# noahares/raxtax

Measured on AMD Instinct MI355X. Metric: classified queries/sec (whole node), higher is better.
Workload: dtype u32 bit-planes + f64

## Files before the change

raxtax_amd/csrc/rtx_api_batch.hip:

```cpp
#include "rtx_index.hpp"

#ifndef RTX_B2_HEAVY_PER_ATILE
#define RTX_B2_HEAVY_PER_ATILE 4u
#endif

namespace rtxi {

int bind(rtx_index *ix) {
    if (!ix) { set_error("null index handle"); return RTX_ERR_INVALID; }
    RTX_HIP(hipSetDevice(ix->device));
    return RTX_OK;
}

int ensure_events(rtx_index *ix, size_t count) {
    while (ix->events.size() < count) {
        hipEvent_t e;
        RTX_HIP(hipEventCreate(&e));
        ix->events.push_back(e);
    }
    return RTX_OK;
}


SubBatch sub_batch_of(rtx_index *ix, uint32_t sb, bool timed) {
    const rtx_index::SubPlan &p = ix->plan[sb];
    SubBatch b;
    b.sb = sb;
    b.q0 = p.q0;
    b.nq = p.nq;
    b.cls = &ix->cls[p.cls];
    b.set = ix->staged ? (sb & 1u) : 0u;
    b.s = ix->stream;
    b.timed = timed;
    b.timed_all = timed && ix->stage_timing != 0;
    return b;
}

int plan_sub_batches(rtx_index *ix) {
    ix->plan.clear();
    uint64_t pos = 0;
    for (uint32_t c = 0; c < ix->n_cls; c++) {
        ix->cls[c].pos0 = pos;
        pos += ix->cls[c].n;
    }
    if (pos != ix->n_q) { set_error("internal: the length classes hold %llu of %llu queries", (unsigned long long)pos, (unsigned long long)ix->n_q); return RTX_ERR_STATE; }
    for (int pass = 0; pass < 2; pass++)
        for (uint32_t c = 0; c < ix->n_cls; c++) {
            rtx_index::BatchClass &k = ix->cls[c];
            if (k.side != (pass == 0)) continue;
            k.sb0 = ix->n_sub_total();
            for (uint64_t a = 0; a < k.n; a += k.sub_batch) ix->plan.push_back({k.pos0 + a, (uint32_t)std::min<uint64_t>(k.sub_batch, k.n - a), c});
            k.n_sub = ix->n_sub_total() - k.sb0;
        }
    return RTX_OK;
}

constexpr uint32_t kDietMinRows = 1024;
uint32_t diet_rows(const rtx_index *ix, uint32_t B) { return std::min<uint32_t>(B, std::max<uint32_t>(kDietMinRows, B >> ix->diet_shift)); }
uint32_t counts_rows_layout(const rtx_index *ix, const rtx_index::BatchClass &k) { return k.diet && !ix->dbg_full_run && !ix->dbg_full ? k.cnt_rows : k.sub_batch; }
uint8_t *counts_lo(rtx_index *ix, rtx_index::Scratch &sc) { return reinterpret_cast<uint8_t *>(sc.d_counts.p); }
uint16_t *counts_hi(rtx_index *ix, const rtx_index::BatchClass &k, rtx_index::Scratch &sc) {
    return reinterpret_cast<uint16_t *>(reinterpret_cast<uint8_t *>(sc.d_counts.p) + (size_t)counts_rows_layout(ix, k) * ix->npad);
}
int ensure_full_counts(rtx_index *ix, const rtx_index::BatchClass &k, rtx_index::Scratch &sc) { return sc.d_counts.alloc(counts_elems(ix, k.planes, k.sub_batch)); }

hipEvent_t stage_event(rtx_index *ix, const SubBatch &b, int stage, int which) {
    return ix->events[((size_t)b.sb * RTX_NUM_STAGES + stage) * 2 + which];
}

static KmerParams kmer_params(rtx_index *ix, const SubBatch &b) {
    rtx_index::Scratch &sc = ix->sc[b.set];
    rtx_index::ResultSet &r = ix->res();
    const rtx_index::BatchClass &k = *b.cls;
    KmerParams kp{};
    kp.bases = ix->d_bases.p;
    kp.base_off = ix->in[ix->cur_in].d_base_off.p;
    kp.q0 = b.q0;
    kp.perm = r.d_perm.p;
    kp.row_of = ix->d_row_of.p;
    kp.list_len = ix->d_list_len.p;
    kp.row_len = ix->d_row_len.p;
    kp.zero_row = ix->n_rows;
    kp.kmers = sc.d_kmers.p;
    kp.kstride = k.kstride;
    kp.seginfo = ix->d_seginfo.p;
    kp.seg_stride = ix->seg_stride;
    kp.segcls = ix->d_segcls.p;
    kp.cls_stride = ix->cls_stride;
    kp.ntiles = ix->ntiles;
    kp.seg_dbits = ix->d_seg_dbits.p;
    kp.seg_sbits = ix->d_seg_sbits.p;
    kp.seg_sbase = ix->d_seg_sbase.p;
    kp.seg_blocks = ix->seg_blocks;
    kp.rows = sc.d_rows.p;
    kp.rstride = k.rstride;
    kp.dmask = sc.d_dmask.p;
    kp.srows = sc.d_srows.p;
    kp.nsparse = sc.d_nsparse.p;
    kp.t = sc.d_t.p;
    kp.nrows = sc.d_nrows.p;
    kp.hq = r.d_hq.p;
    kp.t_all = r.d_t_all.p;
    kp.nrows_all = r.d_nrows_all.p;
    kp.hist = sc.d_hist.p;
    kp.hstride = k.hstride;
    return kp;
}

static bool run_prunes(const rtx_index *ix, const rtx_index::BatchClass &k) { return k.prune && !ix->dbg_full_run; }
static bool on_records_path(const rtx_index *ix, const rtx_index::BatchClass &k, const rtx_index::Scratch &sc) { return run_prunes(ix, k) && k.rec && sc.d_rec.p != nullptr; }
static bool on_diet(const rtx_index *ix, const rtx_index::BatchClass &k, const rtx_index::Scratch &sc) { return on_records_path(ix, k, sc) && k.diet && sc.d_cnt_row.p != nullptr; }

static RecordRef record_ref(const rtx_index *ix, const rtx_index::Scratch &sc, const rtx_index::ResultSet &r) { return RecordRef{sc.d_rec_nslots.p, sc.d_rec_slots.p, sc.d_rec_cnt.p, sc.d_rec.p, ix->rec_slots(), ix->rec_seg_len, r.d_flags.p}; }
static ProbTables prob_tables(const rtx_index *ix) { return ProbTables{ix->d_tab_cmf.p, ix->d_tab_ratio.p, ix->d_tab_off.p, ix->d_tab_moff.p, ix->d_tab_ilo.p, ix->d_tab_sat.p, ix->tab_tmax}; }

int enqueue_kmer(rtx_index *ix, const SubBatch &b, hipStream_t s) {
    KmerParams kp = kmer_params(ix, b);
    kp.mode = run_prunes(ix, *b.cls) && ix->seg_blocks ? 1u : 0u;
    if (b.timed_all) RTX_HIP(hipEventRecord(stage_event(ix, b, RTX_STAGE_KMER_EXTRACT, 0), s));
    launch_kmer_extract(s, kp, b.nq);
    if (b.timed_all) RTX_HIP(hipEventRecord(stage_event(ix, b, RTX_STAGE_KMER_EXTRACT, 1), s));
    return RTX_OK;
}

static HitParams hit_params(rtx_index *ix, const SubBatch &b, uint32_t flags) {
    rtx_index::Scratch &sc = ix->sc[b.set];
    rtx_index::ResultSet &r = ix->res();
    const rtx_index::BatchClass &k = *b.cls;
    HitParams hp{};
    hp.bitmap = ix->d_bitmap.p;
    hp.stride_bytes = ix->stride_bytes;
    hp.n_rows1 = ix->n_rows + 1;
    hp.n_refs = ix->n_refs;
    hp.ref_base = ix->ref_lo;
    hp.rows = sc.d_rows.p;
    hp.rstride = k.rstride;
    hp.dmask = sc.d_dmask.p;
    hp.nrows = sc.d_nrows.p;
    hp.zero_row = ix->n_rows;
    hp.srows = sc.d_srows.p;
    hp.nsparse = sc.d_nsparse.p;
    hp.segslots = ix->d_segslots.p;
    hp.ntiles = ix->ntiles;
    hp.t = sc.d_t.p;
    hp.counts = sc.d_counts.p;
    hp.counts_lo = ix->packs(k.planes) ? counts_lo(ix, sc) : nullptr;
    hp.counts_hi = ix->packs(k.planes) ? counts_hi(ix, k, sc) : nullptr;
    hp.npad = ix->npad;
    hp.hist = sc.d_hist.p;
    hp.hstride = k.hstride;
    hp.tile_max = sc.d_tilemax.p;
    hp.flags = flags;
    hp.q0 = b.q0;
    hp.perm = r.d_perm.p;
    hp.exact = ExactRef{ix->in[ix->cur_in].d_exact_ids.p, ix->in[ix->cur_in].d_exact_off.p, r.dev_exact ? r.d_exact_grp.p : nullptr, ix->d_em_goff.p, ix->d_em_gids.p};
    hp.nq = b.nq;
    hp.group_rows = k.pair ? ix->d_group_rows.p : nullptr;
    hp.group_base = b.sb * ix->groups_per_sub;
    hp.pair_urec = sc.d_urec.p;
    hp.pair_nu = sc.d_nu.p;
    hp.pair_ustride = 2u * k.rstride;
    return hp;
}

static HitParams bounds_params(const rtx_index *ix, const rtx_index::Scratch &sc, const HitParams &hp) {
    HitParams up = hp;
    up.bitmap = ix->d_ubitmap.p;
    up.stride_bytes = ix->u_stride_bytes;
    up.n_refs = ix->u_nblocks;
    up.dmask = nullptr;
    up.nsparse = nullptr;
    up.ntiles = ix->u_ntiles;
    up.counts = nullptr;
    up.counts_lo = nullptr;
    up.counts_hi = nullptr;
    up.hist = nullptr;
    up.tile_max = nullptr;
    up.bounds_tile_ub = sc.d_tile_ub.p;
    up.bounds_tile_stride = ix->ntiles;
    up.bounds_ntiles = ix->ntiles;
    up.bounds_best = sc.d_best_key.p;
    up.flags = 0;
    up.group_base = hp.group_base + ix->n_groups_run;
    return up;
}

static Bounds2Params bounds2_params(const rtx_index *ix, const rtx_index::Scratch &sc, const HitParams &up, bool heavy) {
    Bounds2Params bp{};
    bp.abitmap = ix->d_abitmap.p;
    bp.bbitmap = ix->d_bbitmap.p;
    bp.n_rows1 = ix->n_rows + 1;
    bp.n_atiles = ix->n_atiles;
    bp.ntiles = ix->ntiles;
    bp.zero_row = ix->n_rows;
    bp.pair_urec = sc.d_urec.p;
    bp.pair_nu = sc.d_nu.p;
    bp.pair_ustride = up.pair_ustride;
    bp.nq = up.nq;
    bp.t = sc.d_t.p;
    bp.tile_ub = sc.d_tile_ub.p;
    bp.tile_ub_stride = ix->ntiles;
    bp.best_key = sc.d_best_key.p;
    bp.delta_ct = ix->b2_delta[0];
    bp.delta_cm = ix->b2_delta[1];
    bp.delta_lo = ix->b2_delta[2];
    bp.delta_hi = ix->b2_delta[3];
    bp.group_rows = up.group_rows;
    bp.group_base = up.group_base;
    bp.heavy = heavy ? sc.d_heavy.p : nullptr;
    bp.heavy_max = std::max<uint32_t>(1u, std::min<uint32_t>(RTX_B2_HEAVY_PER_ATILE * ix->n_atiles, ix->n_btiles / 2u));
    return bp;
}

static PruneParams prune_params(rtx_index *ix, const SubBatch &b, uint32_t flags, int part, const ExactRef &exact) {
    rtx_index::Scratch &sc = ix->sc[b.set];
    const rtx_index::BatchClass &k = *b.cls;
    PruneParams pr{};
    pr.tile_ub = sc.d_tile_ub.p;
    pr.best_key = sc.d_best_key.p;
    pr.tile_ub_stride = ix->ntiles;
    pr.ntiles = ix->ntiles;
    pr.nq = b.nq;
    pr.n_refs = ix->n_refs;
    pr.n_total = ix->n_total;
    pr.ref_base = ix->ref_lo;
    pr.phase = (uint32_t)part;
    pr.best = part ? sc.d_best.p : nullptr;
    pr.bitmap = ix->d_bitmap.p;
    pr.cbitmap = part == 0 && (ix->two_level_used || (k.planes > kBounds2MaxPlanes && ix->two_level_opt && ix->n_refs == ix->n_total)) ? reinterpret_cast<const uint2 *>(ix->d_cbitmap.p) : nullptr;
    pr.n_rows1 = ix->n_rows + 1;
    pr.stride_bytes = ix->stride_bytes;
    pr.rows = sc.d_rows.p;
    pr.rstride = k.rstride;
    pr.nrows = sc.d_nrows.p;
    pr.t = sc.d_t.p;
    pr.flags = flags;
    pr.q0 = b.q0;
    pr.perm = ix->res().d_perm.p;
    pr.exact = exact;
    pr.lnfact = ix->d_lnfact.p;
    pr.inv = ix->d_inv.p;
    pr.nlf = std::min<uint32_t>(kLnFactLen, k.tmax + k.tmax / 2 + 2);
    pr.hist = sc.d_hist.p;
    pr.hstride = k.hstride;
    pr.live = sc.d_live.p;
    pr.live_words = LiveLayout{ix->ntiles}.words();
    pr.pair_live = ItemsLayout(b.nq, ix->ntiles).pair_live(sc.d_items.p);
    pr.thr_out = sc.d_prune_thr.p;
    pr.i1_out = sc.d_prune_i1.p;
    pr.stats = ix->d_prune_stats.p;
    pr.detail = ix->debug_taps && ix->d_prune_detail.n >= (size_t)b.nq * kPruneDetailWords ? ix->d_prune_detail.p : nullptr;
    return pr;
}

static HitParams fine_params(const rtx_index *ix, const rtx_index::Scratch &sc, const HitParams &hp) {
    HitParams fp = hp;
    fp.bitmap = ix->d_fbitmap.p;
    fp.stride_bytes = ix->f_stride_bytes;
    fp.n_refs = ix->f_nblocks;
    fp.ntiles = ix->f_ntiles;
    fp.counts = nullptr;
    fp.counts_lo = nullptr;
    fp.counts_hi = nullptr;
    fp.tile_max = nullptr;
    fp.flags = 0;
    fp.group_rows = nullptr;
    fp.live = sc.d_live.p;
    fp.live_words = LiveLayout{ix->ntiles}.words();
    fp.prune_thr = sc.d_prune_thr.p;
    fp.fine_n_refs = ix->n_refs;
    fp.fine_ref_ntiles = ix->ntiles;
    fp.fine_stats = ix->d_prune_stats.p + 2 * kPruneStatCopies * 8;
    return fp;
}

int enqueue_hit(rtx_index *ix, const SubBatch &b, uint32_t flags, hipStream_t s, int part, hipStream_t s_mid) {
    rtx_index::Scratch &sc = ix->sc[b.set];
    rtx_index::ResultSet &r = ix->res();
    const rtx_index::BatchClass &k = *b.cls;
    ix->last_set = b.set;
    HitParams hp = hit_params(ix, b, flags);
    const bool prune = run_prunes(ix, k);
    if (k.pair && part != 2) {
        if (b.timed_all) RTX_HIP(hipEventRecord(stage_event(ix, b, RTX_STAGE_PAIR_UNION, 0), s));
        launch_pair_union(s, sc.d_rows.p, sc.d_nrows.p, k.rstride, b.nq, sc.d_urec.p, sc.d_nu.p, 2u * k.rstride);
        if (b.timed_all) RTX_HIP(hipEventRecord(stage_event(ix, b, RTX_STAGE_PAIR_UNION, 1), s));
    }
    if (b.timed && !prune) RTX_HIP(hipEventRecord(stage_event(ix, b, RTX_STAGE_HIT_COUNT, 0), s));
    if (part != 0 && !prune) { set_error("internal: a split run without tile pruning"); return RTX_ERR_STATE; }
    if (prune) {
        if (part != 2) {
            const HitParams up = bounds_params(ix, sc, hp);
            if (b.timed) RTX_HIP(hipEventRecord(stage_event(ix, b, RTX_STAGE_TILE_BOUNDS, 0), s));
            ix->two_level_used = part == 0 && ix->two_level_opt && ix->d_abitmap.p && ix->d_bbitmap.p && ix->n_refs == ix->n_total && k.planes <= kBounds2MaxPlanes;
            if (ix->two_level_used) {
                const bool heavy_ok = sc.d_heavy.p && sc.d_heavy_items.p && sc.d_heavy_items.n >= HeavyItemsLayout(b.nq, ix->u_ntiles).total();
                launch_bounds2(s, bounds2_params(ix, sc, up, heavy_ok), b.nq, k.planes, up, ix->u_ntiles, heavy_ok ? sc.d_heavy_items.p : nullptr);
            } else {
                RTX_HIP(hipMemsetAsync(sc.d_best_key.p, 0, (size_t)b.nq * 4, s));
                launch_hit_count_pair_bounds(s, up, b.nq, ix->u_ntiles, k.planes);
            }
            if (b.timed) RTX_HIP(hipEventRecord(stage_event(ix, b, RTX_STAGE_TILE_BOUNDS, 1), s));
        }
        if (s_mid && s_mid != s && part == 0) {
            RTX_HIP(hipEventRecord(ix->ev_mid[b.sb], s));
            RTX_HIP(hipStreamWaitEvent(s_mid, ix->ev_mid[b.sb], 0));
            s = s_mid;
        }
        if (b.timed && part != 1) RTX_HIP(hipEventRecord(stage_event(ix, b, RTX_STAGE_TILE_PRUNE, 0), s));
        PruneParams pr = prune_params(ix, b, flags, part, hp.exact);
        const bool records = part == 0 && on_records_path(ix, k, sc), diet = part == 0 && on_diet(ix, k, sc);
        const RecordRef rr = record_ref(ix, sc, r);
        if (records) { pr.rec = rr; pr.rec_max_slots = rr.stride; }
        if (k.diet && !diet) { set_error("internal: the counts buffer is on its diet without the records path"); return RTX_ERR_STATE; }
        if (diet) {
            RTX_HIP(hipMemsetAsync(sc.d_cnt_cursor.p, 0, 4, s));
            pr.cnt_row = sc.d_cnt_row.p;
            pr.cnt_cursor = sc.d_cnt_cursor.p;
            pr.cnt_cap = k.cnt_rows;
            pr.flags_out = r.d_flags.p;
            hp.cnt_row = sc.d_cnt_row.p;
        }
        launch_prune(s, pr, prob_tables(ix), b.nq);
        if (part == 1) { RTX_HIP(hipGetLastError()); return RTX_OK; }
        if (part == 0 && ix->fine_opt && ix->d_fbitmap.p && k.pair && sc.d_fine_items.p) {
            const FineItemsLayout fine(b.nq, ix->f_ntiles);
            uint32_t *const fi = sc.d_fine_items.p;
            launch_fine_bounds(s, fine_params(ix, sc, hp), b.nq, ix->ntiles, ix->f_ntiles, pr.pair_live, fine.cursors(fi), fine.items(fi), fine.count(fi), k.planes);
        }
        RTX_HIP(hipMemsetAsync(sc.d_tilemax.p, 0, (size_t)b.nq * ix->ntiles * 2, s));
        hp.live = sc.d_live.p;
        hp.live_words = pr.live_words;
        hp.prune_thr = sc.d_prune_thr.p;
        if (records) hp.rec = rr;
        if (k.pair) {
            const ItemsLayout items(b.nq, ix->ntiles);
            launch_live_items(s, sc.d_live.p, pr.live_words, pr.pair_live, b.nq, ix->ntiles, items.offsets(sc.d_items.p), items.items(sc.d_items.p), items.count(sc.d_items.p));
            hp.items = items.items(sc.d_items.p);
            hp.n_items = items.count(sc.d_items.p);
        }
        if (ix->seg_blocks) {
            KmerParams kp = kmer_params(ix, b);
            kp.mode = 2u;
            kp.live = sc.d_live.p;
            kp.live_words = pr.live_words;
            launch_kmer_extract(s, kp, b.nq);
        }
        if (b.timed) {
            RTX_HIP(hipEventRecord(stage_event(ix, b, RTX_STAGE_TILE_PRUNE, 1), s));
            RTX_HIP(hipEventRecord(stage_event(ix, b, RTX_STAGE_HIT_COUNT, 0), s));
        }
    }
    if (k.pair) launch_hit_count_pair(s, hp, b.nq, ix->ntiles, k.planes);
    else launch_hit_count(s, hp, b.nq, ix->ntiles, k.planes);
    if (b.timed) RTX_HIP(hipEventRecord(stage_event(ix, b, RTX_STAGE_HIT_COUNT, 1), s));
    ix->hit_stream = s;
    return RTX_OK;
}

int enqueue_count(rtx_index *ix, const SubBatch &b, uint32_t flags, hipStream_t s_mid) {
    int rc = enqueue_kmer(ix, b, b.s);
    return rc ? rc : enqueue_hit(ix, b, flags, b.s, 0, s_mid);
}

static WalkParams walk_params(rtx_index *ix, const SubBatch &b, const double *prefix);
static int reset_sub_alloc(rtx_index *ix, hipStream_t s);

int enqueue_prob_prefix(rtx_index *ix, const SubBatch &b, bool fuse_walk, bool prob_only) {
    rtx_index::Scratch &sc = ix->sc[b.set];
    const rtx_index::BatchClass &k = *b.cls;
    hipStream_t s = b.s;
    ProbParams pp{};
    pp.t = sc.d_t.p;
    pp.hist = sc.d_hist.p;
    pp.hstride = k.hstride;
    pp.tmax = k.tmax;
    pp.n1max = k.tmax / 2 + 1;
    pp.lnfact = ix->d_lnfact.p;
    pp.n_refs = ix->n_total;
    pp.q0 = b.q0;
    pp.table_z = sc.d_table_z.p;
    rtx_index::ResultSet &r = ix->res();
    pp.z = r.d_z.p;
    pp.gs = r.d_gs.p;
    pp.status = r.d_status.p;
    pp.ndist = r.d_ndist.p;
    pp.prune_thr = run_prunes(ix, k) ? sc.d_prune_thr.p : nullptr;
    pp.prune_i1 = pp.prune_thr ? sc.d_prune_i1.p : nullptr;
    if (b.timed_all) RTX_HIP(hipEventRecord(stage_event(ix, b, RTX_STAGE_PROB_TABLE, 0), s));
    if (k.use_tables) {
        launch_prob_order(s, sc.d_t.p, b.nq, sc.d_order.p);
        pp.order = sc.d_order.p;
        launch_prob_lookup(s, pp, prob_tables(ix), b.nq);
    } else {
        if (k.huge) {
            pp.gstride = (uint32_t)((prob_table_lds_bytes(k.tmax) + 7) / 8);
            if (ix->d_prob_scratch.n < (size_t)b.nq * pp.gstride) { set_error("internal: scratch of prob_table too small"); return RTX_ERR_STATE; }
            pp.gscratch = ix->d_prob_scratch.p;
        }
        launch_prob_table(s, pp, b.nq);
    }
    if (b.timed_all) RTX_HIP(hipEventRecord(stage_event(ix, b, RTX_STAGE_PROB_TABLE, 1), s));
    if (prob_only) return RTX_OK;

    PrefixParams fp{};
    fp.status = r.d_status.p;
    fp.t = sc.d_t.p;
    fp.tz_in_lds = (size_t)k.hstride * 8 <= 16 * 1024 ? 1u : 0u;
    fp.q0 = b.q0;
    fp.counts = sc.d_counts.p;
    fp.counts_lo = counts_lo(ix, sc);
    fp.counts_hi = counts_hi(ix, k, sc);
    fp.packed = ix->packs(k.planes) ? 1u : 0u;
    fp.npad = ix->npad;
    fp.table_z = sc.d_table_z.p;
    fp.hstride = k.hstride;
    fp.n_refs = ix->n_refs;
    fp.bnd_bits = ix->d_bnd_bits.p;
    fp.bnd_rank = ix->d_bnd_rank.p;
    fp.prefix = sc.d_prefix.p;
    fp.n_bnd = ix->n_bnd_local;
    fp.tile_max = ix->tile_skip ? sc.d_tilemax.p : nullptr;
    fp.ntiles = ix->ntiles;
    fp.prune_thr = pp.prune_thr;
    fp.prune_stats = fp.prune_thr ? ix->d_prune_stats.p + kPruneStatCopies * 8 : nullptr;
    fp.fuse_walk = fuse_walk ? 1u : 0u;
    const bool records = fuse_walk && on_records_path(ix, k, sc);
    fp.rec_nslots = records ? sc.d_rec_nslots.p : nullptr;
    fp.cnt_row = fuse_walk && on_diet(ix, k, sc) ? sc.d_cnt_row.p : nullptr;
    if (fuse_walk) {
        fp.walk = walk_params(ix, b, sc.d_prefix.p);
        int rc_r = fp.walk.sub_alloc ? reset_sub_alloc(ix, s) : RTX_OK;
        if (rc_r) return rc_r;
    }
    if (b.timed_all) RTX_HIP(hipEventRecord(stage_event(ix, b, RTX_STAGE_TAXON_PREFIX, 0), s));
    launch_taxon_prefix(s, fp, b.nq);
    if (records) {
        TailParams tp{};
        tp.rec = record_ref(ix, sc, r);
        tp.t = sc.d_t.p;
        tp.table_z = sc.d_table_z.p;
        tp.hstride = k.hstride;
        tp.bnd_bits = ix->d_bnd_bits.p;
        tp.bnd_rank = ix->d_bnd_rank.p;
        tp.prefix = sc.d_prefix.p;
        if (fp.cnt_row) { tp.cnt_cursor = sc.d_cnt_cursor.p; tp.cnt_cap = k.cnt_rows; tp.flags_out = r.d_flags.p; }
        tp.n_bnd = ix->n_bnd_local;
        tp.nq = b.nq;
        tp.walk = fp.walk;
        tp.prefix_stats = fp.prune_stats;
        tp.stats = ix->d_prune_stats.p ? ix->d_prune_stats.p + 3 * kPruneStatCopies * 8 : nullptr;
        launch_records_tail(s, tp, b.nq);
    }
    if (b.timed_all) RTX_HIP(hipEventRecord(stage_event(ix, b, RTX_STAGE_TAXON_PREFIX, 1), s));
    return RTX_OK;
}

int alloc_result_set(rtx_index *ix, rtx_index::ResultSet &r, uint64_t n_queries, uint64_t min_arena) {
    int rc;
    if ((rc = r.d_status.alloc(n_queries)) || (rc = r.d_t_all.alloc(n_queries)) || (rc = r.d_nrows_all.alloc(n_queries)) ||
        (rc = r.d_n_rows.alloc(n_queries)) || (rc = r.d_gs.alloc(n_queries)) || (rc = r.d_z.alloc(n_queries)) ||
        (rc = r.d_hq.alloc(n_queries)) || (rc = r.d_row_start.alloc(n_queries)) || (rc = r.d_ndist.alloc(n_queries)) ||
        (rc = r.d_cursor.alloc(2)) || (rc = r.d_flags.alloc(1)))
        return rc;
    const uint64_t want_arena = std::max<uint64_t>(n_queries * 10 + 4096, min_arena);
    if (r.arena_cap < want_arena) {
        if ((rc = r.d_arena.alloc(want_arena))) return rc;
        r.arena_cap = want_arena;
    }
    return alloc_final(ix, r, n_queries);
}

int settle_join(rtx_index *ix) {
    if (ix->join_pending && ix->join_ev) RTX_HIP(hipStreamWaitEvent(ix->stream, ix->join_ev, 0));
    ix->join_pending = false;
    return RTX_OK;
}

int alloc_final(rtx_index *ix, rtx_index::ResultSet &r, uint64_t n_queries) {
    int rc;
    if ((rc = r.d_fin_t.alloc(n_queries)) || (rc = r.d_fin_status.alloc(n_queries)) || (rc = r.d_fin_gs.alloc(n_queries)) ||
        (rc = r.d_fin_row_begin.alloc(n_queries)) || (rc = r.d_fin_row_count.alloc(n_queries)) || (rc = r.d_fin_cursor.alloc(2)))
        return rc;
    if ((rc = r.d_peak2.alloc(n_queries)) || (rc = r.d_peak.alloc(n_queries)) || (rc = r.d_strand.alloc(n_queries))) return rc;
    if (ix->nearest_opt && ((rc = r.d_nearest2.alloc(n_queries)) || (rc = r.d_ties2.alloc(n_queries)) || (rc = r.d_nearest.alloc(n_queries)) || (rc = r.d_ties.alloc(n_queries))))
        return rc;
    if (ix->identity_opt && ((rc = r.d_dist.alloc(n_queries)) || (rc = r.d_qlen.alloc(n_queries)))) return rc;
    if (ix->strand_opt && ((rc = r.d_sel_t.alloc(n_queries)) || (rc = r.d_sel_status.alloc(n_queries)) || (rc = r.d_sel_gs.alloc(n_queries)) ||
                           (rc = r.d_sel_row_begin.alloc(n_queries)) || (rc = r.d_sel_row_count.alloc(n_queries))))
        return rc;
    const uint64_t rows = r.arena_cap, D = ix->fin_D;
    if ((rc = r.d_fin_lineage.alloc(rows)) || (rc = r.d_fin_node.alloc(rows)) || (rc = r.d_fin_depth.alloc(rows)) || (rc = r.d_fin_depth8.alloc(rows)) ||
        (rc = r.d_fin_local.alloc(rows)) || (rc = r.d_fin_conf.alloc(rows * D)) || (rc = r.d_fin_hund.alloc(rows * D)))
        return rc;
    r.fin_cap = rows;
    return RTX_OK;
}

int enqueue_finalise(rtx_index *ix, const SubBatch &b, hipStream_t s) {
    rtx_index::ResultSet &r = ix->res();
    FinaliseParams fp{};
    fp.status = r.d_status.p;
    fp.t_all = r.d_t_all.p;
    fp.gs = r.d_gs.p;
    fp.n_rows = r.d_n_rows.p;
    fp.row_start = r.d_row_start.p;
    fp.arena = r.d_arena.p;
    fp.arena_cap = r.arena_cap;
    fp.perm = r.d_perm.p;
    fp.q0 = b.q0;
    fp.nq = b.nq;
    fp.node_depth = ix->d_node_depth.p;
    fp.node_sig0 = ix->d_node_sig0.p;
    fp.node_begin = ix->d_node_begin.p;
    fp.node_eb = ix->d_node_eb.p;
    fp.D = ix->fin_D;
    fp.o_t = r.d_fin_t.p;
    fp.o_status = r.d_fin_status.p;
    fp.o_gs = r.d_fin_gs.p;
    fp.o_row_begin = r.d_fin_row_begin.p;
    fp.o_row_count = r.d_fin_row_count.p;
    fp.r_lineage = r.d_fin_lineage.p;
    fp.r_node = r.d_fin_node.p;
    fp.r_depth = r.d_fin_depth.p;
    fp.r_depth8 = r.d_fin_depth8.p;
    fp.r_hund = r.d_fin_hund.p;
    fp.r_local = r.d_fin_local.p;
    fp.r_conf = r.d_fin_conf.p;
    fp.row_cap = r.fin_cap;
    fp.fin_cursor = r.d_fin_cursor.p;
    fp.flags_out = r.d_flags.p;
    launch_finalise(s, fp);
    if (r.stream_dl && b.sb < r.h_fin_sub.size())
        RTX_HIP(hipMemcpyAsync(&r.h_fin_sub[b.sb], r.d_fin_cursor.p, 8, hipMemcpyDeviceToHost, s));
    return RTX_OK;
}

static WalkParams walk_params(rtx_index *ix, const SubBatch &b, const double *prefix) {
    rtx_index::ResultSet &r = ix->res();
    WalkParams wp{};
    wp.status = r.d_status.p;
    wp.q0 = b.q0;
    wp.prefix = prefix;
    wp.n_bnd = ix->n_bnd;
    wp.rec = ix->d_noderec.p;
    wp.arena = r.d_arena.p;
    const bool side = b.cls->side;
    wp.arena_cap = side ? r.arena_cap : r.side_base;
    wp.arena_cursor = r.d_cursor.p + (side ? 1 : 0);
    wp.sub_alloc = !side && b.nq >= kWalkSubMinQueries && r.arena_cap < (1ull << 32) ? ix->d_sub_alloc.p : nullptr;
    wp.n_rows = r.d_n_rows.p;
    wp.row_start = r.d_row_start.p;
    wp.flags_out = r.d_flags.p;
    return wp;
}
static int reset_sub_alloc(rtx_index *ix, hipStream_t s) {
    if (ix->d_sub_alloc.p) RTX_HIP(hipMemsetAsync(ix->d_sub_alloc.p, 0, (size_t)kWalkSubAllocs * kWalkSubStride * 8, s));
    return RTX_OK;
}

int enqueue_walk(rtx_index *ix, const SubBatch &b, const double *prefix, hipStream_t s) {
    const WalkParams wp = walk_params(ix, b, prefix);
    int rc_r = wp.sub_alloc ? reset_sub_alloc(ix, s) : RTX_OK;
    if (rc_r) return rc_r;
    if (b.timed_all) RTX_HIP(hipEventRecord(stage_event(ix, b, RTX_STAGE_LINEAGE_WALK, 0), s));
    launch_lineage_walk(s, wp, b.nq);
    if (b.timed_all) RTX_HIP(hipEventRecord(stage_event(ix, b, RTX_STAGE_LINEAGE_WALK, 1), s));
    return RTX_OK;
}

int order_batch(rtx_index *ix, bool cluster) {
    const uint32_t n = (uint32_t)ix->n_q;
    rtx_index::ResultSet &r = ix->res();
    int rc;
    if ((rc = r.d_perm.alloc(n)) || (rc = r.d_iperm.alloc(n))) return rc;
    const bool multi = ix->n_cls > 1;
    const bool sketch = cluster && n > 2;
    if (sketch || multi) {
        if ((rc = ix->d_skey_in.alloc(n)) || (rc = ix->d_skey_out.alloc(n)) || (rc = ix->d_sidx.alloc(n))) return rc;
        size_t tmp = 0;
        if (cluster_sort(ix->stream, nullptr, &tmp, ix->d_skey_in.p, ix->d_skey_out.p, ix->d_sidx.p, r.d_perm.p, n, multi)) {
            set_error("radix sort: size query failed");
            return RTX_ERR_HIP;
        }
        if (ix->d_sort_tmp.n < tmp && (rc = ix->d_sort_tmp.alloc(tmp + 256))) return rc;
        if (sketch) {
            launch_sketch(ix->stream, ix->d_bases.p, ix->in[ix->cur_in].d_base_off.p, n, ix->d_skey_in.p, ix->d_sidx.p);
            if (ix->d_loc_table.p && ix->locator_opt)
                launch_locator(ix->stream, ix->d_bases.p, ix->in[ix->cur_in].d_base_off.p, n, ix->d_loc_table.p, ix->n_total, ix->d_skey_in.p);
        }
        if (multi) launch_class_keys(ix->stream, ix->d_skey_in.p, ix->in[ix->cur_in].d_base_off.p, n, ix->key_lim, !sketch, ix->d_sidx.p);
        tmp = ix->d_sort_tmp.n;
        if (cluster_sort(ix->stream, ix->d_sort_tmp.p, &tmp, ix->d_skey_in.p, ix->d_skey_out.p, ix->d_sidx.p, r.d_perm.p, n, multi)) {
            set_error("radix sort of the query sketches failed");
            return RTX_ERR_HIP;
        }
        launch_invert_perm(ix->stream, r.d_perm.p, n, r.d_iperm.p);
    } else {
        launch_identity_perm(ix->stream, n, r.d_perm.p, r.d_iperm.p);
    }
    RTX_HIP(hipGetLastError());
    return RTX_OK;
}

void record_batch(rtx_index *ix) {
    rtx_index::ResultSet &r = ix->res();
    r.n_q = ix->n_q;
    r.n_user = ix->strand_used ? ix->n_user : ix->n_q;
    r.has_peak = false;
    r.has_nearest = false;
    r.has_identity = false;
    r.profiled = false;
    r.n_sub = ix->n_sub_total();
    r.n_side = 0;
    for (uint32_t c = 0; c < ix->n_cls; c++)
        if (ix->cls[c].side) r.n_side += ix->cls[c].n_sub;
    r.in_set = ix->cur_in;
    r.dev_exact = ix->dev_exact_used;
    r.stream_dl = false;
}

int begin_run(rtx_index *ix, uint32_t *n_sub_out, bool *timed_out, bool cluster) {
    int rc_p = plan_sub_batches(ix);
    if (rc_p) return rc_p;
    const uint32_t n_sub = ix->n_sub_total();
    record_batch(ix);
    rtx_index::ResultSet &r = ix->res();
    const bool timed = n_sub <= 4096;
    if (timed) {
        int rc = ensure_events(ix, (size_t)n_sub * RTX_NUM_STAGES * 2);
        if (rc) return rc;
    }
    const bool ev_all = timed && ix->stage_timing;
    if (ev_all) RTX_HIP(hipEventRecord(ix->events[(size_t)RTX_STAGE_ORDER * 2], ix->stream));
    int rc_o = order_batch(ix, cluster);
    if (rc_o) return rc_o;
    if (ev_all) RTX_HIP(hipEventRecord(ix->events[(size_t)RTX_STAGE_ORDER * 2 + 1], ix->stream));
    {
        uint64_t n_side_q = 0;
        for (uint32_t c = 0; c < ix->n_cls; c++)
            if (ix->cls[c].side) n_side_q += ix->cls[c].n;
        const uint64_t side_rows = n_side_q ? n_side_q * kWalkMaxRows + 64 : 0;
        if (side_rows + ix->n_q * 2 + 1024 > r.arena_cap) {
            int rc_a = r.d_arena.alloc(r.arena_cap + side_rows);
            if (rc_a) return rc_a;
            r.arena_cap += side_rows;
        }
        if (r.fin_cap < r.arena_cap || r.d_fin_t.n < ix->n_q) {
            int rc_f = alloc_final(ix, r, ix->n_q);
            if (rc_f) return rc_f;
        }
        r.side_base = r.arena_cap - side_rows;
        int rc_h = r.h_side_base.resize(2);
        if (rc_h) return rc_h;
        r.h_side_base[0] = 0;
        r.h_side_base[1] = r.side_base;
        RTX_HIP(hipMemcpyAsync(r.d_cursor.p, r.h_side_base.data(), 2 * sizeof(unsigned long long), hipMemcpyHostToDevice, ix->stream));
    }
    RTX_HIP(hipMemsetAsync(r.d_flags.p, 0, sizeof(uint32_t), ix->stream));
    RTX_HIP(hipMemsetAsync(r.d_fin_cursor.p, 0, 2 * sizeof(unsigned long long), ix->stream));
    const bool whole = ix->n_refs == ix->n_total && !ix->staged;
    const bool shard = ix->staged && ix->shard_prune_opt && ix->n_refs != ix->n_total;
    auto scratch_ok = [&](const rtx_index::Scratch &sc, uint32_t B) {
        const ScratchNeed n = ScratchNeed().set_queries(ix, B);
        return sc.d_tile_ub.p != nullptr && sc.d_tile_ub.n >= n.tile_ub && sc.d_best_key.n >= n.best_key && sc.d_prune_thr.n >= n.prune_thr &&
               sc.d_live.n >= n.live && sc.d_best.n >= n.best && sc.d_items.n >= n.items;
    };
    bool any_pair = false, any_prune = false;
    uint32_t b_max = 1;
    for (uint32_t c = 0; c < ix->n_cls; c++) {
        rtx_index::BatchClass &k = ix->cls[c];
        k.pair = ix->pair_opt && cluster && k.planes <= 11 && ix->n_q > 1 && k.rstride <= 4096;
        const rtx_index::Scratch &s0 = ix->sc[k.side ? kSideSet : 0u];
        ScratchNeed need = ScratchNeed().set_queries(ix, k.sub_batch);
        if (whole && ix->rec_opt != 0u && ix->pruning())
            for (uint32_t j = 0; j < 4u; j++) {
                rtx_index::Scratch &sc = ix->sc[j];
                if ((j == kSideSet) != k.side || sc.d_kmers.p == nullptr || sc.d_rec.p == nullptr || sc.d_rec.n >= need.rec) continue;
                RTX_HIP(hipStreamSynchronize(ix->stream));
                if (sc.d_rec.alloc(need.rec)) sc.d_rec.release();
            }
        k.prune = ix->pruning() && k.pair && k.use_tables && ix->tile_skip && ix->d_ubitmap.p && (whole || shard) &&
                  scratch_ok(s0, k.sub_batch) && (!ix->staged || scratch_ok(ix->sc[1], k.sub_batch));
        k.rec = k.prune && whole && ix->rec_opt != 0u && ix->n_bnd_local == ix->n_bnd && s0.d_rec.p != nullptr && s0.d_rec.n >= need.rec;
        auto diet_ok = [&](const rtx_index::Scratch &sc) { return sc.d_rec.p != nullptr && sc.d_cnt_row.p != nullptr && sc.d_cnt_cursor.p != nullptr && sc.d_cnt_row.n >= need.cnt_row; };
        k.diet = k.rec && diet_rows(ix, k.sub_batch) < k.sub_batch && diet_ok(s0);
        if (k.diet && !k.side)
            for (uint32_t j = 1; j <= 2u; j++)
                if (ix->sc[j].d_kmers.p != nullptr && !diet_ok(ix->sc[j])) k.diet = false;
        k.cnt_rows = k.diet ? diet_rows(ix, k.sub_batch) : k.sub_batch;
        {
            need.add_class(ix, k, k.sub_batch, k.cnt_rows);
            for (uint32_t j = 0; j < 4u; j++) {
                rtx_index::Scratch &sc = ix->sc[j];
                if ((j == kSideSet) != k.side || sc.d_kmers.p == nullptr || (sc.d_counts.n >= need.counts && sc.d_prefix.n >= need.prefix)) continue;
                RTX_HIP(hipStreamSynchronize(ix->stream));
                int rc_c = sc.d_counts.alloc(need.counts);
                if (!rc_c) rc_c = sc.d_prefix.alloc(need.prefix);
                if (rc_c) return rc_c;
            }
        }
        any_pair = any_pair || k.pair;
        any_prune = any_prune || k.prune;
        b_max = std::max(b_max, k.sub_batch);
    }
    ix->sub_batch_max = b_max;
    ix->any_prune = any_prune;
    ix->groups_per_sub = (b_max + 1u) / 2u;
    ix->dbg_full = false;
    if (any_prune) {
        int rc_s = ix->d_prune_stats.alloc(kPruneStatCopies * 32);
        if (!rc_s && ix->debug_taps) rc_s = ix->d_prune_detail.alloc((size_t)b_max * kPruneDetailWords);
        if (rc_s) return rc_s;
        RTX_HIP(hipMemsetAsync(ix->d_prune_stats.p, 0, kPruneStatCopies * 256, ix->stream));
    }
    if (any_pair) {
        ix->n_groups_run = n_sub * ix->groups_per_sub;
        int rc_g = ix->d_group_rows.alloc((size_t)2 * n_sub * ix->groups_per_sub);
        if (rc_g) return rc_g;
        RTX_HIP(hipMemsetAsync(ix->d_group_rows.p, 0, (size_t)2 * n_sub * ix->groups_per_sub * 4, ix->stream));
    }
    ix->n_sub_last = timed ? n_sub : 0;
    ix->overlap_used = 0;
    if (ix->overlap_opt != 0u && whole && n_sub >= 2 && !ix->shared_device && any_prune && ix->sc[1].d_kmers.p != nullptr && scratch_ok(ix->sc[1], b_max) == scratch_ok(ix->sc[0], b_max)) {
        ix->overlap_used = 2;
        if (ix->overlap_opt >= 2u && n_sub >= 3 && ix->sc[2].d_kmers.p != nullptr && scratch_ok(ix->sc[2], b_max) == scratch_ok(ix->sc[0], b_max)) ix->overlap_used = 3;
    }
    if (r.dev_exact) {
        ExactParams xp{ix->d_bases.p, ix->in[ix->cur_in].d_base_off.p, (uint32_t)ix->n_q, ix->d_em_table.p, ix->em_bits, ix->d_em_rep_off.p,
                       ix->d_em_rep_bytes.p, r.d_exact_grp.p, ix->em_hash_mask};
        const bool ev = timed && ix->stage_timing;
        if (ev) RTX_HIP(hipEventRecord(ix->events[(size_t)RTX_STAGE_EXACT_MATCH * 2], ix->stream));
        launch_exact_match(ix->stream, xp);
        if (ev) RTX_HIP(hipEventRecord(ix->events[(size_t)RTX_STAGE_EXACT_MATCH * 2 + 1], ix->stream));
        if (!r.ev_exact) RTX_HIP(hipEventCreateWithFlags(&r.ev_exact, hipEventDisableTiming));
        RTX_HIP(hipEventRecord(r.ev_exact, ix->stream));
    }
    *n_sub_out = n_sub;
    *timed_out = timed;
    return RTX_OK;
}

int enqueue_batch(rtx_index *ix, uint32_t flags) {
    if (ix->n_refs != ix->n_total) {
        set_error("this handle holds a reference shard: drive it with rtx_shard_count/_prob/_walk");
        return RTX_ERR_STATE;
    }
    uint32_t n_sub = 0;
    bool timed = false;
    int rc;
    if (ix->join_pending && !ix->hold_join && (rc = settle_join(ix))) return rc;
    rc = begin_run(ix, &n_sub, &timed, ix->cluster != 0);
    if (rc) return rc;
    rtx_index::ResultSet &r = ix->res();
    ix->n_near_last = 0;
    r.has_nearest = ix->nearest_opt != 0u && r.d_nearest2.p != nullptr && r.d_nearest2.n >= r.n_q && r.d_nearest.n >= r.n_user;
    if (ix->nearest_opt != 0u && !r.has_nearest) { set_error("internal: RTX_OPT_NEAREST without its arrays"); return RTX_ERR_STATE; }
    ix->ident_timed = false;
    r.has_identity = ix->identity_opt != 0u && r.has_nearest && r.d_dist.p != nullptr && r.d_dist.n >= r.n_user && r.d_qlen.n >= r.n_user && ix->d_em_ref_grp.p != nullptr;
    if (ix->identity_opt != 0u && !r.has_identity) { set_error("internal: RTX_OPT_IDENTITY without its arrays"); return RTX_ERR_STATE; }
    if (n_sub <= 4096) {
        if (!ix->copy_stream) RTX_HIP(hipStreamCreateWithFlags(&ix->copy_stream, hipStreamNonBlocking));
        while (r.ev_sub.size() < n_sub) {
            hipEvent_t e;
            RTX_HIP(hipEventCreateWithFlags(&e, hipEventDisableTiming));
            r.ev_sub.push_back(e);
        }
        if ((rc = r.h_cursor_sub.resize(n_sub)) || (rc = r.h_fin_sub.resize(n_sub))) return rc;
        r.stream_dl = true;
    }
    const bool fuse = ix->n_bnd_local == ix->n_bnd;
    const uint32_t nsets = ix->overlap_used;
    const bool overlap = nsets != 0u;
    if (overlap) {
        if (!ix->stream2) RTX_HIP(hipStreamCreateWithFlags(&ix->stream2, hipStreamNonBlocking));
        if (nsets == 3u && !ix->stream3) RTX_HIP(hipStreamCreateWithFlags(&ix->stream3, hipStreamNonBlocking));
        while (ix->ev_front.size() < n_sub) {
            hipEvent_t e, f, g;
            RTX_HIP(hipEventCreateWithFlags(&e, hipEventDisableTiming));
            RTX_HIP(hipEventCreateWithFlags(&f, hipEventDisableTiming));
            RTX_HIP(hipEventCreateWithFlags(&g, hipEventDisableTiming));
            ix->ev_front.push_back(e);
            ix->ev_back.push_back(f);
            ix->ev_mid.push_back(g);
        }
    }
    const uint32_t n_side = r.n_side;
    const bool ra = ix->run_ahead_opt != 0u && nsets == 2u && n_side == 0u && r.stream_dl && n_sub >= 2u;
    if (ix->join_pending) {
        if (ra) ix->join_pending = false;
        else if ((rc = settle_join(ix))) return rc;
    }
    if (ra)
        for (uint32_t k = 0; k < 2u; k++)
            if (!ix->ev_set_free[k]) RTX_HIP(hipEventCreateWithFlags(&ix->ev_set_free[k], hipEventDisableTiming));
    for (uint32_t sb = 0; sb < n_sub; sb++) {
        SubBatch b = sub_batch_of(ix, sb, timed);
        const bool side = b.cls->side;
        if (side) {
            b.set = kSideSet;
            if (overlap) {
                if (sb == 0) {
                    RTX_HIP(hipEventRecord(ix->ev_mid[0], ix->stream));
                    RTX_HIP(hipStreamWaitEvent(ix->stream2, ix->ev_mid[0], 0));
                }
                b.s = ix->stream2;
            }
        } else if (overlap) {
            const uint32_t m = sb - n_side;
            b.set = m % nsets;
            if (m >= nsets) RTX_HIP(hipStreamWaitEvent(ix->stream, ix->ev_back[sb - nsets], 0));
            else if (ra && ix->set_busy[b.set]) RTX_HIP(hipStreamWaitEvent(ix->stream, ix->ev_set_free[b.set], 0));
        }
        if ((rc = enqueue_count(ix, b, flags, nsets == 3u && !side && n_side == 0 ? ix->stream3 : nullptr))) return rc;
        if (overlap && !side) {
            RTX_HIP(hipEventRecord(ix->ev_front[sb], ix->hit_stream));
            b.s = ix->stream2;
            RTX_HIP(hipStreamWaitEvent(b.s, ix->ev_front[sb], 0));
        }
        {
            const rtx_index::Scratch &sc = ix->sc[b.set];
            launch_peak(b.s, PeakParams{sc.d_hist.p, b.cls->hstride, sc.d_t.p, b.q0, r.d_perm.p, b.nq, r.d_peak2.p});
        }
        if (r.has_nearest) {
            rtx_index::Scratch &sc = ix->sc[b.set];
            const rtx_index::BatchClass &k = *b.cls;
            NearestParams np{};
            np.hist = sc.d_hist.p;
            np.hstride = k.hstride;
            np.t = sc.d_t.p;
            np.q0 = b.q0;
            np.perm = r.d_perm.p;
            np.nq = b.nq;
            np.tile_max = sc.d_tilemax.p;
            np.ntiles = ix->ntiles;
            np.n_refs = ix->n_refs;
            np.counts = sc.d_counts.p;
            np.counts_lo = ix->packs(k.planes) ? counts_lo(ix, sc) : nullptr;
            np.counts_hi = ix->packs(k.planes) ? counts_hi(ix, k, sc) : nullptr;
            np.npad = ix->npad;
            np.cnt_rows = counts_rows_layout(ix, k);
            np.cnt_row = on_diet(ix, k, sc) ? sc.d_cnt_row.p : nullptr;
            if (on_records_path(ix, k, sc)) {
                const RecordRef rr = record_ref(ix, sc, r);
                np.rec_nslots = rr.nslots;
                np.rec_slots = rr.slots;
                np.rec_cnt = rr.cnt;
                np.rec = rr.rec;
                np.rec_stride = rr.stride;
                np.rec_seg_len = rr.seg_len;
            }
// ... 168 lines not shown
    k.hstride = (uint32_t)align_up(tmax + 1, 8);
    k.planes = tmax <= 255 ? 8 : (tmax <= 1023 ? 10 : (tmax <= kMidClassMaxT && mid ? 11 : (tmax <= 4095 ? 12 : 16)));
    k.huge = prob_table_lds_bytes((uint32_t)tmax) > kProbTableLdsLimit;
}

static int size_workspace(rtx_index *ix, uint64_t n_queries);

int prepare_workspace(rtx_index *ix, uint64_t n_queries, const uint64_t cls_n_in[5], const uint64_t cls_max_in[5]) {
    uint64_t cn[5], cm[5];
    for (int c = 0; c < 5; c++) { cn[c] = cls_n_in[c]; cm[c] = cls_max_in[c]; }
    if (ix->n_refs != ix->n_total) {
        uint64_t mx = 0;
        for (int c = 0; c < 5; c++) mx = std::max(mx, cm[c]);
        return prepare_workspace_single(ix, n_queries, mx >= 8 ? mx - 7 : 1, mx);
    }
    if (cn[0] && cn[1] && cn[0] < kMinShortClass) { cn[1] += cn[0]; cm[1] = std::max(cm[1], cm[0]); cn[0] = 0; cm[0] = 0; }
    if (cn[2] && ((cn[2] < kMinMidClass && ix->prob_mode != 2) || !ix->pair_opt || !ix->pruning() || ix->prob_mode == 1)) { cn[3] += cn[2]; cm[3] = std::max(cm[3], cm[2]); cn[2] = 0; cm[2] = 0; }
    if (cn[3] && cn[4] && cn[3] + cn[4] <= kSideMaxQueries) { cn[4] += cn[3]; cm[4] = std::max(cm[4], cm[3]); cn[3] = 0; cm[3] = 0; }
    const uint64_t key[14] = {n_queries, cn[0], cn[1], cn[2] << 32 | cn[3], cn[4], cm[0], cm[1], cm[2] << 32 | cm[3], cm[4], ix->sub_batch_req,
                              (uint64_t)ix->packed_opt | (uint64_t)ix->pair_opt << 1 | (uint64_t)ix->pruning() << 2 | (uint64_t)ix->shard_prune_opt << 3 | (uint64_t)ix->fine_opt << 4 |
                                  (uint64_t)(ix->prob_mode & 3) << 5 | (uint64_t)ix->rec_opt << 8 | (uint64_t)ix->overlap_opt << 16 | (uint64_t)ix->min_subs << 20,
                              (uint64_t)ix->n_bnd_local, ix->shared_device ? 1u : 0u, ix->strand_opt | ix->nearest_opt << 1 | ix->identity_opt << 2};
    if (ix->ws_valid && std::memcmp(key, ix->ws_key, sizeof key) == 0 && !ix->staged) {
        ix->n_q = n_queries;
        return RTX_OK;
    }
    ix->ws_valid = false;
    ix->n_cls = 0;
    const uint64_t cls_len[4] = {255 + 7, 1023 + 7, kMidClassMaxT + 7, class3_max_len()};
    for (int c = 0; c < 4; c++) ix->key_lim[c] = ~0ull;
    int last = -1;
    for (int c = 0; c < 5; c++) {
        if (!cn[c]) continue;
        if (last >= 0) ix->key_lim[ix->n_cls - 1] = cls_len[last];
        shape_class(ix->cls[ix->n_cls], cn[c], cm[c], c == 2);
        ix->n_cls++;
        last = c;
    }
    if (ix->n_cls == 0) { set_error("internal: a batch without queries"); return RTX_ERR_INVALID; }
    ix->n_q = n_queries;
    int rc = size_workspace(ix, n_queries);
    if (rc) return rc;
    std::memcpy(ix->ws_key, key, sizeof key);
    ix->ws_valid = true;
    return RTX_OK;
}

int prepare_workspace_single(rtx_index *ix, uint64_t n_queries, uint64_t tmax, uint64_t max_len) {
    ix->ws_valid = false;
    ix->strand_used = false;
    tmax = std::min<uint64_t>(tmax, 65535);
    ix->n_cls = 1;
    for (int c = 0; c < 4; c++) ix->key_lim[c] = ~0ull;
    shape_class(ix->cls[0], n_queries, tmax + 7);
    ix->cls[0].max_len = max_len;
    ix->n_q = n_queries;
    return size_workspace(ix, n_queries);
}

static int size_workspace(rtx_index *ix, uint64_t n_queries) {
    int rc;
    uint32_t tab_t = 0;
    for (uint32_t c = 0; c < ix->n_cls; c++) {
        if (ix->cls[c].tmax > kProbTablesMaxT && ix->prob_mode == 2) { set_error("prob tables need t <= %u (got %u)", kProbTablesMaxT, ix->cls[c].tmax); return RTX_ERR_TOO_LONG; }
        if (ix->cls[c].tmax <= kProbTablesMaxT && ix->cls[c].planes <= 11) tab_t = std::max(tab_t, ix->cls[c].tmax);
    }
    bool tables = false;
    if (tab_t && (rc = ensure_prob_tables(ix, tab_t, &tables))) return rc;
    for (uint32_t c = 0; c < ix->n_cls; c++) ix->cls[c].use_tables = tables && ix->cls[c].tmax >= 2 && ix->cls[c].tmax <= kProbTablesMaxT && ix->cls[c].planes <= 11;
    rtx_index::ResultSet &r = ix->res();
    if ((rc = alloc_result_set(ix, r, n_queries))) return rc;
    if ((rc = ix->d_sub_alloc.alloc((size_t)kWalkSubAllocs * kWalkSubStride))) return rc;
    const uint64_t want_arena = n_queries * 10 + 4096;
    uint32_t n_sets = ix->n_refs == ix->n_total && !ix->shared_device ? 1u + std::min<uint32_t>(ix->overlap_opt, 2u) : 1u;
    size_t free_b = 0, total_b = 0;
    RTX_HIP(hipMemGetInfo(&free_b, &total_b));
    uint64_t held = 0;
    for (const auto &sc : ix->sc) held += sc.d_counts.n * 2 + sc.d_prefix.n * 8 + sc.d_rec.n * 4 + sc.d_srows.n * 4;
    const uint64_t budget = (uint64_t)((free_b + held) * 0.6);
    uint64_t worst = 0;
    for (uint32_t c = 0; c < ix->n_cls; c++) {
        rtx_index::BatchClass &k = ix->cls[c];
        k.will_prune = ix->pruning() && ix->d_ubitmap.p && ix->pair_opt && ix->ntiles >= RTX_PRUNE_MIN_TILES && k.tmax <= kProbTablesMaxT && (ix->n_refs == ix->n_total || ix->shard_prune_opt);
        const uint64_t per_q = class_per_q(ix, k);
        uint32_t B = ix->sub_batch_req;
        if (B == 0) {
            B = (uint32_t)std::min<uint64_t>(k.will_prune ? kDefaultSubBatchPruned : ix->ntiles >= 16 ? kDefaultSubBatchLarge : kDefaultSubBatch,
                                             std::max<uint64_t>(64, budget / per_q));
            if (k.huge) B = std::min<uint32_t>(B, 1024u);
            if (k.will_prune && k.n < (uint64_t)ix->min_subs * B) B = (uint32_t)std::max<uint64_t>(16384, (k.n + ix->min_subs - 1) / ix->min_subs);
        }
        if (B > kMaxSubBatch) B = kMaxSubBatch;
        B = (uint32_t)std::max<uint64_t>(1, std::min<uint64_t>(B, k.n));
        k.sub_batch = B;
        worst = std::max<uint64_t>(worst, (uint64_t)B * per_q);
    }
    {
        uint32_t bulk = 0;
        for (uint32_t c = 1; c < ix->n_cls; c++)
            if (ix->cls[c].n > ix->cls[bulk].n) bulk = c;
        worst = 0;
        for (uint32_t c = 0; c < ix->n_cls; c++) {
            ix->cls[c].side = ix->n_refs == ix->n_total && c != bulk && ix->cls[c].n <= kSideMaxQueries && ix->cls[c].n * 64u <= ix->cls[bulk].n;
            if (!ix->cls[c].side) worst = std::max<uint64_t>(worst, (uint64_t)ix->cls[c].sub_batch * class_per_q(ix, ix->cls[c]));
        }
    }
    {
        uint64_t n_side_q = 0;
        for (uint32_t c = 0; c < ix->n_cls; c++)
            if (ix->cls[c].side) n_side_q += ix->cls[c].n;
        const uint64_t want2 = want_arena + (n_side_q ? n_side_q * kWalkMaxRows + 64 : 0);
        if (r.arena_cap < want2) {
            if ((rc = r.d_arena.alloc(want2))) return rc;
            r.arena_cap = want2;
        }
    }
    while (n_sets > 1u && (uint64_t)n_sets * worst > budget) n_sets--;
    ix->staged = false;
    if ((rc = plan_sub_batches(ix))) return rc;
    if ((rc = alloc_scratch_set(ix, 0))) return rc;
    {
        bool any_side = false;
        for (uint32_t c = 0; c < ix->n_cls; c++) any_side = any_side || ix->cls[c].side;
        if (any_side) { if ((rc = alloc_scratch_set(ix, kSideSet))) return rc; }
        else ix->sc[kSideSet].release_all();
    }
    for (uint32_t k = 1; k <= 2u; k++) {
        if (k < n_sets && ix->n_sub_total() > 1) {
            if (alloc_scratch_set(ix, k)) ix->sc[k].d_kmers.release();
        } else if (ix->n_refs == ix->n_total) {
            ix->sc[k].release_all();
        }
    }
    return RTX_OK;
}

int alloc_scratch_set(rtx_index *ix, uint32_t k) {
    int rc;
    rtx_index::Scratch &sc = ix->sc[k];
    const ScratchNeed n = scratch_set_need(ix, k);
    if ((rc = sc.d_kmers.alloc(n.kmers)) || (rc = sc.d_rows.alloc(n.rows)) || (rc = sc.d_dmask.alloc(n.dmask)) || (rc = sc.d_nsparse.alloc(n.nsparse)) || (rc = sc.d_srows.alloc(n.srows)) ||
        (rc = sc.d_t.alloc(n.t)) || (rc = sc.d_nrows.alloc(n.nrows)) || (rc = sc.d_counts.alloc(n.counts)) || (rc = sc.d_hist.alloc(n.hist)) || (rc = sc.d_table_z.alloc(n.hist)) ||
        (rc = sc.d_prefix.alloc(n.prefix)) || (rc = sc.d_order.alloc(n.order)) || (rc = sc.d_tilemax.alloc(n.tilemax)) || (rc = sc.d_urec.alloc(n.urec)) || (rc = sc.d_nu.alloc(n.nu)))
        return rc;
    if (n.prob_scratch && (rc = ix->d_prob_scratch.alloc(std::max(n.prob_scratch, ix->d_prob_scratch.n)))) return rc;
    if (ix->pruning() && ix->d_ubitmap.p && (ix->n_refs == ix->n_total || ix->shard_prune_opt)) {
        if ((rc = sc.d_tile_ub.alloc(n.tile_ub)) || (rc = sc.d_best_key.alloc(n.best_key)) || (rc = sc.d_prune_thr.alloc(n.prune_thr)) || (rc = sc.d_prune_i1.alloc(n.prune_i1)) ||
            (rc = sc.d_best.alloc(n.best)) || (rc = sc.d_live.alloc(n.live)) || (rc = sc.d_items.alloc(n.items)))
            return rc;
        if (ix->d_abitmap.p && (sc.d_heavy.alloc(n.heavy) || sc.d_heavy_items.alloc(n.heavy_items))) { sc.d_heavy.release(); sc.d_heavy_items.release(); }
        if (ix->d_fbitmap.p && sc.d_fine_items.alloc(n.fine_items)) sc.d_fine_items.release();
        if (ix->rec_opt && ix->n_refs == ix->n_total) {
            if (sc.d_rec_nslots.alloc(n.rec_nslots) || sc.d_rec_slots.alloc(n.rec_slots) || sc.d_rec_cnt.alloc(n.rec_cnt) ||
                sc.d_rec.alloc(n.rec) || sc.d_cnt_row.alloc(n.cnt_row) || sc.d_cnt_cursor.alloc(n.cnt_cursor))
                sc.d_rec.release();
        }
    }
    return RTX_OK;
}

}

extern "C" {

int rtx_batch_prefetch(rtx_index *ix, uint64_t n_queries, const uint8_t *bases, const uint64_t *base_off,
                       const uint32_t *exact_ids, const uint64_t *exact_off) {
    int rc = bind(ix);
    if (rc) return rc;
    rtx_index::Inputs &in = ix->in[ix->cur_in ^ 1u];
    const bool with_labels = in.labels_pending && in.n_labels == n_queries;
    in.labels_pending = in.has_labels = false;
    const bool with_weights = in.weights_pending && in.n_weights == n_queries;
    in.weights_pending = in.has_weights = false;
    if (n_queries == 0 || !base_off || (!bases && base_off[n_queries])) {
        set_error("rtx_batch_upload: invalid argument");
        return RTX_ERR_INVALID;
    }
    const bool both = ix->strand_opt != 0u;
    if (both) {
        if (exact_off || exact_ids) { set_error("RTX_OPT_STRAND: exact-match ids cannot be passed in (those of the reverse complements must come from the same lookup: pass NULL)"); return RTX_ERR_INVALID; }
        if (!rtx_index_has_exact_lookup(ix) || ix->n_refs != ix->n_total) { set_error("RTX_OPT_STRAND needs the exact-match lookup of the device (a handle built from the reference sequences, RTX_OPT_DEVICE_EXACT on)"); return RTX_ERR_STATE; }
        if (n_queries > 0x7FFFFFFFull) { set_error("RTX_OPT_STRAND: too many queries in one batch"); return RTX_ERR_INVALID; }
    }
    const uint64_t n_dev = both ? 2 * n_queries : n_queries;
    if (!ix->h2d_stream) RTX_HIP(hipStreamCreateWithFlags(&ix->h2d_stream, hipStreamNonBlocking));
    if (!in.ready) RTX_HIP(hipEventCreateWithFlags(&in.ready, hipEventDisableTiming));
    if (in.recorded) RTX_HIP(hipEventSynchronize(in.ready));
    in.staged = false;
    if (ix->ev_activated) RTX_HIP(hipStreamWaitEvent(ix->h2d_stream, ix->ev_activated, 0));
    uint64_t max_len = 0;
    uint64_t cls_n[5] = {0, 0, 0, 0, 0}, cls_max[5] = {0, 0, 0, 0, 0};
    {
        const uint64_t lim3 = class3_max_len();
        for (uint64_t q = 0; q < n_queries; q++) {
            if (base_off[q + 1] < base_off[q]) { set_error("base_off not monotone at query %llu", (unsigned long long)q); return RTX_ERR_INVALID; }
            const uint64_t len = base_off[q + 1] - base_off[q];
            max_len = std::max(max_len, len);
            const int c = len <= 262 ? 0 : (len <= 1030 ? 1 : (len <= kMidClassMaxT + 7 ? 2 : (len <= lim3 ? 3 : 4)));
            cls_n[c]++;
            cls_max[c] = std::max(cls_max[c], len);
        }
    }
    const uint64_t total = base_off[n_queries] - base_off[0];
    uint64_t n_exact = 0;
    if (exact_off) {
        if (exact_off[0] != 0) { set_error("exact_off[0] must be 0"); return RTX_ERR_INVALID; }
        n_exact = exact_off[n_queries];
        for (uint64_t q = 0; q < n_queries; q++)
            if (exact_off[q + 1] < exact_off[q]) { set_error("exact_off not monotone"); return RTX_ERR_INVALID; }
        if (n_exact && !exact_ids) { set_error("exact_ids is null"); return RTX_ERR_INVALID; }
        for (uint64_t i = 0; i < n_exact; i++)
            if (exact_ids[i] >= ix->n_total) { set_error("exact id %u out of range", exact_ids[i]); return RTX_ERR_INVALID; }
    }
    const uint64_t n_packed = (total + 1) / 2;
    if ((rc = in.h_packed.resize(total + 64)) || (rc = in.h_base_off.resize(n_queries + 1)) || (rc = in.d_packed.alloc(total + 64)) ||
        (rc = in.d_base_off.alloc(n_dev + 1)) || (rc = in.d_exact_off.alloc(n_dev + 1)) || (rc = in.d_exact_ids.alloc(n_exact + 1)))
        return rc;
    for (uint64_t q = 0; q <= n_queries; q++) in.h_base_off[q] = base_off[q] - base_off[0];
    in.packed = total == 0 || rtx::pack_nibbles_mt(bases + base_off[0], total, in.h_packed.data(), rtx::host_threads(8u));
    if (!in.packed) std::memcpy(in.h_packed.data(), bases + base_off[0], total);
    RTX_HIP(hipMemcpyAsync(in.d_packed.p, in.h_packed.data(), in.packed ? n_packed : total, hipMemcpyHostToDevice, ix->h2d_stream));
    RTX_HIP(hipMemcpyAsync(in.d_base_off.p, in.h_base_off.data(), (n_queries + 1) * 8, hipMemcpyHostToDevice, ix->h2d_stream));
    if (exact_off) {
        if ((rc = in.h_exact_off.resize(n_queries + 1)) || (rc = in.h_exact_ids.resize(n_exact + 1))) return rc;
        std::memcpy(in.h_exact_off.data(), exact_off, (n_queries + 1) * 8);
        if (n_exact) std::memcpy(in.h_exact_ids.data(), exact_ids, n_exact * 4);
        RTX_HIP(hipMemcpyAsync(in.d_exact_off.p, in.h_exact_off.data(), (n_queries + 1) * 8, hipMemcpyHostToDevice, ix->h2d_stream));
        if (n_exact) RTX_HIP(hipMemcpyAsync(in.d_exact_ids.p, in.h_exact_ids.data(), n_exact * 4, hipMemcpyHostToDevice, ix->h2d_stream));
    } else {
        RTX_HIP(hipMemsetAsync(in.d_exact_off.p, 0, (n_dev + 1) * 8, ix->h2d_stream));
    }
    RTX_HIP(hipEventRecord(in.ready, ix->h2d_stream));
    in.recorded = true;
    in.n_q = n_dev;
    in.n_user = n_queries;
    in.total = total;
    in.max_len = max_len;
    for (int c = 0; c < 5; c++) { in.cls_n[c] = both ? 2 * cls_n[c] : cls_n[c]; in.cls_max[c] = cls_max[c]; }
    in.n_exact = n_exact;
    in.has_exact = exact_off != nullptr;
    in.has_labels = with_labels;
    in.has_weights = with_weights;
    in.staged = true;
    return RTX_OK;
}

int rtx_batch_activate(rtx_index *ix) {
    int rc = bind(ix);
    if (rc) return rc;
    rtx_index::Inputs &in = ix->in[ix->cur_in ^ 1u];
    if (!in.staged) { set_error("rtx_batch_activate without a staged batch (rtx_batch_prefetch)"); return RTX_ERR_STATE; }
    ix->uploaded = ix->ran = ix->synced = false;
    if ((rc = prepare_workspace(ix, in.n_q, in.cls_n, in.cls_max))) return rc;
    const bool both = in.n_q != in.n_user;
    const uint64_t total_dev = both ? 2 * in.total : in.total;
    ix->sum_query_bytes = total_dev;
    if ((rc = ix->d_bases.alloc(total_dev + 64))) return rc;
    RTX_HIP(hipStreamWaitEvent(ix->stream, in.ready, 0));
    if (in.packed) {
        rtx::launch_unpack_nibbles(ix->stream, in.d_packed.p, ix->d_bases.p, in.total, in.total + 64);
    } else {
        RTX_HIP(hipMemcpyAsync(ix->d_bases.p, in.d_packed.p, in.total, hipMemcpyDeviceToDevice, ix->stream));
        RTX_HIP(hipMemsetAsync(ix->d_bases.p + in.total, 0, 64, ix->stream));
    }
    if (both) {
        rtx::launch_revcomp(ix->stream, ix->d_bases.p, in.d_base_off.p, (uint32_t)in.n_user, in.total);
        RTX_HIP(hipMemsetAsync(ix->d_bases.p + total_dev, 0, 64, ix->stream));
    }
    ix->strand_used = both;
    ix->n_user = in.n_user;
    ix->dev_exact_used = !in.has_exact && ix->dev_exact_opt && ix->d_em_table.p && ix->n_refs == ix->n_total;
    if (ix->dev_exact_used && (rc = ix->res().d_exact_grp.alloc(in.n_q))) return rc;
    if (!ix->ev_activated) RTX_HIP(hipEventCreateWithFlags(&ix->ev_activated, hipEventDisableTiming));
    RTX_HIP(hipEventRecord(ix->ev_activated, ix->stream));
    in.staged = false;
    ix->cur_in ^= 1u;
    ix->uploaded = true;
    return RTX_OK;
}

int rtx_pack_bases(const uint8_t *bases, uint64_t n_bases, uint8_t *packed) {
    if ((!bases || !packed) && n_bases) { set_error("rtx_pack_bases: null argument"); return RTX_ERR_INVALID; }
    return rtx::pack_nibbles_mt(bases, n_bases, packed, rtx::host_threads(8u)) ? 1 : 0;
}

int rtx_batch_upload(rtx_index *ix, uint64_t n_queries, const uint8_t *bases, const uint64_t *base_off,
                     const uint32_t *exact_ids, const uint64_t *exact_off) {
    if (ix) ix->uploaded = ix->ran = ix->synced = false;
    int rc = rtx_batch_prefetch(ix, n_queries, bases, base_off, exact_ids, exact_off);
    return rc ? rc : rtx_batch_activate(ix);
}

int rtx_batch_run(rtx_index *ix, uint32_t flags) {
    int rc = bind(ix);
    if (rc) return rc;
    if (!ix->uploaded) { set_error("rtx_batch_run before rtx_batch_upload"); return RTX_ERR_STATE; }
    ix->last_flags = flags;
    ix->synced = false;
    rc = enqueue_batch(ix, flags);
    ix->ran = rc == RTX_OK;
    return rc;
}

int rtx_batch_sync(rtx_index *ix) {
    int rc = bind(ix);
    if (rc) return rc;
    if (!ix->ran) { set_error("rtx_batch_sync before rtx_batch_run"); return RTX_ERR_STATE; }
// ... 8 lines not shown
```

raxtax_amd/csrc/rtx_hit_pair.hip:

```cpp
#include <hip/hip_runtime.h>

#include <algorithm>

#include "rtx_hit_common.hpp"

namespace rtx {

constexpr uint32_t kPairCap = kHitListCap;
constexpr uint32_t kPairListDw = kPairCap + 192u;
constexpr uint32_t kPairMaskWords = 64u;
constexpr uint32_t kPairSidDw = 2u * kSparseIt * 64u;
constexpr uint32_t kPairLdsBytes = 3u * kPairListDw * 4u + 2u * kPairMaskWords * 8u + 32u * 4u + kPairSidDw * 4u;
#ifndef RTX_PAIR_NB
#define RTX_PAIR_NB 3
#endif
#ifndef RTX_PAIR_WAVES
#define RTX_PAIR_WAVES 2
#endif
constexpr int kPairNB = RTX_PAIR_NB;

constexpr uint32_t kUnionMaxRows = 2048u;
__device__ __forceinline__ uint32_t lower_bound_u16(const uint16_t *l, uint32_t n, uint32_t key) {
    uint32_t lo = 0;
#pragma unroll
// ... 130 lines not shown
    constexpr int kRecChunks = 8;
    auto load_recs = [&](uint2 (&rec)[kRecChunks], uint32_t from) {
#pragma unroll
        for (int c = 0; c < kRecChunks; c++) {
            const uint32_t i = from + (uint32_t)c * 64u + lane;
            rec[c] = urec[i < p.pair_ustride ? i : p.pair_ustride - 1u];
        }
    };
    uint2 rec[kRecChunks];
    load_recs(rec, 0);
    const uint32_t ns_a = kBounds || !has_a ? 0u : p.nsparse[(size_t)qa * p.ntiles + tile], ns_b = !kBounds && has_b ? p.nsparse[(size_t)qb * p.ntiles + tile] : 0u;
    const uint32_t *srows_a = p.srows + ((size_t)qa * p.ntiles + tile) * (kSegMaxSparseRows + 1);
    const uint32_t *srows_b = p.srows + ((size_t)(has_b ? qb : qa) * p.ntiles + tile) * (kSegMaxSparseRows + 1);
    {
        const unsigned long long *dm_a = p.dmask + ((size_t)qa * p.ntiles + tile) * mwords;
        const unsigned long long *dm_b = p.dmask + ((size_t)(has_b ? qb : qa) * p.ntiles + tile) * mwords;
        uint32_t sa[kSparseIt], sb[kSparseIt];
#pragma unroll
        for (int it = 0; it < kSparseIt; it++) {
            sa[it] = kBounds ? 0u : srows_a[(uint32_t)it * 64u + lane];
            sb[it] = kBounds ? 0u : srows_b[(uint32_t)it * 64u + lane];
        }
        for (uint32_t i = lane; i < mwords; i += 64) {
            m_a[i] = has_a ? (kBounds ? ~0ull : dm_a[i]) : 0ull;
            m_b[i] = has_b ? (kBounds ? ~0ull : dm_b[i]) : 0ull;
        }
#pragma unroll
        for (int it = 0; it < kSparseIt; it++) {
            l_sid[(uint32_t)it * 64u + lane] = sa[it];
            l_sid[(kSparseIt + (uint32_t)it) * 64u + lane] = sb[it];
        }
    }
    wave_lds_sync();
    const uint32_t n_u = p.pair_nu[pair];
    const __amdgpu_buffer_rsrc_t rsrc = tile_rsrc(p.bitmap, p.n_rows1, tile);
    const uint32_t voff = lane * 16u;
    const uint32_t zero_off = p.zero_row << 10;
    const unsigned long long lt_mask = (1ull << lane) - 1ull;
    uint32_t rows_loaded = 0;
    uint32_t u0 = 0;
    bool first_round = true;
    while (u0 < n_u) {
        uint32_t n_both = 0, n_a = 0, n_b = 0;
        bool room = true;
        while (room && u0 < n_u) {
            if (u0) load_recs(rec, u0);
#pragma unroll
            for (int c = 0; c < kRecChunks; c++) {
                if (u0 >= n_u) break;
                if (n_both + 64u > kPairCap || n_a + 64u > kPairCap || n_b + 64u > kPairCap) { room = false; break; }
                const bool in = u0 + lane < n_u;
                const uint32_t pos_a = rec[c].y & 0xFFFFu, pos_b = rec[c].y >> 16;
                const bool da = in && (rec[c].x & (1u << 30)) && ((m_a[pos_a >> 6] >> (pos_a & 63u)) & 1ull);
                const bool db = in && (rec[c].x & (1u << 31)) && ((m_b[pos_b >> 6] >> (pos_b & 63u)) & 1ull);
                const uint32_t row = (rec[c].x & 0x3FFFFFFFu) << 10;
                const bool sh = da && db && first_round, oa = da && !sh, ob = db && !sh;
                const unsigned long long bb = __ballot(sh), ba = __ballot(oa), bo = __ballot(ob);
                if (sh) l_both[n_both + (uint32_t)__popcll(bb & lt_mask)] = row;
                if (oa) l_a[n_a + (uint32_t)__popcll(ba & lt_mask)] = row;
                if (ob) l_b[n_b + (uint32_t)__popcll(bo & lt_mask)] = row;
                n_both += (uint32_t)__popcll(bb);
                n_a += (uint32_t)__popcll(ba);
                n_b += (uint32_t)__popcll(bo);
                u0 += 64;
            }
        }
        rows_loaded += n_both + n_a + n_b;
        constexpr int NB = NP > 10 ? 3 : kPairNB;
        constexpr uint32_t GR = 8u * (uint32_t)NB;
        const uint32_t g_both = (n_both + GR - 1u) / GR, g_a = (n_a + GR - 1u) / GR, g_b = (n_b + GR - 1u) / GR;
        for (uint32_t i = n_both + lane; i < g_both * GR; i += 64) l_both[i] = zero_off;
        for (uint32_t i = n_a + lane; i < g_a * GR; i += 64) l_a[i] = zero_off;
        for (uint32_t i = n_b + lane; i < g_b * GR; i += 64) l_b[i] = zero_off;
        wave_lds_sync();
        const uint32_t *first = g_both ? l_both : (g_a ? l_a : (g_b ? l_b : nullptr));
        if (first) {
            uint4 buf[NB][8];
            const uint32_t idv = first[lane < GR ? lane : 0u];
#pragma unroll
            for (int b = 0; b < NB; b++) load8v_at(buf[b], rsrc, voff, idv, b * 8);
            const uint32_t *after_a = g_b ? l_b : l_zero, *after_both = g_a ? l_a : after_a;
            if (g_both) {
                fold_seg<NP, 1, NB>(pa, pb, buf, l_both, g_both, after_both, lane, rsrc, voff);
#pragma unroll
                for (int w = 0; w < 4; w++)
#pragma unroll
                    for (int b = 0; b < NP; b++) pb[w][b] = pa[w][b];
            }
            if (g_a) fold_seg<NP, 1, NB>(pa, pb, buf, l_a, g_a, after_a, lane, rsrc, voff);
            if (g_b) fold_seg<NP, 2, NB>(pa, pb, buf, l_b, g_b, l_zero, lane, rsrc, voff);
        }
        wave_lds_sync();
        first_round = false;
    }
    if (lane == 0 && p.group_rows) atomicAdd(&p.group_rows[p.group_base + pair], rows_loaded);

    if (kBounds == 1) {
        if (has_a) bounds_epilogue<NP>(p, pa, qa, tile, lane);
        if (has_b) bounds_epilogue<NP>(p, pb, qb, tile, lane);
        return;
    }
    if (kBounds == 2) {
        if (has_a) fine_epilogue<NP>(p, pa, qa, tile, lane, fine_a);
        if (has_b) fine_epilogue<NP>(p, pb, qb, tile, lane, fine_b);
        if (lane == 0u && p.fine_stats) atomicAdd(&p.fine_stats[(size_t)(pair & (kPruneStatCopies - 1u)) * 8u + 1u], 1ull);
        return;
    }
    uint32_t *hist_lds = lds_dw;
    uint32_t *cnt8 = lds_dw + (NP > 10 ? 2048u : 1024u);
    uint4 pre_a[kSparseIt][kSparseV], pre_b[kSparseIt][kSparseV];
    auto thr_of = [&](uint32_t q) -> uint32_t { return p.prune_thr ? (uint32_t)__builtin_amdgcn_readfirstlane((int)p.prune_thr[q]) : 0u; };
    if (ns_a) sparse_prefetch(p, lane, ns_a, l_sid, pre_a);
    if (ns_b) sparse_prefetch(p, lane, ns_b, l_sid + kSparseIt * 64u, pre_b);
    if (has_a) {
        const uint32_t ka = rec_slot_of(p, qa, tile, lane);
        if (ka != 0xFFFFFFFFu) rec_epilogue<NP>(p, pa, qa, tile, lane, p.t[qa], active, hist_lds, cnt8, ns_a, pre_a, thr_of(qa), ka, p.rec.stride);
        else hit_epilogue_x<NP, kPacked, true, true, true>(p, pa, qa, tile, lane, p.t[qa], active, hist_lds, cnt8, ns_a, srows_a, pre_a, thr_of(qa));
    }
    if (has_b) {
        wave_lds_sync();
        const uint32_t kb = rec_slot_of(p, qb, tile, lane);
        if (kb != 0xFFFFFFFFu) rec_epilogue<NP>(p, pb, qb, tile, lane, p.t[qb], active, hist_lds, cnt8, ns_b, pre_b, thr_of(qb), kb, p.rec.stride);
        else hit_epilogue_x<NP, kPacked, true, true, true>(p, pb, qb, tile, lane, p.t[qb], active, hist_lds, cnt8, ns_b, srows_b, pre_b, thr_of(qb));
    }
}

template <int NP, bool kPacked, int kBounds, bool kItems>
__global__ __launch_bounds__(64, RTX_PAIR_WAVES) void hit_count_pair_kernel(HitParams p) {
    extern __shared__ uint32_t lds_dw[];
    const uint32_t lane = threadIdx.x;
    if (kItems) {
        const uint32_t n_items = (uint32_t)__builtin_amdgcn_readfirstlane((int)p.n_items[0]), g8 = gridDim.x >> 3, x = blockIdx.x & 7u;
        const uint32_t e8 = (n_items + 7u) >> 3, first = x * e8;
        const uint32_t end = first + e8 < n_items ? first + e8 : n_items;
        uint32_t j = first + (blockIdx.x >> 3);
        while (j < end) {
            const uint32_t item = (uint32_t)__builtin_amdgcn_readfirstlane((int)p.items[j]);
            uint32_t lane_v = lane;
            asm volatile("" : "+v"(lane_v));
            pair_tile_block<NP, kPacked, kBounds>(p, lds_dw, item / p.ntiles, item % p.ntiles, lane_v);
            wave_lds_sync();
            if (e8 <= g8) break;
            uint32_t nxt = 0;
            if (lane_v == 0u) nxt = atomicAdd(&p.n_items[1u + x], 1u);
            j = first + g8 + (uint32_t)__builtin_amdgcn_readfirstlane((int)nxt);
        }
        return;
    }
    const uint32_t np8 = gridDim.x >> 3;
    const uint32_t pair = blockIdx.x < np8 * 8u ? (blockIdx.x & 7u) * np8 + (blockIdx.x >> 3) : blockIdx.x;
    pair_tile_block<NP, kPacked, kBounds>(p, lds_dw, pair, blockIdx.y, lane);
}

__global__ __launch_bounds__(1024) void live_offsets_kernel(const uint32_t *__restrict__ pair_live, uint32_t np, uint32_t *__restrict__ off,
                                                            uint32_t *__restrict__ n_items) {
    __shared__ uint32_t wsum[2][16];
    const uint32_t tid = threadIdx.x, lane = tid & 63u, wave = tid >> 6;
    constexpr uint32_t kPer = 8;
    uint32_t carry = 0, buf = 0;
    for (uint32_t base = 0; base < np; base += 1024u * kPer, buf ^= 1u) {
        const uint32_t i0 = base + tid * kPer;
        uint32_t c[kPer], cnt = 0;
#pragma unroll
        for (uint32_t j = 0; j < kPer; j++) c[j] = i0 + j < np ? pair_live[i0 + j] : 0u;
#pragma unroll
        for (uint32_t j = 0; j < kPer; j++) cnt += c[j];
        const uint32_t incl = wave_incl_scan_u32(cnt);
        if (lane == 63u) wsum[buf][wave] = incl;
        __syncthreads();
        uint32_t o = carry + incl - cnt, tot = 0;
#pragma unroll
        for (uint32_t w = 0; w < 16u; w++) {
            const uint32_t sw = wsum[buf][w];
            o += w < wave ? sw : 0u;
            tot += sw;
        }
#pragma unroll
        for (uint32_t j = 0; j < kPer; j++) {
            if (i0 + j < np) off[i0 + j] = o;
            o += c[j];
        }
        carry += tot;
    }
    if (tid == 0u) n_items[0] = carry;
    if (tid < 8u) n_items[1u + tid] = 0;
}

__global__ __launch_bounds__(1024) void live_items_kernel(const uint32_t *__restrict__ live, uint32_t live_words, uint32_t nq, uint32_t ntiles,
                                                          const uint32_t *__restrict__ off, uint32_t *__restrict__ items) {
    extern __shared__ uint32_t tl[];
    const uint32_t tid = threadIdx.x, lane = tid & 63u;
    const uint32_t np = (nq + 1u) / 2u, g0 = blockIdx.x * 1024u, pair = g0 + tid;
    for (uint32_t T = tid; T < ntiles; T += 1024) tl[T] = 0;
    __syncthreads();
    const uint32_t nw = (ntiles + 31u) >> 5;
    const bool valid = pair < np;
    const uint32_t *wa = live + (size_t)((valid ? pair : 0u) * 2u) * live_words;
    const bool hb = valid && pair * 2u + 1u < nq;
    if (valid)
        for (uint32_t w = 0; w < nw; w++) {
            uint32_t bits = wa[w] | (hb ? wa[live_words + w] : 0u);
            while (bits) {
                atomicAdd(&tl[w * 32u + (uint32_t)__builtin_ctz(bits)], 1u);
                bits &= bits - 1u;
            }
        }
    __syncthreads();
    if (tid < 64u) {
        uint32_t running = 0;
        for (uint32_t T0 = 0; T0 < ntiles; T0 += 64) {
            const uint32_t v = T0 + lane < ntiles ? tl[T0 + lane] : 0u;
            const uint32_t incl = wave_incl_scan_u32(v);
            if (T0 + lane < ntiles) tl[T0 + lane] = running + incl - v;
            running += (uint32_t)__builtin_amdgcn_readlane((int)incl, 63);
        }
    }
    __syncthreads();
    if (!valid) return;
    const uint32_t base = off[g0];
    for (uint32_t w = 0; w < nw; w++) {
        uint32_t bits = wa[w] | (hb ? wa[live_words + w] : 0u);
        while (bits) {
            const uint32_t tile = w * 32u + (uint32_t)__builtin_ctz(bits);
            bits &= bits - 1u;
            items[base + atomicAdd(&tl[tile], 1u)] = pair * ntiles + tile;
        }
    }
}

void launch_pair_union(hipStream_t s, const uint32_t *rows, const uint32_t *nrows, uint32_t rstride, uint32_t nq, uint2 *urec,
                       uint32_t *nu, uint32_t ustride) {
    hipLaunchKernelGGL(pair_union_kernel, dim3((nq + 1u) / 2u), dim3(64), 0, s, rows, nrows, rstride, nq, urec, nu, ustride);
}

#ifndef RTX_ITEM_GRID_HALVES
#define RTX_ITEM_GRID_HALVES 4
#endif
template <int NP>
static void launch_hit_count_pair_np(hipStream_t s, const HitParams &p, uint32_t nq, uint32_t ntiles) {
    static_assert(3u * kPairListDw >= 1024u + 2048u + 64u, "histogram (t <= 1023) and byte counters (+ pad words) alias the lists");
    static_assert(kPairLdsBytes >= (2048u + 2048u + 64u) * 4u, "eleven planes: histogram (t <= 2047) and byte counters alias the whole prologue");
    static_assert(kSegMaxSparseRows + 1 >= kSparseIt * 64, "the slot id lists are read without a bound");
    const uint32_t np = (nq + 1u) / 2u;
    const dim3 grid = p.items ? dim3((uint32_t)((std::min<uint64_t>((uint64_t)np * ntiles, std::max<uint64_t>((uint64_t)RTX_ITEM_GRID_HALVES * np / 2u, 2048ull)) + 7u) & ~7ull)) : dim3(np, ntiles);
    if (NP <= 10 && p.counts_lo) {
        if (p.items) hipLaunchKernelGGL((hit_count_pair_kernel<(NP <= 10 ? NP : 10), true, false, true>), grid, dim3(64), kPairLdsBytes, s, p);
        else hipLaunchKernelGGL((hit_count_pair_kernel<(NP <= 10 ? NP : 10), true, false, false>), grid, dim3(64), kPairLdsBytes, s, p);
    } else {
        if (p.items) hipLaunchKernelGGL((hit_count_pair_kernel<NP, false, false, true>), grid, dim3(64), kPairLdsBytes, s, p);
        else hipLaunchKernelGGL((hit_count_pair_kernel<NP, false, false, false>), grid, dim3(64), kPairLdsBytes, s, p);
    }
}
void launch_hit_count_pair(hipStream_t s, const HitParams &p, uint32_t nq, uint32_t ntiles, int planes) {
    if (planes <= 8) launch_hit_count_pair_np<8>(s, p, nq, ntiles);
    else if (planes <= 10) launch_hit_count_pair_np<10>(s, p, nq, ntiles);
    else launch_hit_count_pair_np<11>(s, p, nq, ntiles);
}

void launch_live_items(hipStream_t s, const uint32_t *live, uint32_t live_words, const uint32_t *pair_live, uint32_t nq, uint32_t ntiles, uint32_t *off,
                       uint32_t *items, uint32_t *n_items) {
    const uint32_t np = (nq + 1u) / 2u;
    hipLaunchKernelGGL(live_offsets_kernel, dim3(1), dim3(1024), 0, s, pair_live, np, off, n_items);
    hipLaunchKernelGGL(live_items_kernel, dim3((np + 1023u) / 1024u), dim3(1024), (size_t)ntiles * 4, s, live, live_words, nq, ntiles, off, items);
}

void launch_hit_count_pair_bounds(hipStream_t s, const HitParams &p, uint32_t nq, uint32_t u_ntiles, int planes) {
    if (planes <= 8) hipLaunchKernelGGL((hit_count_pair_kernel<8, true, 1, false>), dim3((nq + 1u) / 2u, u_ntiles), dim3(64), kPairLdsBytes, s, p);
    else if (planes <= 10) hipLaunchKernelGGL((hit_count_pair_kernel<10, true, 1, false>), dim3((nq + 1u) / 2u, u_ntiles), dim3(64), kPairLdsBytes, s, p);
    else hipLaunchKernelGGL((hit_count_pair_kernel<11, false, 1, false>), dim3((nq + 1u) / 2u, u_ntiles), dim3(64), kPairLdsBytes, s, p);
}

void launch_hit_count_pair_bounds_items(hipStream_t s, const HitParams &p, uint32_t nq, uint32_t u_ntiles, int planes) {
    const uint32_t np = (nq + 1u) / 2u;
    const dim3 grid((uint32_t)((std::min<uint64_t>((uint64_t)np * u_ntiles, 4096ull) + 7u) & ~7ull));
    if (planes <= 8) hipLaunchKernelGGL((hit_count_pair_kernel<8, true, 1, true>), grid, dim3(64), kPairLdsBytes, s, p);
    else if (planes <= 10) hipLaunchKernelGGL((hit_count_pair_kernel<10, true, 1, true>), grid, dim3(64), kPairLdsBytes, s, p);
    else hipLaunchKernelGGL((hit_count_pair_kernel<11, false, 1, true>), grid, dim3(64), kPairLdsBytes, s, p);
}

__device__ __forceinline__ uint32_t fine_pair_mask(const uint32_t *live, uint32_t live_words, uint32_t pair, uint32_t nq, uint32_t U) {
    const uint32_t T0 = U * 8u;
    const uint32_t *wa = live + (size_t)(pair * 2u) * live_words + (T0 >> 5);
    uint32_t m = (wa[0] >> (T0 & 31u)) & 0xFFu;
    if (pair * 2u + 1u < nq) m |= (wa[live_words] >> (T0 & 31u)) & 0xFFu;
    return m;
}
__global__ __launch_bounds__(256) void fine_count_kernel(const uint32_t *__restrict__ live, uint32_t live_words, const uint32_t *__restrict__ pair_live,
                                                         uint32_t nq, uint32_t f_ntiles, uint32_t *__restrict__ cnt) {
    const uint32_t pair = blockIdx.x * 256u + threadIdx.x, np = (nq + 1u) / 2u, lane = threadIdx.x & 63u;
    const bool on = pair < np && pair_live[pair < np ? pair : 0u] >= kFineMinLive;
    for (uint32_t U = 0; U < f_ntiles; U++) {
        const unsigned long long b = __ballot(on && fine_pair_mask(live, live_words, pair, nq, U) != 0u);
        if (b && lane == (uint32_t)__builtin_ctzll(b)) atomicAdd(&cnt[U], (uint32_t)__popcll(b));
    }
}
__global__ void fine_scan_kernel(uint32_t *__restrict__ cnt, uint32_t f_ntiles, uint32_t *__restrict__ n_items) {
    uint32_t run = 0;
    for (uint32_t U = 0; U < f_ntiles; U++) {
        const uint32_t c = cnt[U];
        cnt[U] = run;
        run += c;
    }
    n_items[0] = run;
    for (uint32_t x = 1; x <= 8u; x++) n_items[x] = 0;
}
__global__ __launch_bounds__(256) void fine_scatter_kernel(const uint32_t *__restrict__ live, uint32_t live_words, const uint32_t *__restrict__ pair_live,
                                                           uint32_t nq, uint32_t f_ntiles, uint32_t *__restrict__ cursor, uint32_t *__restrict__ items) {
    const uint32_t pair = blockIdx.x * 256u + threadIdx.x, np = (nq + 1u) / 2u, lane = threadIdx.x & 63u;
    const bool on = pair < np && pair_live[pair < np ? pair : 0u] >= kFineMinLive;
    for (uint32_t U = 0; U < f_ntiles; U++) {
        const bool has = on && fine_pair_mask(live, live_words, pair, nq, U) != 0u;
        const unsigned long long b = __ballot(has);
        if (b == 0ull) continue;
        const int leader = __builtin_ctzll(b);
        uint32_t base = 0;
        if ((int)lane == leader) base = atomicAdd(&cursor[U], (uint32_t)__popcll(b));
        base = (uint32_t)__shfl((int)base, leader, 64);
        if (has) items[base + (uint32_t)__popcll(b & ((1ull << lane) - 1ull))] = pair * f_ntiles + U;
    }
}
__global__ __launch_bounds__(256) void pair_live_recount_kernel(const uint32_t *__restrict__ live, uint32_t live_words, uint32_t nq, uint32_t ntiles,
                                                                uint32_t *__restrict__ pair_live, unsigned long long *__restrict__ stats) {
    const uint32_t pair = blockIdx.x * 256u + threadIdx.x, np = (nq + 1u) / 2u;
    uint32_t n = 0;
    if (pair < np) {
        const uint32_t *wa = live + (size_t)(pair * 2u) * live_words;
        const bool hb = pair * 2u + 1u < nq;
        for (uint32_t w = 0; w < (ntiles + 31u) >> 5; w++) n += (uint32_t)__popc(wa[w] | (hb ? wa[live_words + w] : 0u));
        pair_live[pair] = n;
    }
    if (stats) {
        n = wave_incl_scan_u32(n);
        if ((threadIdx.x & 63u) == 63u && n) atomicAdd(&stats[(size_t)(blockIdx.x & (kPruneStatCopies - 1u)) * 8u + 2u], (unsigned long long)n);
    }
}

void launch_fine_bounds(hipStream_t s, const HitParams &p, uint32_t nq, uint32_t ntiles, uint32_t f_ntiles, uint32_t *pair_live, uint32_t *cnt,
                        uint32_t *items, uint32_t *n_items, int planes) {
    const uint32_t np = (nq + 1u) / 2u, nb = (np + 255u) / 256u;
    (void)hipMemsetAsync(cnt, 0, (size_t)f_ntiles * 4, s);
    hipLaunchKernelGGL(fine_count_kernel, dim3(nb), dim3(256), 0, s, p.live, p.live_words, pair_live, nq, f_ntiles, cnt);
    hipLaunchKernelGGL(fine_scan_kernel, dim3(1), dim3(1), 0, s, cnt, f_ntiles, n_items);
    hipLaunchKernelGGL(fine_scatter_kernel, dim3(nb), dim3(256), 0, s, p.live, p.live_words, pair_live, nq, f_ntiles, cnt, items);
    HitParams fp = p;
    fp.items = items;
    fp.n_items = n_items;
    const dim3 grid((uint32_t)((std::min<uint64_t>((uint64_t)np * f_ntiles, std::max<uint64_t>((uint64_t)RTX_ITEM_GRID_HALVES * np / 2u, 2048ull)) + 7u) & ~7ull));
    if (planes <= 8) hipLaunchKernelGGL((hit_count_pair_kernel<8, true, 2, true>), grid, dim3(64), kPairLdsBytes, s, fp);
    else if (planes <= 10) hipLaunchKernelGGL((hit_count_pair_kernel<10, true, 2, true>), grid, dim3(64), kPairLdsBytes, s, fp);
    else hipLaunchKernelGGL((hit_count_pair_kernel<11, false, 2, true>), grid, dim3(64), kPairLdsBytes, s, fp);
    hipLaunchKernelGGL(pair_live_recount_kernel, dim3(nb), dim3(256), 0, s, p.live, p.live_words, nq, ntiles, pair_live, p.fine_stats);
}

}
```

raxtax_amd/csrc/rtx_index.hpp:

```cpp
#pragma once

#include <hip/hip_runtime.h>

#include <algorithm>
#include <cmath>
#include <cstdlib>
#include <cstring>
#include <thread>

#include "rtx_internal.hpp"
#include "rtx_kernels.hpp"
#include "rtx_math.hpp"

using namespace rtx;

namespace rtxi {


constexpr uint32_t kEmptyRow = 0xFFFFFFFFu;
constexpr uint32_t kLnFactLen = 98320;

#define RTX_HIP(call)                                                                          \
    do {                                                                                       \
        hipError_t e_ = (call);                                                                \
// ... 106 lines not shown
    DevBuf<double> d_lnfact, d_inv;
    int prob_mode = 0;
    uint32_t tab_tmax = 0;
    DevBuf<double> d_tab_cmf, d_tab_ratio;
    DevBuf<uint64_t> d_tab_off;
    DevBuf<uint32_t> d_tab_moff;
    DevBuf<uint16_t> d_tab_ilo, d_tab_sat;
    FlatNodes nodes;
    std::vector<uint32_t> bnd;
    uint32_t n_bnd = 0;
    DevBuf<uint4> d_noderec;
    DevBuf<uint8_t> d_node_depth, d_node_sig0;
    DevBuf<uint32_t> d_node_begin;
    DevBuf<double> d_node_eb;
    uint32_t fin_D = 1;
    DevBuf<uint32_t> d_bnd_rank;
    DevBuf<uint8_t> d_bnd_bits;
    uint32_t dev_exact_opt = 1;
    uint32_t nearest_opt = 0;
    uint32_t identity_opt = 0;
    DevBuf<uint32_t> d_em_ref_grp;
    uint32_t strand_opt = 0;
    bool strand_used = false;
    uint64_t n_user = 0;
    uint32_t em_groups = 0, em_bits = 0;
    uint64_t em_hash_mask = ~0ull;
    DevBuf<uint2> d_em_table;
    DevBuf<uint64_t> d_em_rep_off;
    DevBuf<uint8_t> d_em_rep_bytes;
    DevBuf<uint32_t> d_em_goff, d_em_gids;
    std::vector<uint32_t> h_em_goff, h_em_gids;
    bool dev_exact_used = false;
    struct HostExact {
        std::vector<uint32_t> grp;
        std::vector<uint64_t> off;
        std::vector<uint32_t> ids;
        bool csr_valid = false, valid = false;
    } host_exact[2];
    uint64_t n_q = 0;
    bool uploaded = false, ran = false, synced = false;
    uint32_t last_flags = 0;
    uint32_t cluster = 1;
    uint32_t packed_opt = 1;
    uint32_t tile_skip = 1;
    uint32_t pair_opt = 1;
    uint32_t prune_opt = 1;
    uint32_t self_sample_opt = 1;
    bool prune_pays = true;
    double self_live = -1.0;
    bool pruning() const { return prune_opt != 0u && (prune_pays || self_sample_opt == 0u); }
    bool dbg_full = false;
    bool dbg_full_run = false;
    DevBuf<uint32_t> d_ubitmap;
    uint32_t u_stride_bytes = 0, u_ntiles = 0;
    uint64_t u_nblocks = 0;
    DevBuf<uint32_t> d_fbitmap;
    uint32_t f_stride_bytes = 0, f_ntiles = 0;
    uint64_t f_nblocks = 0;
    uint32_t fine_opt = 1;
    DevBuf<uint32_t> d_abitmap;
    DevBuf<uint8_t> d_bbitmap;
    uint32_t n_atiles = 0, n_btiles = 0;
    DevBuf<uint8_t> d_cbitmap;
    uint32_t two_level_opt = 1;
    uint32_t b2_delta[4] = {283u, 205u, 92u, 128u};
    bool two_level_used = false;
    uint32_t rec_seg_len = 1024;
    uint32_t diet_shift = 3;
    uint32_t rec_opt = 4;
    uint32_t rec_slots() const { return std::min<uint32_t>(rec_opt, kRecMaxSlots); }
    uint32_t overlap_opt = 1;
    uint32_t overlap_used = 0;
    hipStream_t stream2 = nullptr, stream3 = nullptr, hit_stream = nullptr;
    std::vector<hipEvent_t> ev_front, ev_back, ev_mid;
    DevBuf<unsigned long long> d_prune_stats;
    uint32_t shard_prune_opt = 0;
    uint32_t debug_taps = 0;
    DevBuf<uint32_t> d_prune_detail;
    uint32_t locator_opt = 1;
    DevBuf<uint32_t> d_loc_table;
    DevBuf<uint32_t> d_group_rows;
    uint32_t n_groups_run = 0;
    uint32_t groups_per_sub = 0;
    bool packs(int pl) const { return packed_opt && pl <= 10; }
    DevBuf<uint64_t> d_skey_in, d_skey_out;
    DevBuf<uint32_t> d_sidx;
    DevBuf<uint8_t> d_sort_tmp;
    DevBuf<uint8_t> d_bases;
    struct Inputs {
        DevBuf<uint8_t> d_packed;
        DevBuf<uint64_t> d_base_off, d_exact_off;
        DevBuf<uint32_t> d_exact_ids;
        PinBuf<uint8_t> h_packed;
        PinBuf<uint64_t> h_base_off, h_exact_off;
        PinBuf<uint32_t> h_exact_ids;
        uint64_t n_q = 0, total = 0, max_len = 0, n_exact = 0;
        uint64_t n_user = 0;
        uint64_t cls_n[5] = {0, 0, 0, 0, 0}, cls_max[5] = {0, 0, 0, 0, 0};
        bool packed = true, has_exact = false, staged = false, recorded = false;
        DevBuf<char> d_labels;
        DevBuf<uint64_t> d_label_off;
        PinBuf<char> h_labels;
        PinBuf<uint64_t> h_label_off;
        uint64_t n_labels = 0;
        bool labels_pending = false, has_labels = false;
        DevBuf<uint32_t> d_weights;
        PinBuf<uint32_t> h_weights;
        uint64_t n_weights = 0;
        bool weights_pending = false, has_weights = false;
        hipEvent_t ready = nullptr;
    } in[2];
    uint32_t cur_in = 0;
    hipStream_t h2d_stream = nullptr;
    hipEvent_t ev_activated = nullptr;
    uint64_t sum_query_bytes = 0;
    uint32_t sub_batch_req = 0;
    uint32_t min_subs = 4;
    uint64_t ws_key[14] = {0};
    bool ws_valid = false;
    struct BatchClass {
        uint64_t pos0 = 0, n = 0, max_len = 0;
        uint32_t tmax = 0, kstride = 0, rstride = 0, hstride = 0, sub_batch = 0, sb0 = 0, n_sub = 0;
        int planes = 10;
        bool use_tables = false, pair = false, prune = false, rec = false, huge = false, will_prune = false;
        bool side = false;
        bool diet = false;
        uint32_t cnt_rows = 0;
    } cls[5];
    uint32_t n_cls = 0;
    uint64_t key_lim[4] = {~0ull, ~0ull, ~0ull, ~0ull};
    struct SubPlan { uint64_t q0; uint32_t nq, cls; };
    std::vector<SubPlan> plan;
    uint32_t n_sub_total() const { return (uint32_t)plan.size(); }
    uint32_t sub_batch_max = 0;
    bool any_prune = false;
    DevBuf<double> d_prob_scratch;
    struct Scratch {
        DevBuf<uint16_t> d_kmers, d_counts, d_tilemax;
        DevBuf<uint32_t> d_rows, d_t, d_nrows, d_hist, d_order, d_srows, d_nsparse;
        DevBuf<unsigned long long> d_dmask;
        DevBuf<double> d_table_z, d_prefix;
        DevBuf<uint2> d_urec;
        DevBuf<uint32_t> d_nu;
        DevBuf<uint32_t> d_live, d_best_key;
        DevBuf<uint32_t> d_items;
        DevBuf<uint16_t> d_tile_ub, d_prune_thr, d_prune_i1;
        DevBuf<uint32_t> d_best;
        DevBuf<uint8_t> d_heavy;
        DevBuf<uint32_t> d_heavy_items;
        DevBuf<uint32_t> d_fine_items;
        DevBuf<uint16_t> d_rec_nslots, d_rec_slots;
        DevBuf<uint32_t> d_rec_cnt, d_rec;
        DevBuf<uint32_t> d_cnt_row, d_cnt_cursor;
        template <class S, class F>
        static void each(S &s, F &&f) {
            f(s.d_kmers); f(s.d_counts); f(s.d_tilemax); f(s.d_rows); f(s.d_t); f(s.d_nrows); f(s.d_hist); f(s.d_order); f(s.d_srows); f(s.d_nsparse);
            f(s.d_dmask); f(s.d_table_z); f(s.d_prefix); f(s.d_urec); f(s.d_nu); f(s.d_live); f(s.d_best_key); f(s.d_items); f(s.d_tile_ub); f(s.d_prune_thr);
            f(s.d_prune_i1); f(s.d_best); f(s.d_heavy); f(s.d_heavy_items); f(s.d_fine_items); f(s.d_rec_nslots); f(s.d_rec_slots); f(s.d_rec_cnt); f(s.d_rec);
            f(s.d_cnt_row); f(s.d_cnt_cursor);
        }
        void release_all() { each(*this, [](auto &b) { b.release(); }); }
        uint64_t bytes() const {
            uint64_t b = 0;
            each(*this, [&](const auto &buf) { b += buf.bytes(); });
            return b - d_cnt_row.bytes() - d_cnt_cursor.bytes();
        }
    } sc[4];
    bool staged = false;
    uint32_t last_set = 0;
    const BatchClass &last_cls() const { return cls[staged ? 0u : plan.back().cls]; }
    DevBuf<double> d_probs_dbg;
    DevBuf<uint16_t> d_counts_dbg;
    DevBuf<unsigned long long> d_sub_alloc;
    struct ResultSet {
        DevBuf<uint8_t> d_status;
        DevBuf<uint32_t> d_t_all, d_nrows_all, d_n_rows, d_flags, d_ndist;
        DevBuf<double> d_gs, d_z;
        DevBuf<unsigned long long> d_hq, d_row_start, d_cursor;
        DevBuf<DevRow> d_arena;
        uint64_t arena_cap = 0;
        uint64_t side_base = 0;
        PinBuf<unsigned long long> h_side_base;
        DevBuf<uint32_t> d_fin_t, d_fin_row_count, d_fin_lineage, d_fin_node, d_fin_depth;
        DevBuf<uint8_t> d_fin_status, d_fin_depth8, d_fin_hund;
        DevBuf<double> d_fin_gs, d_fin_local, d_fin_conf;
        DevBuf<unsigned long long> d_fin_row_begin, d_fin_cursor;
        uint64_t fin_cap = 0;
        DevBuf<uint32_t> d_perm, d_iperm;
        DevBuf<uint32_t> d_exact_grp;
        DevBuf<uint32_t> d_peak2, d_peak, d_sel_t, d_sel_row_count;
        DevBuf<uint8_t> d_strand, d_sel_status;
        DevBuf<double> d_sel_gs;
        DevBuf<unsigned long long> d_sel_row_begin;
        hipEvent_t ev_select = nullptr;
        DevBuf<uint32_t> d_nearest2, d_ties2, d_nearest, d_ties;
        bool has_nearest = false;
        DevBuf<uint32_t> d_dist, d_qlen;
        bool has_identity = false;
        uint64_t n_user = 0;
        bool has_peak = false;
        hipEvent_t ev_exact = nullptr;
        PinBuf<uint32_t> h_flags;
        hipEvent_t ev_flags = nullptr;
        std::vector<hipEvent_t> ev_sub;
        PinBuf<unsigned long long> h_cursor_sub, h_fin_sub;
        uint64_t n_q = 0;
        uint32_t n_sub = 0, n_side = 0;
        uint32_t in_set = 0;
        bool dev_exact = false;
        bool stream_dl = false;
        bool profiled = false;
        struct Bytes { uint64_t order, groups, rest; };
        Bytes bytes() const {
            return {(d_perm.n + d_iperm.n) * 4, d_exact_grp.n * 4,
                    d_status.n + (d_t_all.n + d_nrows_all.n + d_n_rows.n + d_ndist.n) * 4 + (d_gs.n + d_z.n + d_hq.n + d_row_start.n) * 8 + d_arena.n * sizeof(DevRow) +
                        (d_fin_t.n + d_fin_row_count.n + d_fin_lineage.n + d_fin_node.n + d_fin_depth.n) * 4 + d_fin_status.n + d_fin_depth8.n + d_fin_hund.n +
                        (d_fin_gs.n + d_fin_local.n + d_fin_conf.n + d_fin_row_begin.n) * 8};
        }
        void destroy_events() {
            for (auto e : ev_sub) (void)hipEventDestroy(e);
            if (ev_exact) (void)hipEventDestroy(ev_exact);
            if (ev_flags) (void)hipEventDestroy(ev_flags);
            if (ev_select) (void)hipEventDestroy(ev_select);
        }
    } rs[2];
    uint32_t rs_w = 0;
    ResultSet &res() { return rs[rs_w]; }
    std::vector<hipEvent_t> events;
    uint32_t n_sub_last = 0;
    std::vector<hipEvent_t> ev_near;
    uint32_t n_near_last = 0;
    hipEvent_t ev_ident[2] = {nullptr, nullptr};
    bool ident_timed = false;
    struct HostRes {
        PinBuf<uint32_t> v_row_lineage, v_row_node, v_row_depth;
        PinBuf<uint8_t> v_row_depth8, v_row_hund;
        PinBuf<uint32_t> h_t;
        PinBuf<uint8_t> h_status;
        PinBuf<double> v_row_conf, v_row_local;
        PinBuf<double> h_gs;
        PinBuf<unsigned long long> v_row_begin;
        PinBuf<uint32_t> v_row_count;
        PinBuf<uint8_t> h_strand;
        PinBuf<uint32_t> h_peak;
        PinBuf<uint32_t> h_nearest, h_ties;
        bool has_nearest = false;
        PinBuf<uint32_t> h_dist, h_qlen;
        bool has_identity = false;
        uint64_t n_user = 0;
        bool both = false;
    } host_res[2];
    uint32_t res_set = 0;
    PinBuf<uint32_t> h_nrows_all;
    bool text_on = false;
    uint32_t text_flags = 0;
    uint64_t text_tree_uid = 0;
    uint32_t device_text_opt = 0;
    uint32_t derep_opt = 0;
    rtx_qual_params quality{};
    bool quality_on = false;
    std::vector<rtx::TrimPrimer> primers;
    DevBuf<char> d_lin_bytes, d_text;
    DevBuf<uint64_t> d_lin_off;
    DevBuf<uint8_t> d_lin_depth, d_text_tmp;
    DevBuf<unsigned long long> d_text_len, d_text_off;
    struct HostText {
        PinBuf<char> out, tsv;
        PinBuf<uint64_t> out_off, tsv_off;
        uint64_t nq = 0;
        bool valid = false, tsv_on = false;
    } host_text[2];
    hipStream_t copy_stream = nullptr;
    PinBuf<unsigned long long> h_hq;
    uint32_t stage_timing = 0;

    uint32_t run_ahead_opt = 0;
    bool join_pending = false;
    hipEvent_t join_ev = nullptr;
    bool hold_join = false;
    hipEvent_t ev_set_free[3] = {nullptr, nullptr, nullptr};
    bool set_busy[3] = {false, false, false};
    uint64_t n_run_ahead = 0, n_run_ahead_retry = 0;

    struct Profile {
        bool on = false;
        uint32_t cutoff = 0, flags = 0;
        DevBuf<unsigned long long> d_acc;
        DevBuf<uint32_t> d_parent, d_ref_leaf;
        std::vector<uint64_t> h_acc;
        float ms = 0.f;
        uint32_t launches = 0;
        hipEvent_t ev[2] = {nullptr, nullptr};
    } prof;

    bool shared_device = false;
    ~rtx_index() {
        for (auto e : events) (void)hipEventDestroy(e);
        for (auto e : prof.ev)
            if (e) (void)hipEventDestroy(e);
        for (auto e : ev_near) (void)hipEventDestroy(e);
        for (auto e : ev_ident)
            if (e) (void)hipEventDestroy(e);
        for (auto &r : rs) r.destroy_events();
        for (auto e : ev_set_free)
            if (e) (void)hipEventDestroy(e);
        for (auto e : ev_front) (void)hipEventDestroy(e);
        for (auto e : ev_back) (void)hipEventDestroy(e);
        for (auto e : ev_mid) (void)hipEventDestroy(e);
        if (stream2) (void)hipStreamDestroy(stream2);
        if (stream3) (void)hipStreamDestroy(stream3);
        for (auto &i : in)
            if (i.ready) (void)hipEventDestroy(i.ready);
        if (ev_activated) (void)hipEventDestroy(ev_activated);
        if (h2d_stream) (void)hipStreamDestroy(h2d_stream);
        if (copy_stream) (void)hipStreamDestroy(copy_stream);
        if (stream) (void)hipStreamDestroy(stream);
    }
};

namespace rtxi {

int bind(rtx_index *ix);
int ensure_events(rtx_index *ix, size_t count);

struct SubBatch {
    uint32_t sb, nq, set;
    uint64_t q0;
    const rtx_index::BatchClass *cls;
    hipStream_t s;
    bool timed;
    bool timed_all;
};
SubBatch sub_batch_of(rtx_index *ix, uint32_t sb, bool timed);
uint8_t *counts_lo(rtx_index *ix, rtx_index::Scratch &sc);
uint16_t *counts_hi(rtx_index *ix, const rtx_index::BatchClass &k, rtx_index::Scratch &sc);
uint32_t counts_rows_layout(const rtx_index *ix, const rtx_index::BatchClass &k);
uint32_t diet_rows(const rtx_index *ix, uint32_t B);
int ensure_full_counts(rtx_index *ix, const rtx_index::BatchClass &k, rtx_index::Scratch &sc);
hipEvent_t stage_event(rtx_index *ix, const SubBatch &b, int stage, int which);
int enqueue_kmer(rtx_index *ix, const SubBatch &b, hipStream_t s);
int enqueue_hit(rtx_index *ix, const SubBatch &b, uint32_t flags, hipStream_t s, int part = 0, hipStream_t s_mid = nullptr);
int enqueue_count(rtx_index *ix, const SubBatch &b, uint32_t flags, hipStream_t s_mid = nullptr);
int enqueue_prob_prefix(rtx_index *ix, const SubBatch &b, bool fuse_walk, bool prob_only = false);
int enqueue_walk(rtx_index *ix, const SubBatch &b, const double *prefix, hipStream_t s);
int order_batch(rtx_index *ix, bool cluster);
void record_batch(rtx_index *ix);
int begin_run(rtx_index *ix, uint32_t *n_sub_out, bool *timed_out, bool cluster);
int enqueue_batch(rtx_index *ix, uint32_t flags);
int ensure_prob_tables(rtx_index *ix, uint32_t tmax, bool *usable);
uint32_t length_class(uint64_t len);
uint64_t class3_max_len();
int prepare_workspace(rtx_index *ix, uint64_t n_queries, const uint64_t cls_n[5], const uint64_t cls_max[5]);
int prepare_workspace_single(rtx_index *ix, uint64_t n_queries, uint64_t tmax, uint64_t max_len);
int plan_sub_batches(rtx_index *ix);
int alloc_scratch_set(rtx_index *ix, uint32_t k);
constexpr uint32_t kSideSet = 3;
int node_tables(rtx_index *ix);
int alloc_result_set(rtx_index *ix, rtx_index::ResultSet &r, uint64_t n_queries, uint64_t min_arena = 0);
int settle_join(rtx_index *ix);
int alloc_final(rtx_index *ix, rtx_index::ResultSet &r, uint64_t n_queries);
int enqueue_finalise(rtx_index *ix, const SubBatch &b, hipStream_t s);
int enqueue_profile(rtx_index *ix, rtx_index::ResultSet &r);
void set_derep_hash_mask(uint64_t mask);
int enqueue_text(rtx_index *ix, const rtx_index::ResultSet &r);


struct ItemList {
    size_t np, ntiles;
    ItemList(size_t nq, size_t tiles) : np((nq + 1u) / 2u), ntiles(tiles) {}
    size_t cap() const { return np * ntiles; }
    size_t end() const { return cap() + 9u; }
    uint32_t *items(uint32_t *p) const { return p; }
    uint32_t *count(uint32_t *p) const { return p + cap(); }
};
struct ItemsLayout : ItemList {
    using ItemList::ItemList;
    size_t total() const { return end() + 2u * np; }
    uint32_t *pair_live(uint32_t *p) const { return p + end(); }
    uint32_t *offsets(uint32_t *p) const { return p + end() + np; }
};
struct FineItemsLayout : ItemList {
    using ItemList::ItemList;
    size_t total() const { return end() + ntiles; }
    uint32_t *cursors(uint32_t *p) const { return p + end(); }
};
struct HeavyItemsLayout : ItemList {
    using ItemList::ItemList;
    size_t total() const { return end(); }
};
struct LiveLayout {
    uint32_t ntiles;
    uint32_t words() const { return (ntiles + 31u) / 32u + 1u; }
    size_t total(size_t B) const { return (B + 1u) * words(); }
};

inline size_t counts_elems(const rtx_index *ix, int planes, size_t rows) { return ix->packs(planes) ? rows * ix->npad * 5 / 8 : rows * ix->npad; }

struct ScratchNeed {
    size_t kmers = 0, rows = 0, dmask = 0, counts = 0, hist = 0 , prefix = 0, urec = 0;
    size_t prob_scratch = 0;
    size_t nsparse = 0, srows = 0, t = 0, nrows = 0, order = 0, tilemax = 0, nu = 0;
    size_t tile_ub = 0, best_key = 0, prune_thr = 0, prune_i1 = 0, best = 0, live = 0, items = 0;
    size_t heavy = 0, heavy_items = 0, fine_items = 0;
    size_t rec_nslots = 0, rec_slots = 0, rec_cnt = 0, rec = 0, cnt_row = 0, cnt_cursor = 0;
    ScratchNeed &set_queries(const rtx_index *ix, size_t B) {
        const size_t nt = ix->ntiles;
        t = nrows = order = best_key = prune_thr = prune_i1 = rec_nslots = cnt_row = B;
        nsparse = tilemax = tile_ub = B * nt;
        srows = B * nt * (kSegMaxSparseRows + 1);
        nu = (B + 1u) / 2u;
        best = B * kPruneBestWords;
        live = LiveLayout{ix->ntiles}.total(B);
        items = ItemsLayout(B, nt).total();
        heavy = B + 1u;
        heavy_items = HeavyItemsLayout(B, ix->u_ntiles).total();
        fine_items = FineItemsLayout(B, ix->f_ntiles).total();
        rec_slots = rec_cnt = B * kRecMaxSlots;
        rec = B * ix->rec_slots() * ix->rec_seg_len;
        cnt_cursor = 4;
        return *this;
    }
    void add_class(const rtx_index *ix, const rtx_index::BatchClass &kc, size_t B, size_t cnt_rows) {
        auto up = [](size_t &a, size_t v) { a = std::max(a, v); };
        up(kmers, B * kc.kstride);
        up(rows, B * kc.rstride);
        up(dmask, B * ix->ntiles * (kc.rstride / 64));
        up(counts, counts_elems(ix, kc.planes, cnt_rows));
        up(prefix, cnt_rows * ix->n_bnd_local);
        up(hist, B * kc.hstride);
        up(urec, ((B + 1u) / 2u) * 2u * kc.rstride);
        if (kc.huge) up(prob_scratch, B * ((prob_table_lds_bytes(kc.tmax) + 7) / 8));
    }
};

inline ScratchNeed scratch_set_need(const rtx_index *ix, uint32_t k) {
    ScratchNeed n;
    size_t b_max = 1;
    for (uint32_t c = 0; c < ix->n_cls; c++) {
        const rtx_index::BatchClass &kc = ix->cls[c];
        if (kc.side != (k == kSideSet)) continue;
        const size_t B = kc.sub_batch;
        b_max = std::max(b_max, B);
        const bool diet = kc.will_prune && ix->rec_opt != 0u && ix->n_refs == ix->n_total && ix->n_bnd_local == ix->n_bnd;
        n.add_class(ix, kc, B, diet ? diet_rows(ix, (uint32_t)B) : B);
    }
    return n.set_queries(ix, b_max);
}

inline uint64_t class_per_q(const rtx_index *ix, const rtx_index::BatchClass &k) {
    return (uint64_t)k.kstride * 2 + (uint64_t)k.rstride * 12 + 4 + (uint64_t)ix->ntiles * (k.rstride / 8 + ((kSegMaxSparseRows + 1) * 4 + 10)) + (ix->packs(k.planes) ? ix->npad * 5 / 4 : ix->npad * 2) +
           (uint64_t)k.hstride * 12 + (uint64_t)ix->n_bnd_local * 8 + 64 + (k.huge ? prob_table_lds_bytes(k.tmax) : 0) +
           (k.will_prune ? (uint64_t)ix->ntiles * 2 + 12 + (ix->ntiles + 31u) / 32u * 2u + 2u + kPruneBestWords * 4 +
                               ((uint64_t)ix->ntiles + 2u) * 2u   +
                               (ix->d_fbitmap.p ? (uint64_t)ix->f_ntiles * 2u + 1u : 0u)  +
                               (ix->rec_opt && ix->n_refs == ix->n_total ? (uint64_t)std::min<uint32_t>(ix->rec_opt, kRecMaxSlots) * 32768u + kRecMaxSlots * 6u + 2u : 0u)
                           : 0);
}

}
```

raxtax_amd/csrc/rtx_kernels.hip:

```cpp
#include <hip/hip_runtime.h>

#include "rtx_kernels.hpp"
#include "rtx_math.hpp"
#include "rtx_wave.hpp"
#include "rtx_hit_common.hpp"
#include "rtx_walk.hpp"

namespace rtx {

static constexpr uint32_t kEmptyRow = 0xFFFFFFFFu;

__global__ __launch_bounds__(256) void bitmap_build_kernel(const uint64_t *__restrict__ off,
                                                           const uint32_t *__restrict__ post,
                                                           const uint32_t *__restrict__ row_of,
                                                           uint32_t *__restrict__ bitmap, uint32_t stride_words, uint32_t n_rows1,
                                                           uint32_t ref_lo, uint32_t ref_hi, uint32_t shift) {
    const uint32_t k = blockIdx.x;
    const uint32_t row = row_of[k];
    if (row == kEmptyRow) return;
    const uint64_t b = off[k], e = off[k + 1];
    for (uint64_t i = b + threadIdx.x; i < e; i += blockDim.x) {
        const uint32_t g = post[i];
        if (g < ref_lo || g >= ref_hi) continue;
        uint32_t word, bit;
        ref_slot((g - ref_lo) >> shift, stride_words * 4u, word, bit);
        atomicOr(&bitmap[bitmap_word(row, word, n_rows1)], 1u << bit);
    }
}

__device__ __forceinline__ bool window_kmer(const uint8_t *__restrict__ seq, uint64_t w, uint32_t &k) {
    k = 0;
    bool ok = true;
#pragma unroll
    for (int j = 0; j < 8; j++) {
        const uint32_t c = seq[w + j];
        ok = ok && (c == 1u || c == 2u || c == 4u || c == 8u);
        k |= ((uint32_t)__ffs((int)c) - 1u) << (14 - 2 * j);
    }
    k &= 0xFFFFu;
    return ok;
}

__global__ __launch_bounds__(64) void ref_kmer_mark_kernel(const uint8_t *__restrict__ bases,
                                                           const uint64_t *__restrict__ off, uint64_t n_refs,
                                                           uint32_t *__restrict__ present ) {
    __shared__ uint32_t bm[2048];
    const uint32_t lane = threadIdx.x;
    for (uint32_t i = lane; i < 2048; i += 64) bm[i] = 0;
    __syncthreads();
    for (uint64_t r = blockIdx.x; r < n_refs; r += gridDim.x) {
        const uint64_t b0 = off[r], len = off[r + 1] - b0;
        for (uint64_t w = lane; w + 8 <= len; w += 64) {
            uint32_t k;
            if (window_kmer(bases + b0, w, k)) atomicOr(&bm[k >> 5], 1u << (k & 31u));
        }
    }
    __syncthreads();
    for (uint32_t i = lane; i < 2048; i += 64)
        if (bm[i]) atomicOr(&present[i], bm[i]);
}

__global__ __launch_bounds__(64) void ref_bitmap_set_kernel(const uint8_t *__restrict__ bases,
                                                            const uint64_t *__restrict__ off, uint64_t n_refs,
                                                            const uint32_t *__restrict__ row_of,
                                                            uint32_t *__restrict__ bitmap, uint32_t stride_words, uint32_t n_rows1,
                                                            uint32_t shift) {
    const uint64_t r = blockIdx.x;
    if (r >= n_refs) return;
    const uint32_t lane = threadIdx.x;
    const uint64_t b0 = off[r], len = off[r + 1] - b0;
    uint32_t word, bitpos;
    ref_slot((uint32_t)(r >> shift), stride_words * 4u, word, bitpos);
    const uint32_t bit = 1u << bitpos;
    for (uint64_t w = lane; w + 8 <= len; w += 64) {
        uint32_t k;
        if (window_kmer(bases + b0, w, k)) atomicOr(&bitmap[bitmap_word(row_of[k], word, n_rows1)], bit);
    }
}

__global__ __launch_bounds__(256) void row_popcount_kernel(const uint32_t *__restrict__ row_of,
                                                           const uint32_t *__restrict__ bitmap, uint32_t stride_words, uint32_t n_rows1,
                                                           uint32_t *__restrict__ list_len) {
    __shared__ uint32_t part[4];
    const uint32_t k = blockIdx.x;
    const uint32_t row = row_of[k];
    if (row == kEmptyRow) {
        if (threadIdx.x == 0) list_len[k] = 0;
        return;
    }
    uint32_t c = 0;
    for (uint32_t i = threadIdx.x; i < stride_words; i += 256) c += __popc(bitmap[bitmap_word(row, i, n_rows1)]);
#pragma unroll
    for (int d = 32; d >= 1; d >>= 1) c += __shfl_xor(c, d, 64);
    if ((threadIdx.x & 63u) == 0) part[threadIdx.x >> 6] = c;
    __syncthreads();
    if (threadIdx.x == 0) list_len[k] = part[0] + part[1] + part[2] + part[3];
}

__device__ __forceinline__ unsigned long long transpose64(unsigned long long x, uint32_t lane) {
#pragma unroll
    for (int s = 32; s >= 1; s >>= 1) {
        const unsigned long long m = s == 32 ? 0x00000000FFFFFFFFull : s == 16 ? 0x0000FFFF0000FFFFull : s == 8 ? 0x00FF00FF00FF00FFull
                                   : s == 4 ? 0x0F0F0F0F0F0F0F0Full : s == 2 ? 0x3333333333333333ull : 0x5555555555555555ull;
        const unsigned long long y = __shfl_xor(x, s, 64);
        x = (lane & (uint32_t)s) ? (((y >> s) & m) | (x & ~m)) : ((x & m) | ((y & m) << s));
    }
    return x;
}

template <bool kTilesOnly>
__global__ __launch_bounds__(64) void kmer_extract_kernel(KmerParams p) {
    const uint32_t mode = kTilesOnly ? 2u : p.mode;
    __shared__ __attribute__((aligned(16))) uint32_t bm[kTilesOnly ? 64 : 2048];
    const uint32_t q = blockIdx.x;
    const uint32_t lane = threadIdx.x;
    const uint64_t gq = p.q0 + q;
    const uint64_t qin = p.perm[gq];
    const uint64_t b0 = p.base_off[qin];
    const uint64_t len = p.base_off[qin + 1] - b0;
    const uint8_t *seq = p.bases + b0;

    uint32_t t = 0, nrows = 0;
    unsigned long long hq = 0;
    uint32_t *rout = p.rows + (size_t)q * p.rstride;
    const unsigned long long lt_mask = (1ull << lane) - 1ull;
    if (mode == 2u) {
        nrows = p.nrows[q];
    } else {
    for (uint32_t i = lane; i < 2048; i += 64) bm[i] = 0;
    {
        uint32_t *h = p.hist + (size_t)q * p.hstride;
        for (uint32_t i = lane; i < p.hstride; i += 64) h[i] = 0;
    }
    __syncthreads();

    if (len >= 8) {
        const uint64_t nwin = len - 7;
        const uint64_t wpl = (nwin + 63) / 64;
        const uint64_t w0 = (uint64_t)lane * wpl;
        const uint64_t w1 = w0 + wpl < nwin ? w0 + wpl : nwin;
        for (uint64_t i = w0; i < w1; i += 16) {
            unsigned long long v[3];
            __builtin_memcpy(v, seq + i, 24);
            const uint32_t nw = w1 - i < 16 ? (uint32_t)(w1 - i) : 16u;
            uint32_t k = 0, run = 0;
#pragma unroll
            for (int b = 0; b < 23; b++) {
                const uint32_t c = (uint32_t)(v[b >> 3] >> ((b & 7) * 8)) & 0xFFu;
                const bool ok = c == 1u || c == 2u || c == 4u || c == 8u;
                k = ((k << 2) | (((uint32_t)__ffs((int)c) - 1u) & 3u)) & 0xFFFFu;
                run = ok ? run + 1u : 0u;
                if (b >= 7 && (uint32_t)(b - 7) < nw && run >= 8u) atomicOr(&bm[k >> 5], 1u << (k & 31u));
            }
        }
    }
    __syncthreads();

    uint16_t *kout = p.kmers + (size_t)q * p.kstride;
    const unsigned long long *bm64 = reinterpret_cast<const unsigned long long *>(bm);
    uint32_t base = 0;
    for (uint32_t r = 0; r < 16; r++) {
        unsigned long long word = bm64[r * 64 + lane];
        const uint32_t cnt = (uint32_t)__popcll(word);
        const uint32_t incl = wave_incl_scan_u32(cnt);
        uint32_t pos = base + incl - cnt;
        const uint32_t kbase = (r * 64 + lane) * 64;
        while (word) {
            const uint32_t bit = (uint32_t)__builtin_ctzll(word);
            word &= word - 1;
            if (pos < p.kstride) kout[pos] = (uint16_t)(kbase + bit);
            pos++;
        }
        base += (uint32_t)__builtin_amdgcn_readlane((int)incl, 63);
    }
    t = base;
    __syncthreads();
    const bool all_kmers = t > 65535u;

    const uint32_t tt = all_kmers ? 0u : (t < p.kstride ? t : p.kstride);
    for (uint32_t i0 = 0; i0 < tt; i0 += 256) {
        uint32_t kk[4], row[4], ll[4];
#pragma unroll
        for (int u = 0; u < 4; u++) {
            const uint32_t i = i0 + u * 64 + lane;
            kk[u] = i < tt ? (uint32_t)kout[i] : 0xFFFFFFFFu;
        }
#pragma unroll
        for (int u = 0; u < 4; u++) {
            row[u] = kEmptyRow;
            ll[u] = 0;
            if (kk[u] != 0xFFFFFFFFu) {
                const uint2 rl = p.row_len[kk[u]];
                row[u] = rl.x;
                ll[u] = rl.y;
            }
        }
#pragma unroll
        for (int u = 0; u < 4; u++) {
            hq += ll[u];
            const unsigned long long m = __ballot(row[u] != kEmptyRow);
            if (row[u] != kEmptyRow) rout[nrows + __popcll(m & lt_mask)] = row[u];
            nrows += (uint32_t)__popcll(m);
        }
    }
    for (uint32_t i = nrows + lane; i < ((nrows + 63u) & ~63u); i += 64) rout[i] = p.zero_row;
    __syncthreads();
    }
    if (mode == 1u) {
#pragma unroll
        for (int d = 32; d >= 1; d >>= 1) hq += __shfl_xor(hq, d, 64);
        if (lane == 0) { p.t[q] = t > 65535u ? 0u : t; p.nrows[q] = nrows; p.hq[gq] = hq; p.t_all[gq] = t; }
        return;
    }
    const uint32_t nchunks = (nrows + 63u) >> 6;
    const uint32_t *live = mode == 2u ? p.live + (size_t)q * p.live_words : nullptr;
    const uint32_t nt = p.ntiles;
    const uint32_t mstride = p.rstride >> 6;
    unsigned long long *dm = p.dmask + (size_t)q * nt * mstride;
    uint32_t *sout = p.srows + (size_t)q * nt * (kSegMaxSparseRows + 1);
    uint32_t nseg = 0;
    __shared__ unsigned long long l_sb[64];
    __shared__ uint32_t l_base[64];
    bool few_done = false;
    if (live && p.seg_blocks) {
        const uint32_t lw = (nt + 31u) >> 5;
        uint32_t nlive = 0;
        for (uint32_t w = 0; w < lw; w++) nlive += (uint32_t)__popc(live[w]);
        if (nlive <= kKmerFewLive) {
            for (uint32_t w = 0; w < lw; w++) {
                uint32_t bits = (uint32_t)__builtin_amdgcn_readfirstlane((int)live[w]);
                while (bits) {
                    const uint32_t tile = w * 32u + (uint32_t)__builtin_ctz(bits);
                    bits &= bits - 1u;
                    if (tile >= nt) break;
                    uint32_t cd = 0, cs = 0;
                    for (uint32_t c0 = 0; c0 < nchunks; c0 += 4) {
                        uint32_t row[4], cls[4];
#pragma unroll
                        for (int u = 0; u < 4; u++) {
                            const uint32_t i = (c0 + (uint32_t)u) * 64 + lane;
                            row[u] = i < nrows ? rout[i] : kEmptyRow;
                        }
#pragma unroll
                        for (int u = 0; u < 4; u++) {
                            const uint32_t r = row[u] == kEmptyRow ? 0u : row[u];
                            cls[u] = (p.segcls[(size_t)tile * p.cls_stride + (r >> 4)] >> ((r & 15u) * 2u)) & 3u;
                            if (row[u] == kEmptyRow) cls[u] = 0u;
                        }
                        uint32_t srank[4], slot[4];
                        bool take[4];
#pragma unroll
                        for (int u = 0; u < 4; u++) {
                            const uint32_t c = c0 + (uint32_t)u;
                            take[u] = false;
                            srank[u] = 0u;
                            if (c >= nchunks) continue;
                            const bool sparse = cls[u] == 2u;
                            const unsigned long long ms = __ballot(sparse);
                            srank[u] = cs + (uint32_t)__popcll(ms & lt_mask);
                            take[u] = sparse && srank[u] < kSegMaxSparseRows;
                            const unsigned long long bt = __ballot(take[u]);
                            const unsigned long long md = __ballot(cls[u] == 1u || (sparse && !take[u]));
                            if (lane == 0) dm[(size_t)tile * mstride + c] = md;
                            cd += (uint32_t)__popcll(md);
                            cs += (uint32_t)__popcll(bt);
                        }
#pragma unroll
                        for (int u = 0; u < 4; u++) {
                            slot[u] = 0u;
                            if (take[u]) slot[u] = p.seginfo[(size_t)row[u] * p.seg_stride + tile] - 2u;
                        }
#pragma unroll
                        for (int u = 0; u < 4; u++)
                            if (take[u]) sout[(size_t)tile * (kSegMaxSparseRows + 1) + srank[u]] = slot[u];
                    }
                    if (lane == 0) {
                        p.nsparse[(size_t)q * nt + tile] = cs;
                        nseg += cd;
                    }
                }
            }
            few_done = true;
        }
    }
    for (uint32_t tb = 0; p.seg_blocks && !few_done && tb < nt; tb += 64) {
// ... 327 lines not shown
            for (uint32_t i0 = 0; i0 < i_lo; i0 += 64) {
                const uint32_t i = i0 + lane;
                const bool hit = i < i_lo && ln_pmf_tab(lf, t, n, m_lo, i, ln_total) >= kLnNegligibleP;
                const unsigned long long bal = __ballot(hit);
                if (bal) { i_s = i0 + (uint32_t)__ffsll((long long)bal) - 1u; break; }
            }
            const uint32_t h = act ? hist[m] : 0u;
            PmfState st{1.0, 1.0, 0};
            if (act) st = pmf_start_at(lf, t, n, m, i_s, ln_total);
            uint32_t bw = n + 1;
            double base = 1.0;
            double fbuf = 1.0;
            uint32_t f_lo = 0xFFFFFFFFu;
            auto flush = [&](uint32_t i_last) {
                if (!kGlobal || f_lo == 0xFFFFFFFFu) return;
                const uint32_t idx = (i_last & ~63u) + lane;
                if (idx >= f_lo && idx <= i_last) slots[wave * n1 + idx] *= fbuf;
                f_lo = 0xFFFFFFFFu;
            };
            for (uint32_t i = i_s; i <= n; i++) {
                bool sat = !act;
                if (i > i_s && act) {
                    const double c_old = st.c;
                    const int k_old = st.k;
                    if (kGlobal) pmf_step(st, InvDiv(), t, n, m, i);
                    else pmf_step(st, inv, t, n, m, i);
                    sat = st.c == c_old && k_old == 0 && st.k == 0;
                }
                if (i > i_s && __all(sat)) {
                    if (i > 0) flush(i - 1u);
                    base = wave_prod_f64_dpp(act ? pmf_cmf_pow(st, h) : 1.0);
                    bw = i;
                    break;
                }
                if (i >= i_lo) {
                    const double f = wave_prod_f64_dpp(act ? pmf_cmf_pow(st, h) : 1.0);
                    if (kGlobal) {
                        if (lane == (i & 63u)) fbuf = f;
                        if (f_lo == 0xFFFFFFFFu) f_lo = i;
                        if ((i & 63u) == 63u || i == n) flush(i);
                    } else if (lane == 0) {
                        slots[wave * n1 + i] *= f;
                    }
                }
            }
            if (lane == 0) { gbw[g] = bw; gbase[g] = base; gstart[g] = i_s; }
        }
        __syncthreads();
        for (uint32_t i = tid; i <= n; i += kProbThreads) {
            double P = 0.0;
            if (i >= i_lo) {
                P = slots[i];
#pragma unroll
                for (uint32_t w = 1; w < kProbWaves; w++) P *= slots[w * n1 + i];
                for (uint32_t g = 0; g < ngroups; g++) {
                    const uint32_t b = gbw[g];
                    if (b != kGroupSkipped && i >= b) P *= gbase[g];
                }
            }
            Pi[i] = P;
        }
        __syncthreads();
        for (uint32_t g = wave; g < ngroups; g += kProbWaves) {
            const uint32_t j = g * 64 + lane;
            if (!kGlobal && j >= D) continue;
            const bool valid = j < D;
            const uint32_t m_raw = valid ? ms[D - 1 - j] : 1u;
            if (valid && m_raw == 0) tz[0] = Pi[0];
            if (!kGlobal && m_raw == 0) continue;
            const uint32_t m = m_raw ? m_raw : 1u;
            const uint32_t b = gbw[g];
            if (b == kGroupSkipped) {
                if (valid && m_raw) tz[m] = 0.0;
                continue;
            }
            const uint32_t i_s = gstart[g];
            const uint32_t last = b == 0 ? 0u : (b - 1 < n ? b - 1 : n);
            PmfState st = pmf_start_at(lf, t, n, m, i_s, ln_total);
            double acc = 0.0;
            if (kGlobal) {
                double Pc = 0.0;
                const uint32_t i_first = i_s > i_lo ? i_s : i_lo;
                for (uint32_t i = i_s; i <= last; i++) {
                    if (i > i_s) pmf_step(st, InvDiv(), t, n, m, i);
                    if (i < i_lo) continue;
                    if ((i & 63u) == 0u || i == i_first) { const uint32_t idx = (i & ~63u) + lane; Pc = Pi[idx <= n ? idx : n]; }
                    const double P = __shfl(Pc, (int)(i & 63u), 64);
                    if (P > 0.0 && st.k == 0 && st.c > 0.0) acc += st.v * P / st.c;
                }
            } else {
                for (uint32_t i = i_s; i <= last; i++) {
                    if (i > i_s) pmf_step(st, inv, t, n, m, i);
                    if (i < i_lo) continue;
                    const double P = Pi[i];
                    if (P > 0.0 && st.k == 0 && st.c > 0.0) acc += st.v * P / st.c;
                }
            }
            if (!(valid && m_raw)) continue;
            tz[m] = acc;
        }
    }
    __syncthreads();
    double part = 0.0;
    for (uint32_t j = tid; j < D; j += kProbThreads) {
        const uint32_t m = ms[j];
        part += (double)hist[m] * tz[m];
    }
    part = wave_sum_f64(part);
    if (lane == 0) red[wave] = part;
    __syncthreads();
    double Z = red[0];
#pragma unroll
    for (uint32_t w = 1; w < kProbWaves; w++) Z += red[w];
    __syncthreads();
    const double inv_n = 1.0 / (double)p.n_refs;
    double gsum = 0.0;
    for (uint32_t j = tid; j < D; j += kProbThreads) {
        const uint32_t m = ms[j];
        const double v = tz[m] / Z;
        tz[m] = v;
        const double d = v - inv_n;
        gsum += (double)hist[m] * d * d;
    }
    gsum = wave_sum_f64(gsum);
    if (lane == 0) red[8 + wave] = gsum;
    __syncthreads();
    if (tid == 0) {
        p.z[gq] = Z;
        double gtot = red[8];
#pragma unroll
        for (uint32_t w = 1; w < kProbWaves; w++) gtot += red[8 + w];
        p.gs[gq] = sqrt(gtot);
        p.status[gq] = RTX_Q_OK;
    }
}

__global__ __launch_bounds__(64) void lineage_walk_kernel(WalkParams p) {
    __shared__ WalkLds L;
    lineage_walk_wave(p, blockIdx.x, threadIdx.x, L, GapPrefix{p.prefix + (size_t)blockIdx.x * p.n_bnd, nullptr});
}

__device__ __forceinline__ uint4 load_counts8(const uint16_t *p) {
    typedef uint32_t u32x4 __attribute__((ext_vector_type(4)));
    const u32x4 v = __builtin_nontemporal_load(reinterpret_cast<const u32x4 *>(p));
    return make_uint4(v.x, v.y, v.z, v.w);
}

static constexpr double kLiveEps = 1e-30;

template <int NW, bool TZ_LDS, bool PACKED>
__global__ __launch_bounds__(NW * 64) void taxon_prefix_kernel(PrefixParams p) {
    extern __shared__ double tz_lds[];
    __shared__ double wsum[2][NW];
    const uint32_t q = blockIdx.x, tid = threadIdx.x, lane = tid & 63u, wave = tid >> 6;
    const uint64_t gq = p.q0 + q;
    if (p.rec_nslots && p.rec_nslots[q] != 0u) return;
    if (p.status[gq] != RTX_Q_OK || (p.cnt_row && p.cnt_row[q] == 0xFFFFFFFFu)) {
        if (p.fuse_walk && tid == 0) { p.walk.n_rows[gq] = 0; p.walk.row_start[gq] = 0; }
        return;
    }
    const uint32_t crow = p.cnt_row ? p.cnt_row[q] : q;
    double *__restrict__ P = p.prefix + (size_t)crow * p.n_bnd;
    const double *__restrict__ tzg = p.table_z + (size_t)q * p.hstride;
    __shared__ uint32_t s_mlo, s_mlive;
    __shared__ PrefixGaps s_gaps;
    if (tid == 0) s_gaps.n = 0;
    {
        const uint32_t t1 = p.t[q] + 1;
        if (tid == 0) { s_mlo = 0xFFFFFFFFu; s_mlive = 0xFFFFFFFFu; }
        __syncthreads();
        uint32_t mine = 0xFFFFFFFFu, mine_live = 0xFFFFFFFFu;
        for (uint32_t m = tid; m < t1; m += NW * 64) {
            const double v = tzg[m];
            if (TZ_LDS) tz_lds[m] = v;
            if (v != 0.0 && m < mine) mine = m;
            if (v >= kLiveEps && m < mine_live) mine_live = m;
        }
        if (mine != 0xFFFFFFFFu) atomicMin(&s_mlo, mine);
        if (mine_live != 0xFFFFFFFFu) atomicMin(&s_mlive, mine_live);
        __syncthreads();
    }
    const uint32_t m_lo = (PACKED && TZ_LDS) ? s_mlo : 0u;
    const uint32_t ge_add = ((256u - (m_lo & 0xFFu)) & 0x7Fu) * 0x01010101u;
    const uint32_t ge_top = ((256u - (m_lo & 0xFFu)) & 0x80u) ? 0xFFFFFFFFu : 0u;
    const uint16_t *__restrict__ cnt = PACKED ? nullptr : p.counts + (size_t)crow * p.npad;
    const uint8_t *__restrict__ cnt_lo = PACKED ? p.counts_lo + (size_t)crow * p.npad : nullptr;
    const uint16_t *__restrict__ cnt_hi = PACKED ? p.counts_hi + (size_t)crow * (p.npad >> 3) : nullptr;
    if (tid == 0) P[0] = 0.0;
    double carry = 0.0;
    const uint32_t n = (uint32_t)p.n_refs;
    constexpr uint32_t kSweep = NW * 512;
    const uint32_t last_chunk = (n - 1u) >> 3;
    uint4 cv_l;
    uint32_t hi_l = 0, bits_l, rank_l;
    auto request = [&](uint32_t r) {
        const uint32_t ch = r >> 3 < last_chunk ? r >> 3 : last_chunk;
        if (PACKED) {
            typedef uint32_t u32x2 __attribute__((ext_vector_type(2)));
            const u32x2 v = __builtin_nontemporal_load(reinterpret_cast<const u32x2 *>(cnt_lo + (size_t)ch * 8u));
            cv_l = make_uint4(v.x, v.y, 0u, 0u);
            hi_l = __builtin_nontemporal_load(cnt_hi + ch);
        } else {
            cv_l = load_counts8(cnt + (size_t)ch * 8u);
        }
        bits_l = p.bnd_bits[ch];
        rank_l = p.bnd_rank[ch];
    };
    uint4 cv_next;
    uint32_t hi_next = 0, bits_next, rank_next;
    auto accept = [&](uint32_t r) {
        const bool in = r < n;
        cv_next = in ? cv_l : make_uint4(0, 0, 0, 0);
        hi_next = in ? hi_l : 0u;
        bits_next = in ? bits_l : 0u;
        rank_next = rank_l;
    };
    const uint16_t *__restrict__ tmx = p.tile_max ? p.tile_max + (size_t)q * p.ntiles : nullptr;
    const uint32_t u_thr = p.prune_thr ? p.prune_thr[q] : 0u;
    const uint32_t m_live = u_thr && s_mlive <= u_thr ? u_thr + 1u : s_mlive;
    if (p.prune_stats && u_thr && wave == 0 && tmx) {
        uint32_t need = 0;
        for (uint32_t T0 = 0; T0 < p.ntiles; T0 += 64) need += (uint32_t)__popcll(__ballot(T0 + lane < p.ntiles && (uint32_t)tmx[T0 + lane] > u_thr));
        if (lane < 2u) atomicAdd(&p.prune_stats[(size_t)(q & (kPruneStatCopies - 1u)) * 8u + lane], lane == 0u ? (unsigned long long)need : 1ull);
    }
    const uint32_t ntiles = (n + 8191u) >> 13;
    unsigned long long live_mask = ~0ull;
    uint32_t live_group = 0xFFFFFFFFu;
    auto tile_live = [&](uint32_t T) -> bool {
        if (!tmx) return true;
        if ((T >> 6) != live_group) {
            live_group = T >> 6;
            const uint32_t Tl = live_group * 64u + lane;
            live_mask = __ballot(Tl < ntiles && (uint32_t)tmx[Tl] >= m_live);
        }
        return (live_mask >> (T & 63u)) & 1ull;
    };
    uint32_t filled = 1;
    uint32_t n_gaps = 0;
    auto fill = [&](uint32_t a, uint32_t b) {
        if (a >= b) return;
        if (p.fuse_walk && n_gaps < kMaxPrefixGaps) {
            if (tid == 0) { s_gaps.lo[n_gaps] = a; s_gaps.hi[n_gaps] = b; s_gaps.val[n_gaps] = carry; s_gaps.n = n_gaps + 1u; }
            n_gaps++;
            return;
        }
        for (uint32_t i = a + tid; i < b; i += NW * 64) P[i] = carry;
    };
    uint32_t buf = 0;
    uint32_t T = 0;
    while (T < ntiles) {
        while (T < ntiles && !tile_live(T)) T++;
        if (T >= ntiles) break;
        const uint32_t Ts = T;
        while (T < ntiles && tile_live(T)) T++;
        const uint32_t Te = T;
        const uint32_t rb = p.bnd_rank[Ts * 1024u];
        fill(filled, rb);
        filled = Te * 1024u <= last_chunk ? p.bnd_rank[Te * 1024u] : p.n_bnd;
        const uint32_t span_end = Te * 8192u < n ? Te * 8192u : n;
        request(Ts * 8192u + tid * 8u);
        accept(Ts * 8192u + tid * 8u);
    for (uint32_t base = Ts * 8192u; base < span_end; base += kSweep, buf ^= 1u) {
        const uint32_t r0 = base + tid * 8u;
        const uint4 cv = cv_next;
        const uint32_t hi_cur = hi_next;
        const uint32_t bits_cur = bits_next, rank_cur = rank_next;
        request(r0 + kSweep);
        const uint32_t cw[4] = {cv.x, cv.y, cv.z, cv.w};
        bool live = true;
        if (PACKED && TZ_LDS && m_lo != 0u) {
            bool mine = hi_cur != 0u;
            if (m_lo < 256u) {
                const uint32_t tx = (cv.x & 0x7F7F7F7Fu) + ge_add, ty = (cv.y & 0x7F7F7F7Fu) + ge_add;
                const uint32_t gx = (cv.x & ge_top) | (cv.x & tx) | (ge_top & tx), gy = (cv.y & ge_top) | (cv.y & ty) | (ge_top & ty);
                mine = mine || (((gx | gy) & 0x80808080u) != 0u);
            }
            live = __ballot(mine) != 0ull;
        }
        double s[8];
        double run = 0.0, incl = 0.0;
        if (live) {
            double v[8];
            if (PACKED && __ballot(hi_cur != 0u) == 0ull) {
#pragma unroll
                for (int j = 0; j < 8; j++) {
                    const uint32_t c = (cw[j >> 2] >> ((j & 3) * 8)) & 0xFFu;
                    v[j] = TZ_LDS ? tz_lds[c] : tzg[c];
                }
            } else {
#pragma unroll
                for (int j = 0; j < 8; j++) {
                    uint32_t c;
                    if (PACKED) c = ((cw[j >> 2] >> ((j & 3) * 8)) & 0xFFu) | (((hi_cur >> (2 * j)) & 3u) << 8);
                    else c = (cw[j >> 1] >> ((j & 1) * 16)) & 0xFFFFu;
                    v[j] = TZ_LDS ? tz_lds[c] : tzg[c];
                }
            }
            if (base + kSweep > n) {
#pragma unroll
                for (int j = 0; j < 8; j++) v[j] = (r0 + j < n) ? v[j] : 0.0;
            }
            s[0] = v[0];
#pragma unroll
            for (int j = 1; j < 8; j++) s[j] = s[j - 1] + v[j];
            run = s[7];
            incl = wave_incl_scan_f64_dpp(run);
        } else {
#pragma unroll
            for (int j = 0; j < 8; j++) s[j] = 0.0;
        }
        if (lane == 63) wsum[buf][wave] = incl;
        __syncthreads();
        double off = carry + (incl - run);
        double tot = 0.0;
#pragma unroll
        for (int w = 0; w < NW; w++) {
            const double ws = wsum[buf][w];
            if ((uint32_t)w < wave) off += ws;
            tot += ws;
        }
        carry += tot;
        if (PACKED) asm volatile("" : "+v"(cv_l.x), "+v"(cv_l.y), "+v"(hi_l), "+v"(bits_l), "+v"(rank_l)::"memory");
        else asm volatile("" : "+v"(cv_l.x), "+v"(cv_l.y), "+v"(cv_l.z), "+v"(cv_l.w), "+v"(bits_l), "+v"(rank_l)::"memory");
        const uint32_t bits = bits_cur;
#pragma unroll
        for (int j = 0; j < 8; j++)
            if (bits & (1u << j)) P[rank_cur + (uint32_t)__popc(bits & ((1u << j) - 1u))] = off + s[j];
        accept(r0 + kSweep);
    }
    }
    fill(filled, p.n_bnd);
    if (p.fuse_walk) {
        __syncthreads();
        if (wave == 0) lineage_walk_wave(p.walk, q, lane, *reinterpret_cast<WalkLds *>(tz_lds), GapPrefix{P, &s_gaps});
    }
}

__global__ __launch_bounds__(256) void rehist_kernel(const uint16_t *__restrict__ counts, uint64_t npad, uint64_t n_refs,
                                                     const uint32_t *__restrict__ t, uint32_t *__restrict__ hist, uint32_t hstride,
                                                     uint16_t *__restrict__ tile_max, uint32_t ntiles) {
    extern __shared__ uint32_t h_lds[];
    uint32_t *tm_lds = h_lds + hstride;
    const uint32_t q = blockIdx.x, tid = threadIdx.x;
    const uint32_t tq = t[q];
    for (uint32_t m = tid; m <= tq; m += 256) h_lds[m] = 0;
    for (uint32_t i = tid; i < ntiles; i += 256) tm_lds[i] = 0;
    __syncthreads();
    const uint16_t *c = counts + (size_t)q * npad;
    for (uint64_t r0 = 0; r0 < n_refs; r0 += 8192) {
        const uint64_t r1 = r0 + 8192 < n_refs ? r0 + 8192 : n_refs;
        uint32_t mx = 0;
        for (uint64_t r = r0 + tid; r < r1; r += 256) {
            uint32_t v = c[r];
            v = v <= tq ? v : tq;
            atomicAdd(&h_lds[v], 1u);
            mx = v > mx ? v : mx;
        }
        if (mx) atomicMax(&tm_lds[r0 >> 13], mx);
    }
    __syncthreads();
    uint32_t *h = hist + (size_t)q * hstride;
    for (uint32_t m = tid; m <= tq; m += 256) h[m] = h_lds[m];
    if (tile_max)
        for (uint32_t i = tid; i < ntiles; i += 256) tile_max[(size_t)q * ntiles + i] = (uint16_t)tm_lds[i];
}

__global__ void counts_unpack_kernel(const uint8_t *lo, const uint16_t *hi, uint64_t n, uint16_t *out) {
    const uint64_t r = (uint64_t)blockIdx.x * blockDim.x + threadIdx.x;
    if (r < n) out[r] = (uint16_t)(lo[r] | (((hi[r >> 3] >> (2u * (r & 7u))) & 3u) << 8));
}

__global__ void probs_expand_kernel(const uint16_t *counts, const double *tz, uint64_t n, double *out) {
    const uint64_t r = (uint64_t)blockIdx.x * blockDim.x + threadIdx.x;
    if (r < n) out[r] = tz[counts[r]];
}

void launch_bitmap_build(hipStream_t s, const uint64_t *off, const uint32_t *post, const uint32_t *row_of,
                         uint32_t *bitmap, uint32_t stride_words, uint32_t n_rows1, uint32_t ref_lo, uint32_t ref_hi, uint32_t shift) {
    hipLaunchKernelGGL(bitmap_build_kernel, dim3(RTX_NUM_KMERS), dim3(256), 0, s, off, post, row_of, bitmap,
                       stride_words, n_rows1, ref_lo, ref_hi, shift);
}
void launch_ref_kmer_mark(hipStream_t s, const uint8_t *bases, const uint64_t *off, uint64_t n_refs, uint32_t *present) {
    hipLaunchKernelGGL(ref_kmer_mark_kernel, dim3(4096), dim3(64), 0, s, bases, off, n_refs, present);
}
void launch_ref_bitmap_set(hipStream_t s, const uint8_t *bases, const uint64_t *off, uint64_t n_refs,
                           const uint32_t *row_of, uint32_t *bitmap, uint32_t stride_words, uint32_t n_rows1, uint32_t shift) {
    hipLaunchKernelGGL(ref_bitmap_set_kernel, dim3((unsigned)n_refs), dim3(64), 0, s, bases, off, n_refs, row_of, bitmap,
                       stride_words, n_rows1, shift);
}
void launch_row_popcount(hipStream_t s, const uint32_t *row_of, const uint32_t *bitmap, uint32_t stride_words, uint32_t n_rows1,
                         uint32_t *list_len) {
    hipLaunchKernelGGL(row_popcount_kernel, dim3(RTX_NUM_KMERS), dim3(256), 0, s, row_of, bitmap, stride_words, n_rows1, list_len);
}
__global__ __launch_bounds__(256) void row_len_pack_kernel(const uint32_t *__restrict__ row_of, const uint32_t *__restrict__ list_len, uint2 *__restrict__ out) {
    const uint32_t k = blockIdx.x * 256u + threadIdx.x;
    out[k] = make_uint2(row_of[k], list_len[k]);
}
void launch_row_len_pack(hipStream_t s, const uint32_t *row_of, const uint32_t *list_len, uint2 *out) {
    hipLaunchKernelGGL(row_len_pack_kernel, dim3(RTX_NUM_KMERS / 256), dim3(256), 0, s, row_of, list_len, out);
}
void launch_kmer_extract(hipStream_t s, const KmerParams &p, uint32_t nq) {
    if (p.mode == 2u) hipLaunchKernelGGL(kmer_extract_kernel<true>, dim3(nq), dim3(64), 0, s, p);
    else hipLaunchKernelGGL(kmer_extract_kernel<false>, dim3(nq), dim3(64), 0, s, p);
}
constexpr uint32_t kHitLdsHistMax = 12288;
void launch_hit_count(hipStream_t s, const HitParams &p_in, uint32_t nq, uint32_t ntiles, int planes) {
    HitParams p = p_in;
    const bool ghist = p.hstride > kHitLdsHistMax;
    const uint32_t first = std::max<uint32_t>(ghist ? 0u : (p.hstride + 3u) & ~3u, kHitListCap + (RTX_HIT_NB > 2 ? 192u : 64u));
    p.lds_cnt8_off = first;
    const size_t lds = (size_t)first * sizeof(uint32_t) + 4096;
    if (ghist) hipLaunchKernelGGL((hit_count_kernel<16, false, true>), dim3(nq, ntiles), dim3(64), lds, s, p);
    else if (planes <= 10 && p.counts_lo) hipLaunchKernelGGL((hit_count_kernel<10, true>), dim3(nq, ntiles), dim3(64), lds, s, p);
    else if (planes <= 10) hipLaunchKernelGGL((hit_count_kernel<10, false>), dim3(nq, ntiles), dim3(64), lds, s, p);
    else if (planes <= 12) hipLaunchKernelGGL((hit_count_kernel<12, false>), dim3(nq, ntiles), dim3(64), lds, s, p);
    else hipLaunchKernelGGL((hit_count_kernel<16, false>), dim3(nq, ntiles), dim3(64), lds, s, p);
}
size_t prob_table_lds_bytes(uint32_t tmax) {
    const size_t n1max = tmax / 2 + 1;
    const size_t ngmax = (tmax + 64) / 64 + 1;
    return sizeof(double) * (2 * n1max + n1max + (tmax + n1max + 1) + 16 + ngmax) + sizeof(uint32_t) * (2 * ngmax + 2) +
           sizeof(uint16_t) * ((size_t)tmax + 2);
}
void launch_prob_table(hipStream_t s, const ProbParams &p, uint32_t nq) {
    if (p.gscratch) hipLaunchKernelGGL(prob_table_kernel<true>, dim3(nq), dim3(kProbThreads), 0, s, p);
    else hipLaunchKernelGGL(prob_table_kernel<false>, dim3(nq), dim3(kProbThreads), prob_table_lds_bytes(p.tmax), s, p);
}
template <int NW>
static void launch_taxon_prefix_nw(hipStream_t s, const PrefixParams &p, uint32_t nq, size_t lds) {
    if (p.tz_in_lds && p.packed) hipLaunchKernelGGL((taxon_prefix_kernel<NW, true, true>), dim3(nq), dim3(NW * 64), lds, s, p);
    else if (p.tz_in_lds) hipLaunchKernelGGL((taxon_prefix_kernel<NW, true, false>), dim3(nq), dim3(NW * 64), lds, s, p);
    else if (p.packed) hipLaunchKernelGGL((taxon_prefix_kernel<NW, false, true>), dim3(nq), dim3(NW * 64), lds, s, p);
    else hipLaunchKernelGGL((taxon_prefix_kernel<NW, false, false>), dim3(nq), dim3(NW * 64), lds, s, p);
}
void launch_taxon_prefix(hipStream_t s, const PrefixParams &p, uint32_t nq) {
    size_t lds = p.tz_in_lds ? (size_t)p.hstride * sizeof(double) : 0;
    if (p.fuse_walk) lds = std::max(lds, sizeof(WalkLds));
#ifndef RTX_PREFIX_NW
#define RTX_PREFIX_NW 2
#endif
#ifndef RTX_PREFIX_NW_PRUNED
#define RTX_PREFIX_NW_PRUNED 2
#endif
    if (p.prune_thr) launch_taxon_prefix_nw<RTX_PREFIX_NW_PRUNED>(s, p, nq, lds);
    else launch_taxon_prefix_nw<RTX_PREFIX_NW>(s, p, nq, lds);
}
void launch_lineage_walk(hipStream_t s, const WalkParams &p, uint32_t nq) {
    hipLaunchKernelGGL(lineage_walk_kernel, dim3(nq), dim3(64), 0, s, p);
}
void launch_rehist(hipStream_t s, const uint16_t *counts, uint64_t npad, uint64_t n_refs, const uint32_t *t, uint32_t *hist,
                   uint32_t hstride, uint16_t *tile_max, uint32_t ntiles, uint32_t nq) {
    hipLaunchKernelGGL(rehist_kernel, dim3(nq), dim3(256), ((size_t)hstride + ntiles) * 4, s, counts, npad, n_refs, t, hist, hstride,
                       tile_max, ntiles);
}
void launch_counts_unpack(hipStream_t s, const uint8_t *lo, const uint16_t *hi, uint64_t n, uint16_t *out) {
    hipLaunchKernelGGL(counts_unpack_kernel, dim3((unsigned)((n + 255) / 256)), dim3(256), 0, s, lo, hi, n, out);
}
void launch_probs_expand(hipStream_t s, const uint16_t *counts, const double *tz, uint64_t n, double *out) {
    hipLaunchKernelGGL(probs_expand_kernel, dim3((unsigned)((n + 255) / 256)), dim3(256), 0, s, counts, tz, n, out);
}

}
```

raxtax_amd/csrc/rtx_kernels.hpp:

```cpp
#pragma once

#include <hip/hip_runtime.h>

#include <cstdint>

#include "raxtax_hip.h"
#include "rtx_math.hpp"

namespace rtx {

#ifndef RTX_NODE_TYPES_DEFINED
#define RTX_NODE_TYPES_DEFINED
enum NodeType : uint8_t { kInner = 0, kTaxon = 1, kSequence = 2 };
#endif

constexpr uint32_t kWalkMaxRows = 208;
constexpr uint32_t kSegPad = 8192;
__host__ __device__ inline uint32_t seg_pad(uint32_t i) { return kSegPad + ((i & 63u) << 2); }
constexpr uint32_t kKmerFewLive = 8;
constexpr uint32_t kHitListCap = 1024;

struct DevRow {
    uint32_t node;
    uint8_t k[RTX_MAX_DEPTH];
// ... 23 lines not shown
    exact_range(x, qin, e0, e1, ids);
    return e1 - e0 == 1u ? ids[e0] : kTextNoOverride;
}
struct ExactParams {
    const uint8_t *bases;
    const uint64_t *base_off;
    uint32_t n_q;
    const uint2 *table;
    uint32_t bits;
    const uint64_t *rep_off;
    const uint8_t *rep_bytes;
    uint32_t *grp_out;
    uint64_t hash_mask;
};
void launch_exact_match(hipStream_t s, const ExactParams &p);
__device__ __forceinline__ uint64_t em_load_word(const uint8_t *seq, uint64_t len, uint64_t j) {
    uint64_t w;
    __builtin_memcpy(&w, seq + 8u * j, 8);
    const uint64_t rest = len - 8u * j;
    if (rest < 8u) w &= (1ull << (8u * rest)) - 1ull;
    return w;
}
void launch_unpack_nibbles(hipStream_t s, const uint8_t *packed, uint8_t *bases, uint64_t n_bases, uint64_t n_out);
bool pack_nibbles_mt(const uint8_t *in, uint64_t n, uint8_t *out, unsigned nt);

__host__ __device__ inline uint8_t complement_code(uint8_t b) {
    return b > 15u ? b : (uint8_t)(((b & 1u) << 3) | ((b & 2u) << 1) | ((b & 4u) >> 1) | ((b & 8u) >> 3));
}
void launch_revcomp(hipStream_t s, uint8_t *bases, uint64_t *base_off, uint32_t n, uint64_t total);
struct PeakParams {
    const uint32_t *hist;
    uint32_t hstride;
    const uint32_t *t;
    uint64_t q0;
    const uint32_t *perm;
    uint32_t nq;
    uint32_t *peak;
};
void launch_peak(hipStream_t s, const PeakParams &p);
struct StrandParams {
    uint32_t n;
    uint32_t both;
    const uint32_t *peak2;
    const uint8_t *status;
    const uint32_t *t;
    const double *gs;
    const unsigned long long *row_begin;
    const uint32_t *row_count;
    uint8_t *strand;
    uint32_t *peak;
    uint8_t *o_status;
    uint32_t *o_t;
    double *o_gs;
    unsigned long long *o_row_begin;
    uint32_t *o_row_count;
    const uint32_t *nearest2, *ties2;
    uint32_t *nearest, *ties;
};
void launch_strand_select(hipStream_t s, const StrandParams &p);

struct NearestParams {
    const uint32_t *hist;
    uint32_t hstride;
    const uint32_t *t;
    uint64_t q0;
    const uint32_t *perm;
    uint32_t nq;
    const uint16_t *tile_max;
    uint32_t ntiles;
    uint64_t n_refs;
    const uint16_t *counts;
    const uint8_t *counts_lo;
    const uint16_t *counts_hi;
    uint64_t npad;
    uint32_t cnt_rows;
    const uint32_t *cnt_row;
    const uint16_t *rec_nslots;
    const uint16_t *rec_slots;
    const uint32_t *rec_cnt, *rec;
    uint32_t rec_stride, rec_seg_len;
    uint32_t *nearest;
    uint32_t *ties;
};
void launch_nearest(hipStream_t s, const NearestParams &p);

struct ProfileParams {
    ProfileSrc src;
    uint64_t n_pos;
    uint32_t n_user;
    const uint32_t *perm;
    const uint8_t *strand;
    ExactRef exact;
    bool override_ok;
    uint32_t cutoff;
    uint32_t n_nodes;
    unsigned long long *clade, *direct, *conf_sum;
    unsigned long long *totals;
    const uint32_t *weight;
};
void launch_profile(hipStream_t s, const ProfileParams &p);

struct IdentityParams {
    uint32_t n;
    uint32_t max_len;
    const uint32_t *nearest;
    const uint8_t *strand;
    const uint8_t *qbytes;
    const uint64_t *qoff;
    bool packed;
    const uint32_t *ref_grp;
    const uint64_t *rep_off;
    const uint8_t *rep_bytes;
    uint32_t n_refs;
    uint32_t *dist;
    uint32_t *qlen;
};
void launch_identity(hipStream_t s, const IdentityParams &p);
void launch_ref_group(hipStream_t s, const uint32_t *goff, const uint32_t *gids, uint32_t n_groups, uint32_t n_refs, uint32_t *ref_grp);

struct KmerParams {
    const uint8_t *bases;
    const uint64_t *base_off;
    uint64_t q0;
    const uint32_t *perm;
    const uint32_t *row_of;
    const uint32_t *list_len;
    const uint2 *row_len;
    uint32_t zero_row;
    uint16_t *kmers;
    uint32_t kstride;
    const uint32_t *seginfo;
    uint32_t seg_stride;
    uint32_t ntiles;
    const unsigned long long *seg_dbits, *seg_sbits;
    const uint32_t *seg_sbase;
    uint32_t seg_blocks;
    const uint32_t *segcls;
    uint32_t cls_stride;
    uint32_t *rows;
    uint32_t rstride;
    unsigned long long *dmask;
    uint32_t *srows;
    uint32_t *nsparse;
    uint32_t *t;
    uint32_t *nrows;
    unsigned long long *hq;
    uint32_t *t_all;
    uint32_t *nrows_all;
    uint32_t *hist;
    uint32_t hstride;
    uint32_t mode;
    const uint32_t *live;
    uint32_t live_words;
};

constexpr uint32_t kRecMaxSlots = 16;
struct RecordRef {
    uint16_t *nslots;
    uint16_t *slots;
    uint32_t *cnt;
    uint32_t *rec;
    uint32_t stride;
    uint32_t seg_len;
    uint32_t *flags_out;
};

struct HitParams {
    const uint32_t *bitmap;
    uint32_t n_rows1;
    uint32_t stride_bytes;
    uint64_t n_refs;
    uint32_t ref_base;
    const uint32_t *rows;
    uint32_t rstride;
    const unsigned long long *dmask;
    const uint32_t *nrows;
    uint32_t zero_row;
    uint32_t lds_cnt8_off;
    const uint32_t *srows;
    const uint32_t *nsparse;
    const uint16_t *segslots;
    uint32_t ntiles;
    const uint32_t *t;
    uint16_t *counts;
    uint8_t *counts_lo;
    uint16_t *counts_hi;
    uint64_t npad;
    uint32_t *hist;
    uint32_t hstride;
    uint16_t *tile_max;
    uint32_t flags;
    uint64_t q0;
    const uint32_t *perm;
    ExactRef exact;
    uint32_t nq;
    uint32_t *group_rows;
    uint32_t group_base;
    const uint2 *pair_urec;
    const uint32_t *pair_nu;
    uint32_t pair_ustride;
    const uint32_t *live;
    uint32_t live_words;
    const uint16_t *prune_thr;
    const uint32_t *items;
    uint32_t *n_items;
    uint16_t *bounds_tile_ub;
    uint32_t bounds_tile_stride, bounds_ntiles;
    uint32_t *bounds_best;
    const uint8_t *bounds_heavy;
    uint64_t fine_n_refs;
    uint32_t fine_ref_ntiles;
    unsigned long long *fine_stats;
    RecordRef rec;
    const uint32_t *cnt_row;
};
struct Bounds2Params {
    const uint32_t *abitmap;
    const uint8_t *bbitmap;
    uint32_t n_rows1, n_atiles, ntiles, zero_row;
    const uint2 *pair_urec;
    const uint32_t *pair_nu;
    uint32_t pair_ustride, nq;
    const uint32_t *t;
    uint16_t *tile_ub;
    uint32_t tile_ub_stride;
    uint32_t *best_key;
    uint32_t delta_ct, delta_cm, delta_lo, delta_hi;
    uint8_t *heavy;
    uint32_t heavy_max;
    uint32_t *group_rows;
    uint32_t group_base;
};
struct HitParams;
void launch_bounds2(hipStream_t s, const Bounds2Params &p, uint32_t nq, int planes, const HitParams &hp, uint32_t u_ntiles, uint32_t *items);
constexpr uint32_t kTwoLevelMinTiles = 16;
void launch_bounds2_build(hipStream_t s, const uint32_t *ubitmap, uint32_t n_rows1, uint32_t u_ntiles, uint8_t *bbitmap, uint32_t *abitmap);
constexpr uint32_t kFineShift = 3;
constexpr uint32_t kFineMinLive = 4;
constexpr uint32_t kFineMinTiles = 16;

constexpr uint32_t kPruneStatCopies = 64;
#ifndef RTX_PRUNE_SHIFT
#define RTX_PRUNE_SHIFT 6
#endif
constexpr uint32_t kPruneShift = RTX_PRUNE_SHIFT;
static_assert(kPruneShift >= 3 && kPruneShift <= 6, "blocks of 8 .. 64 references");
constexpr uint32_t kPruneBestWords = 66;
struct PruneParams {
    const uint16_t *tile_ub;
    const uint32_t *best_key;
    uint32_t tile_ub_stride, ntiles, nq;
    uint64_t n_refs;
    uint64_t n_total;
    uint32_t ref_base;
    uint32_t phase;
    uint32_t *best;
    const uint2 *cbitmap;
    const uint32_t *bitmap;
    uint32_t n_rows1, stride_bytes;
    const uint32_t *rows;
    uint32_t rstride;
    const uint32_t *nrows, *t;
    uint32_t flags;
    uint64_t q0;
    const uint32_t *perm;
    ExactRef exact;
    const double *lnfact, *inv;
    uint32_t nlf;
    uint32_t *hist;
    uint32_t hstride;
    uint32_t *live;
    uint32_t live_words;
    uint32_t *pair_live;
    uint16_t *thr_out;
    uint16_t *i1_out;
    unsigned long long *stats;
    uint32_t *detail;
    RecordRef rec;
    uint32_t rec_max_slots;
    uint32_t *cnt_row;
    uint32_t *cnt_cursor;
    uint32_t cnt_cap;
    uint32_t *flags_out;
};
constexpr uint32_t kPruneDetailWords = 72;
struct ProbTables;
void launch_prune(hipStream_t s, const PruneParams &p, const ProbTables &tb, uint32_t nq);
void launch_block_major_build(hipStream_t s, const uint32_t *bitmap, uint32_t n_rows1, uint32_t ntiles, uint32_t stride_bytes, uint8_t *cbitmap);

struct ProbTables {
    double *cmf;
    double *ratio;
    const uint64_t *off;
    const uint32_t *moff;
    uint16_t *ilo;
    uint16_t *sat;
    uint32_t tmax;
};


struct ProbParams {
    const uint32_t *order;
    const uint32_t *t;
    const uint32_t *hist;
    uint32_t hstride;
    uint32_t tmax;
    uint32_t n1max;
    const double *lnfact;
    uint64_t n_refs;
    uint64_t q0;
    double *table_z;
    double *z;
    double *gs;
    uint8_t *status;
    uint32_t *ndist;
    const uint16_t *prune_thr;
    const uint16_t *prune_i1;
    double *gscratch;
    uint32_t gstride;
};

constexpr uint32_t kWalkSubAllocs = 128;
constexpr uint32_t kWalkSubStride = 16;
constexpr uint32_t kWalkSubMinQueries = 4096;
constexpr uint32_t kWalkChunkRows = 64;
struct WalkParams {
    const uint8_t *status;
    uint64_t q0;
    const double *prefix;
    uint32_t n_bnd;
    const uint4 *rec;
    DevRow *arena;
    unsigned long long arena_cap;
    unsigned long long *arena_cursor;
    unsigned long long *sub_alloc;
    uint32_t *n_rows;
    unsigned long long *row_start;
    uint32_t *flags_out;
};

struct FinaliseParams {
    const uint8_t *status;
    const uint32_t *t_all;
    const double *gs;
    const uint32_t *n_rows;
    const unsigned long long *row_start;
    const DevRow *arena;
    unsigned long long arena_cap;
    const uint32_t *perm;
    uint64_t q0;
    uint32_t nq;
    const uint8_t *node_depth, *node_sig0;
    const uint32_t *node_begin;
    const double *node_eb;
    uint32_t D;
    uint32_t *o_t;
    uint8_t *o_status;
    double *o_gs;
    unsigned long long *o_row_begin;
    uint32_t *o_row_count;
    uint32_t *r_lineage, *r_node, *r_depth;
    uint8_t *r_depth8, *r_hund;
    double *r_local, *r_conf;
    unsigned long long row_cap;
    unsigned long long *fin_cursor;
    uint32_t *flags_out;
};

constexpr int kBounds2MaxPlanes = 11;

struct PrefixParams {
    const uint8_t *status;
    const uint32_t *t;
    uint32_t tz_in_lds;
    uint64_t q0;
    const uint16_t *counts;
    const uint8_t *counts_lo;
    const uint16_t *counts_hi;
    uint32_t packed;
    uint64_t npad;
    const double *table_z;
    uint32_t hstride;
    uint64_t n_refs;
    const uint8_t *bnd_bits;
    const uint32_t *bnd_rank;
    double *prefix;
    uint32_t n_bnd;
    const uint16_t *tile_max;
    uint32_t ntiles;
    const uint16_t *prune_thr;
    unsigned long long *prune_stats;
    uint32_t fuse_walk;
    WalkParams walk;
    const uint16_t *rec_nslots;
    const uint32_t *cnt_row;
};


struct TailParams {
    RecordRef rec;
    const uint32_t *t;
    const double *table_z;
    uint32_t hstride;
    const uint8_t *bnd_bits;
    const uint32_t *bnd_rank;
    double *prefix;
    uint32_t *cnt_cursor;
    uint32_t cnt_cap;
    uint32_t *flags_out;
    uint32_t n_bnd;
    uint32_t nq;
    WalkParams walk;
    unsigned long long *prefix_stats;
    unsigned long long *stats;
};
void launch_records_tail(hipStream_t s, const TailParams &p, uint32_t nq);

void launch_bitmap_build(hipStream_t s, const uint64_t *off, const uint32_t *post, const uint32_t *row_of,
                         uint32_t *bitmap, uint32_t stride_words, uint32_t n_rows1, uint32_t ref_lo, uint32_t ref_hi, uint32_t shift = 0);
void launch_ref_kmer_mark(hipStream_t s, const uint8_t *bases, const uint64_t *off, uint64_t n_refs, uint32_t *present);
void launch_ref_bitmap_set(hipStream_t s, const uint8_t *bases, const uint64_t *off, uint64_t n_refs,
                           const uint32_t *row_of, uint32_t *bitmap, uint32_t stride_words, uint32_t n_rows1, uint32_t shift = 0);
void launch_row_len_pack(hipStream_t s, const uint32_t *row_of, const uint32_t *list_len, uint2 *out);
void launch_row_popcount(hipStream_t s, const uint32_t *row_of, const uint32_t *bitmap, uint32_t stride_words, uint32_t n_rows1,
                         uint32_t *list_len);
void launch_kmer_extract(hipStream_t s, const KmerParams &p, uint32_t nq);
void launch_hit_count(hipStream_t s, const HitParams &p, uint32_t nq, uint32_t ntiles, int planes);
void launch_pair_union(hipStream_t s, const uint32_t *rows, const uint32_t *nrows, uint32_t rstride, uint32_t nq, uint2 *urec,
                       uint32_t *nu, uint32_t ustride);
void launch_hit_count_pair(hipStream_t s, const HitParams &p, uint32_t nq, uint32_t ntiles, int planes);
void launch_live_items(hipStream_t s, const uint32_t *live, uint32_t live_words, const uint32_t *pair_live, uint32_t nq, uint32_t ntiles, uint32_t *off,
                       uint32_t *items, uint32_t *n_items);
void launch_hit_count_pair_bounds(hipStream_t s, const HitParams &p, uint32_t nq, uint32_t u_ntiles, int planes);
void launch_hit_count_pair_bounds_items(hipStream_t s, const HitParams &p, uint32_t nq, uint32_t u_ntiles, int planes);
void launch_fine_bounds(hipStream_t s, const HitParams &p, uint32_t nq, uint32_t ntiles, uint32_t f_ntiles, uint32_t *pair_live, uint32_t *cnt,
                        uint32_t *items, uint32_t *n_items, int planes);
size_t prob_table_lds_bytes(uint32_t tmax);
void launch_prob_table(hipStream_t s, const ProbParams &p, uint32_t nq);
size_t prob_lookup_lds_bytes(uint32_t tmax);
void launch_prob_tables_build(hipStream_t s, const ProbTables &tb, const double *lf, const double *inv);
void launch_prob_order(hipStream_t s, const uint32_t *t, uint32_t nq, uint32_t *order);
void launch_prob_lookup(hipStream_t s, const ProbParams &p, const ProbTables &tb, uint32_t nq);
void launch_seg_popcount(hipStream_t s, const uint32_t *bitmap, uint32_t stride_bytes, uint32_t n_rows1, uint32_t ntiles, uint16_t *pop);
void launch_seg_emit(hipStream_t s, const uint32_t *bitmap, uint32_t stride_bytes, uint32_t n_rows1, uint32_t ntiles,
                     const uint32_t *seginfo, uint32_t seg_stride, uint16_t *slots);
void launch_sketch(hipStream_t s, const uint8_t *bases, const uint64_t *off, uint32_t n_q, uint64_t *keys, uint32_t *idx);
void launch_invert_perm(hipStream_t s, const uint32_t *perm, uint32_t n, uint32_t *inv);
constexpr uint32_t kLocTableEntries = 1u << 24;
void launch_loc_mark(hipStream_t s, const uint8_t *bases, const uint64_t *off, uint64_t n_refs, uint32_t *pos_min, uint32_t *cnt);
void launch_loc_finish(hipStream_t s, uint32_t *pos_min, const uint32_t *cnt);
void launch_locator(hipStream_t s, const uint8_t *bases, const uint64_t *off, uint32_t n_q, const uint32_t *table, uint64_t n_refs,
                    uint64_t *keys);
void launch_identity_perm(hipStream_t s, uint32_t n, uint32_t *perm, uint32_t *inv);
int cluster_sort(hipStream_t s, void *tmp, size_t *tmp_bytes, const uint64_t *keys_in, uint64_t *keys_out, const uint32_t *idx_in,
                 uint32_t *perm_out, size_t n, bool with_class = false);
void launch_class_keys(hipStream_t s, uint64_t *keys, const uint64_t *off, uint32_t n, const uint64_t lim[4], bool from_index, uint32_t *idx);
void launch_taxon_prefix(hipStream_t s, const PrefixParams &p, uint32_t nq);
void launch_lineage_walk(hipStream_t s, const WalkParams &p, uint32_t nq);
void launch_finalise(hipStream_t s, const FinaliseParams &p);
void launch_probs_expand(hipStream_t s, const uint16_t *counts, const double *tz, uint64_t n, double *out);
void launch_rehist(hipStream_t s, const uint16_t *counts, uint64_t npad, uint64_t n_refs, const uint32_t *t, uint32_t *hist,
                   uint32_t hstride, uint16_t *tile_max, uint32_t ntiles, uint32_t nq);
void launch_counts_unpack(hipStream_t s, const uint8_t *lo, const uint16_t *hi, uint64_t n, uint16_t *out);

}
```

raxtax_amd/csrc/rtx_prune.hip:

```cpp
#include <hip/hip_runtime.h>

#include "rtx_kernels.hpp"
#include "rtx_math.hpp"
#include "rtx_wave.hpp"

namespace rtx {

static constexpr double kPruneLnEps = kPruneLnEpsHD;
static constexpr double kPruneHalfEps = kPruneHalfEpsHD;
#ifndef RTX_PRUNE_WAVES
#define RTX_PRUNE_WAVES 4
#endif
#ifndef RTX_PRUNE_TURNS
#define RTX_PRUNE_TURNS 16
#endif
static constexpr uint32_t kPruneWavesPerBlock = 4;

__device__ __forceinline__ uint32_t wave_max_u32p(uint32_t v) { return wave_max_u32(v); }

__global__ __launch_bounds__(64 * kPruneWavesPerBlock, RTX_PRUNE_WAVES) void prune_kernel(PruneParams p, ProbTables tb) {
    extern __shared__ double prune_lds[];
    for (uint32_t i = threadIdx.x; i < p.nlf; i += 64u * kPruneWavesPerBlock) prune_lds[i] = p.lnfact[i];
    __syncthreads();
    const uint32_t lane = threadIdx.x & 63u, pair = blockIdx.x * kPruneWavesPerBlock + (threadIdx.x >> 6);
// ... 241 lines not shown
                                    const uint32_t b = ub_lds[x * p.ntiles + T];
                                    gub = b > gub ? b : gub;
                                    const uint64_t lo = (uint64_t)T * 8192u, hi = lo + 8192u < p.n_refs ? lo + 8192u : p.n_refs;
                                    gnd += (double)(hi - lo);
                                }
                            }
                        }
                        const double kept = tile_aware ? wave_sum_f64_dpp(gub > u_max ? gnd : 0.0) : (double)p.n_total;
                        const double ln_kept = log(kept > 1.0 ? kept : 1.0);
                        const uint32_t iw = i1 + lane;
                        const bool tail_pt = lane == 63u;
                        const bool vi = iw <= n;
                        double lnG = 0.0;
                        unsigned long long hb = __ballot(hm != 0u);
                        const uint32_t iwc = vi ? iw : n;
                        while (hb) {
                            double v[4];
#pragma unroll
                            for (int k = 0; k < 4; k++) {
                                v[k] = 0.0;
                                if (hb) {
                                    const int h = __builtin_ctzll(hb);
                                    hb &= hb - 1ull;
                                    const uint32_t m = (uint32_t)__builtin_amdgcn_readlane((int)hm, h);
                                    v[k] = Ct[(size_t)m * (n + 1) + iwc];
                                }
                            }
#pragma unroll
                            for (int k = 0; k < 4; k++) lnG += v[k];
                        }
                        const double gw = vi && !tail_pt ? exp(lnG) : 0.0;
                        const double ww = vi && !tail_pt ? exp(fmin(0.0, ln_kept + lnG)) : 0.0;
                        const double incl = wave_incl_scan_f64_dpp(ww);
                        const double a_tot = readlane_f64(incl, 63);
                        const double len_tail = vi ? (double)(n - iw + 1u) : 0.0;
                        const double WA = tail_pt ? len_tail * (a_tot + 1.0) : (vi ? incl - ww : 0.0);
                        const double WB = tail_pt ? len_tail : gw;
                        const double nn = (double)p.n_total;
                        const bool has_tail = i1 + 63u <= n;
                        auto sums_at = [&](uint32_t m, double &a, double &b) {
                            const double P = vi && m != 0u ? exp(ln_pmf_tab(lf, t, n, m, iw, ln_total)) : 0.0;
                            a = wave_sum_f64_dpp(P * WA);
                            b = wave_sum_f64_dpp(P * WB);
                        };
                        double gsa = 0.0, gsb = 0.0, far_a = 0.0, far_b = 0.0, n_far = 0.0, mid_a = 0.0, mid_b = 0.0, n_mid = 0.0;
                        bool near = false;
                        if (tile_aware) {
                            const uint32_t m_far = u_max > kPruneFarGap ? u_max - kPruneFarGap : 0u;
                            near = gnd > 0.0 && gub > u_max;
                            const bool mid = gnd > 0.0 && gub > m_far && gub <= u_max;
                            unsigned long long nb = __ballot(near);
                            if ((uint32_t)__popcll(nb) > kPruneMaxNear) {
                                near = gnd > 0.0;
                                const uint32_t gcap = gub < h_min ? gub : h_min - 1u;
                                prune_window_sums(lf, p.inv, t, n, gcap, i1, ln_total, [&](uint32_t l) { return readlane_f64(WA, (int)l); },
                                                  [&](uint32_t l) { return readlane_f64(WB, (int)l); }, gsa, gsb);
                            } else {
                                n_far = wave_sum_f64_dpp(near || mid ? 0.0 : gnd);
                                n_mid = wave_sum_f64_dpp(mid ? gnd : 0.0);
                                if (m_far) sums_at(m_far, far_a, far_b);
                                if (n_mid > 0.0) sums_at(u_max, mid_a, mid_b);
                                while (nb) {
                                    const int g = __builtin_ctzll(nb);
                                    nb &= nb - 1ull;
                                    const uint32_t m = (uint32_t)__builtin_amdgcn_readlane((int)gub, g);
                                    double a, b;
                                    sums_at(m < h_min ? m : h_min - 1u, a, b);
                                    if ((int)lane == g) { gsa = a; gsb = b; }
                                }
                            }
                        }
                        auto crit = [&](uint32_t u) -> bool {
                            bool falling = true;
                            if (has_tail) {
                                const uint32_t j = i1 + 63u;
                                falling = (double)(u + j) * (double)(n - j) < (double)(j + 1u) * (double)(t - u + n - j - 1u);
                            }
                            double a, b;
                            sums_at(u, a, b);
                            if (!tile_aware) return falling && nn * a <= kPruneHalfEps && nn * b <= kPruneHalfEps;
                            const bool dead = gub <= u;
                            return falling && wave_sum_f64_dpp(near ? gnd * (dead ? gsa : a) : 0.0) + n_far * far_a + n_mid * mid_a <= kPruneHalfEps &&
                                   wave_sum_f64_dpp(near ? gnd * (dead ? gsb : b) : 0.0) + n_far * far_b + n_mid * mid_b <= kPruneHalfEps;
                        };
                        uint32_t lo = u_max, hi = h_min - 1u;
                        while (lo < hi) {
                            const uint32_t mid = (lo + hi + 1u) >> 1;
                            if (crit(mid)) lo = mid; else hi = mid - 1u;
                        }
                        u_max = lo;
                    }
                }
            }
        }
        thr[x] = u_max;
        if (lane == 0) { p.thr_out[q] = (uint16_t)u_max; p.i1_out[q] = (uint16_t)(u_max ? i1_q : 0u); }
        if (p.detail && lane == 0) {
            uint32_t *d = p.detail + (size_t)q * kPruneDetailWords;
            d[0] = bb; d[1] = M; d[2] = u_max; d[3] = u_max ? i1_q : 0u; d[4] = ub_best; d[5] = t; d[6] = 0u; d[7] = 0u;
        }
        st[2] += M; st[3] += u_max; st[4] += ub_best; st[5] += 1ull;
        if (ub_best < M) st[6] += 1ull;
    }
    if (p.phase == 1u) return;
    __builtin_amdgcn_fence(__ATOMIC_ACQ_REL, "wavefront");
    __builtin_amdgcn_wave_barrier();
    unsigned long long dead_refs[2] = {0, 0};
    uint32_t n_live = 0, n_qlive = 0;
    uint32_t n_rec[2] = {0u, 0u};
    for (uint32_t T0 = 0; T0 < p.ntiles; T0 += 64) {
        const uint32_t T = T0 + lane;
        bool la = false, lb = false;
        if (T < p.ntiles) {
            la = thr[0] == 0u || (uint32_t)ub_lds[T] > thr[0];
            lb = has_b && (thr[1] == 0u || (uint32_t)ub_lds[p.ntiles + T] > thr[1]);
        }
        const unsigned long long ba = __ballot(la), bb2 = __ballot(lb);
        if (lane == 0) {
            uint32_t *wa = p.live + (size_t)(pair * 2u) * p.live_words, *wb = wa + p.live_words;
            wa[T0 >> 5] = (uint32_t)ba;
            if ((T0 >> 5) + 1u < p.live_words) wa[(T0 >> 5) + 1u] = (uint32_t)(ba >> 32);
            if (has_b) {
                wb[T0 >> 5] = (uint32_t)bb2;
                if ((T0 >> 5) + 1u < p.live_words) wb[(T0 >> 5) + 1u] = (uint32_t)(bb2 >> 32);
            }
        }
        if (T < p.ntiles) {
            const uint64_t lo = (uint64_t)T * 8192u, hi = lo + 8192u < p.n_refs ? lo + 8192u : p.n_refs;
            if (!la) dead_refs[0] += hi - lo;
            if (!lb) dead_refs[1] += hi - lo;
        }
        if (p.rec.nslots) {
            const unsigned long long lt = (1ull << lane) - 1ull;
            const uint32_t ka = n_rec[0] + (uint32_t)__popcll(ba & lt), kb = n_rec[1] + (uint32_t)__popcll(bb2 & lt);
            if (la && ka < kRecMaxSlots) p.rec.slots[(size_t)(pair * 2u) * kRecMaxSlots + ka] = (uint16_t)T;
            if (lb && kb < kRecMaxSlots) p.rec.slots[(size_t)(pair * 2u + 1u) * kRecMaxSlots + kb] = (uint16_t)T;
            n_rec[0] += (uint32_t)__popcll(ba);
            n_rec[1] += (uint32_t)__popcll(bb2);
        }
        n_live += (uint32_t)__popcll(ba | bb2);
        n_qlive += (uint32_t)__popcll(ba) + (uint32_t)__popcll(bb2);
    }
    if (p.rec.nslots) {
        const uint32_t cap = p.rec_max_slots < kRecMaxSlots ? p.rec_max_slots : kRecMaxSlots;
        const bool ra = thr[0] != 0u && n_rec[0] != 0u && n_rec[0] <= cap, rb = has_b && thr[1] != 0u && n_rec[1] != 0u && n_rec[1] <= cap;
        if (lane < kRecMaxSlots) {
            p.rec.cnt[(size_t)(pair * 2u) * kRecMaxSlots + lane] = 0u;
            if (has_b) p.rec.cnt[(size_t)(pair * 2u + 1u) * kRecMaxSlots + lane] = 0u;
        }
        if (lane == 0) {
            p.rec.nslots[pair * 2u] = (uint16_t)(ra ? n_rec[0] : 0u);
            if (has_b) p.rec.nslots[pair * 2u + 1u] = (uint16_t)(rb ? n_rec[1] : 0u);
            if (p.cnt_row) {
                auto row_for = [&](bool records) -> uint32_t {
                    if (records) return 0xFFFFFFFFu;
                    const uint32_t r = atomicAdd(p.cnt_cursor, 1u);
                    if (r < p.cnt_cap) return r;
                    atomicOr(p.flags_out, 4u);
                    return 0xFFFFFFFFu;
                };
                p.cnt_row[pair * 2u] = row_for(ra);
                if (has_b) p.cnt_row[pair * 2u + 1u] = row_for(rb);
            }
        }
    }
#pragma unroll
    for (int d = 32; d >= 1; d >>= 1) { dead_refs[0] += __shfl_xor(dead_refs[0], d, 64); dead_refs[1] += __shfl_xor(dead_refs[1], d, 64); }
    if (lane == 0) {
        p.hist[(size_t)(pair * 2u) * p.hstride] = (uint32_t)dead_refs[0];
        if (has_b) p.hist[(size_t)(pair * 2u + 1u) * p.hstride] = (uint32_t)dead_refs[1];
    }
    if (lane == 0 && p.pair_live) p.pair_live[pair] = n_live;
    st[7] = n_qlive;
    if (p.stats) {
        st[0] = n_live; st[1] = 1ull;
        unsigned long long mine = 0;
#pragma unroll
        for (int k = 0; k < 8; k++) mine = lane == (uint32_t)k ? st[k] : mine;
        if (lane < 8u && mine) atomicAdd(&p.stats[(size_t)(pair & (kPruneStatCopies - 1u)) * 8u + lane], mine);
    }
}

__global__ __launch_bounds__(256) void block_major_build_kernel(const uint32_t *__restrict__ bitmap, uint32_t n_rows1, uint32_t stride_bytes,
                                                                uint8_t *__restrict__ cbitmap) {
    const uint32_t row = blockIdx.x, tile = blockIdx.y, word = threadIdx.x;
    const uint32_t v = bitmap[((size_t)tile * n_rows1 + row) * 256u + word];
    if (v == 0u) return;
    const uint32_t l = word >> 2, wi = word & 3u, L = tile_lanes(stride_bytes, tile);
    if (l >= L) return;
#pragma unroll
    for (uint32_t k = 0; k < 4u; k++) {
        const uint32_t byte = (v >> (8u * k)) & 0xFFu;
        if (byte == 0u) continue;
        const uint32_t ref0 = tile * 8192u + ((wi * 4u + k) * L + l) * 8u;
        cbitmap[((size_t)(ref0 >> 6) * n_rows1 + row) * 8u + ((ref0 & 63u) >> 3)] = (uint8_t)byte;
    }
}
void launch_block_major_build(hipStream_t s, const uint32_t *bitmap, uint32_t n_rows1, uint32_t ntiles, uint32_t stride_bytes, uint8_t *cbitmap) {
    hipLaunchKernelGGL(block_major_build_kernel, dim3(n_rows1, ntiles), dim3(256), 0, s, bitmap, n_rows1, stride_bytes, cbitmap);
}

void launch_prune(hipStream_t s, const PruneParams &p, const ProbTables &tb, uint32_t nq) {
    const uint32_t pairs = (nq + 1u) / 2u;
    hipLaunchKernelGGL(prune_kernel, dim3((pairs + kPruneWavesPerBlock - 1u) / kPruneWavesPerBlock), dim3(64 * kPruneWavesPerBlock),
                       (size_t)p.nlf * sizeof(double) + (size_t)kPruneWavesPerBlock * 2 * p.ntiles * sizeof(uint16_t), s, p, tb);
}

}
```

Measured before the change: 13.02 million.

## Cut small launches and memsets from the prune pipeline and densify prefix grid

After: 13.16 million, median of 6. 1.01x the previous value.

```diff
diff --git a/raxtax_amd/csrc/rtx_api_batch.hip b/raxtax_amd/csrc/rtx_api_batch.hip
--- a/raxtax_amd/csrc/rtx_api_batch.hip
+++ b/raxtax_amd/csrc/rtx_api_batch.hip
@@ -117,6 +117,14 @@
 int enqueue_kmer(rtx_index *ix, const SubBatch &b, hipStream_t s) {
     KmerParams kp = kmer_params(ix, b);
     kp.mode = run_prunes(ix, *b.cls) && ix->seg_blocks ? 1u : 0u;
+    if (run_prunes(ix, *b.cls)) {
+        rtx_index::Scratch &sc = ix->sc[b.set];
+        const ItemsLayout items(b.nq, ix->ntiles);
+        const FineItemsLayout fine(b.nq, ix->f_ntiles);
+        if (sc.d_items.p) { kp.zero[0] = items.count(sc.d_items.p); kp.zero_n[0] = 9u; }
+        if (sc.d_fine_items.p) { kp.zero[1] = fine.count(sc.d_fine_items.p); kp.zero_n[1] = 9u + ix->f_ntiles; }
+        if (sc.d_cnt_cursor.p) { kp.zero[2] = sc.d_cnt_cursor.p; kp.zero_n[2] = 1u; }
+    }
     if (b.timed_all) RTX_HIP(hipEventRecord(stage_event(ix, b, RTX_STAGE_KMER_EXTRACT, 0), s));
     launch_kmer_extract(s, kp, b.nq);
     if (b.timed_all) RTX_HIP(hipEventRecord(stage_event(ix, b, RTX_STAGE_KMER_EXTRACT, 1), s));
@@ -314,10 +322,10 @@
         if (records) { pr.rec = rr; pr.rec_max_slots = rr.stride; }
         if (k.diet && !diet) { set_error("internal: the counts buffer is on its diet without the records path"); return RTX_ERR_STATE; }
         if (diet) {
-            RTX_HIP(hipMemsetAsync(sc.d_cnt_cursor.p, 0, 4, s));
             pr.cnt_row = sc.d_cnt_row.p;
             pr.cnt_cursor = sc.d_cnt_cursor.p;
             pr.cnt_cap = k.cnt_rows;
+            pr.dense_q = sc.d_dense_q.p;
             pr.flags_out = r.d_flags.p;
             hp.cnt_row = sc.d_cnt_row.p;
         }
@@ -326,7 +334,7 @@
         if (part == 0 && ix->fine_opt && ix->d_fbitmap.p && k.pair && sc.d_fine_items.p) {
             const FineItemsLayout fine(b.nq, ix->f_ntiles);
             uint32_t *const fi = sc.d_fine_items.p;
-            launch_fine_bounds(s, fine_params(ix, sc, hp), b.nq, ix->ntiles, ix->f_ntiles, pr.pair_live, fine.cursors(fi), fine.items(fi), fine.count(fi), k.planes);
+            launch_fine_bounds(s, fine_params(ix, sc, hp), b.nq, ix->f_ntiles, pr.pair_live, fine.cursors(fi), fine.items(fi), fine.count(fi), k.planes);
         }
         RTX_HIP(hipMemsetAsync(sc.d_tilemax.p, 0, (size_t)b.nq * ix->ntiles * 2, s));
         hp.live = sc.d_live.p;
@@ -335,7 +343,8 @@
         if (records) hp.rec = rr;
         if (k.pair) {
             const ItemsLayout items(b.nq, ix->ntiles);
-            launch_live_items(s, sc.d_live.p, pr.live_words, pr.pair_live, b.nq, ix->ntiles, items.offsets(sc.d_items.p), items.items(sc.d_items.p), items.count(sc.d_items.p));
+            launch_live_items(s, sc.d_live.p, pr.live_words, b.nq, ix->ntiles, items.items(sc.d_items.p), items.count(sc.d_items.p),
+                              ix->d_prune_stats.p ? ix->d_prune_stats.p + 2 * kPruneStatCopies * 8 : nullptr);
             hp.items = items.items(sc.d_items.p);
             hp.n_items = items.count(sc.d_items.p);
         }
@@ -428,6 +437,12 @@
     const bool records = fuse_walk && on_records_path(ix, k, sc);
     fp.rec_nslots = records ? sc.d_rec_nslots.p : nullptr;
     fp.cnt_row = fuse_walk && on_diet(ix, k, sc) ? sc.d_cnt_row.p : nullptr;
+    if (fp.cnt_row) {
+        fp.dense_q = sc.d_dense_q.p;
+        fp.cnt_cursor = sc.d_cnt_cursor.p;
+        fp.cnt_cap = k.cnt_rows;
+        fp.nq = b.nq;
+    }
     if (fuse_walk) {
         fp.walk = walk_params(ix, b, sc.d_prefix.p);
         int rc_r = fp.walk.sub_alloc ? reset_sub_alloc(ix, s) : RTX_OK;
@@ -683,7 +698,7 @@
         k.prune = ix->pruning() && k.pair && k.use_tables && ix->tile_skip && ix->d_ubitmap.p && (whole || shard) &&
                   scratch_ok(s0, k.sub_batch) && (!ix->staged || scratch_ok(ix->sc[1], k.sub_batch));
         k.rec = k.prune && whole && ix->rec_opt != 0u && ix->n_bnd_local == ix->n_bnd && s0.d_rec.p != nullptr && s0.d_rec.n >= need.rec;
-        auto diet_ok = [&](const rtx_index::Scratch &sc) { return sc.d_rec.p != nullptr && sc.d_cnt_row.p != nullptr && sc.d_cnt_cursor.p != nullptr && sc.d_cnt_row.n >= need.cnt_row; };
+        auto diet_ok = [&](const rtx_index::Scratch &sc) { return sc.d_rec.p != nullptr && sc.d_cnt_row.p != nullptr && sc.d_cnt_cursor.p != nullptr && sc.d_dense_q.p != nullptr && sc.d_cnt_row.n >= need.cnt_row; };
         k.diet = k.rec && diet_rows(ix, k.sub_batch) < k.sub_batch && diet_ok(s0);
         if (k.diet && !k.side)
             for (uint32_t j = 1; j <= 2u; j++)
@@ -693,10 +708,12 @@
             need.add_class(ix, k, k.sub_batch, k.cnt_rows);
             for (uint32_t j = 0; j < 4u; j++) {
                 rtx_index::Scratch &sc = ix->sc[j];
-                if ((j == kSideSet) != k.side || sc.d_kmers.p == nullptr || (sc.d_counts.n >= need.counts && sc.d_prefix.n >= need.prefix)) continue;
+                const bool list_ok = !k.diet || sc.d_dense_q.n >= need.dense_q;
+                if ((j == kSideSet) != k.side || sc.d_kmers.p == nullptr || (sc.d_counts.n >= need.counts && sc.d_prefix.n >= need.prefix && list_ok)) continue;
                 RTX_HIP(hipStreamSynchronize(ix->stream));
                 int rc_c = sc.d_counts.alloc(need.counts);
                 if (!rc_c) rc_c = sc.d_prefix.alloc(need.prefix);
+                if (!rc_c && !list_ok) rc_c = sc.d_dense_q.alloc(need.dense_q);
                 if (rc_c) return rc_c;
             }
         }
@@ -1171,7 +1188,7 @@
         if (ix->d_fbitmap.p && sc.d_fine_items.alloc(n.fine_items)) sc.d_fine_items.release();
         if (ix->rec_opt && ix->n_refs == ix->n_total) {
             if (sc.d_rec_nslots.alloc(n.rec_nslots) || sc.d_rec_slots.alloc(n.rec_slots) || sc.d_rec_cnt.alloc(n.rec_cnt) ||
-                sc.d_rec.alloc(n.rec) || sc.d_cnt_row.alloc(n.cnt_row) || sc.d_cnt_cursor.alloc(n.cnt_cursor))
+                sc.d_rec.alloc(n.rec) || sc.d_cnt_row.alloc(n.cnt_row) || sc.d_cnt_cursor.alloc(n.cnt_cursor) || sc.d_dense_q.alloc(n.dense_q))
                 sc.d_rec.release();
         }
     }
diff --git a/raxtax_amd/csrc/rtx_hit_pair.hip b/raxtax_amd/csrc/rtx_hit_pair.hip
--- a/raxtax_amd/csrc/rtx_hit_pair.hip
+++ b/raxtax_amd/csrc/rtx_hit_pair.hip
@@ -306,42 +306,9 @@
     pair_tile_block<NP, kPacked, kBounds>(p, lds_dw, pair, blockIdx.y, lane);
 }
 
-__global__ __launch_bounds__(1024) void live_offsets_kernel(const uint32_t *__restrict__ pair_live, uint32_t np, uint32_t *__restrict__ off,
-                                                            uint32_t *__restrict__ n_items) {
-    __shared__ uint32_t wsum[2][16];
-    const uint32_t tid = threadIdx.x, lane = tid & 63u, wave = tid >> 6;
-    constexpr uint32_t kPer = 8;
-    uint32_t carry = 0, buf = 0;
-    for (uint32_t base = 0; base < np; base += 1024u * kPer, buf ^= 1u) {
-        const uint32_t i0 = base + tid * kPer;
-        uint32_t c[kPer], cnt = 0;
-#pragma unroll
-        for (uint32_t j = 0; j < kPer; j++) c[j] = i0 + j < np ? pair_live[i0 + j] : 0u;
-#pragma unroll
-        for (uint32_t j = 0; j < kPer; j++) cnt += c[j];
-        const uint32_t incl = wave_incl_scan_u32(cnt);
-        if (lane == 63u) wsum[buf][wave] = incl;
-        __syncthreads();
-        uint32_t o = carry + incl - cnt, tot = 0;
-#pragma unroll
-        for (uint32_t w = 0; w < 16u; w++) {
-            const uint32_t sw = wsum[buf][w];
-            o += w < wave ? sw : 0u;
-            tot += sw;
-        }
-#pragma unroll
-        for (uint32_t j = 0; j < kPer; j++) {
-            if (i0 + j < np) off[i0 + j] = o;
-            o += c[j];
-        }
-        carry += tot;
-    }
-    if (tid == 0u) n_items[0] = carry;
-    if (tid < 8u) n_items[1u + tid] = 0;
-}
-
 __global__ __launch_bounds__(1024) void live_items_kernel(const uint32_t *__restrict__ live, uint32_t live_words, uint32_t nq, uint32_t ntiles,
-                                                          const uint32_t *__restrict__ off, uint32_t *__restrict__ items) {
+                                                          uint32_t *__restrict__ items, uint32_t *__restrict__ n_items,
+                                                          unsigned long long *__restrict__ stats) {
     extern __shared__ uint32_t tl[];
     const uint32_t tid = threadIdx.x, lane = tid & 63u;
     const uint32_t np = (nq + 1u) / 2u, g0 = blockIdx.x * 1024u, pair = g0 + tid;
@@ -368,10 +335,14 @@
             if (T0 + lane < ntiles) tl[T0 + lane] = running + incl - v;
             running += (uint32_t)__builtin_amdgcn_readlane((int)incl, 63);
         }
+        if (lane == 0u) {
+            tl[ntiles] = running ? atomicAdd(&n_items[0], running) : 0u;
+            if (stats && running) atomicAdd(&stats[(size_t)(blockIdx.x & (kPruneStatCopies - 1u)) * 8u + 2u], (unsigned long long)running);
+        }
     }
     __syncthreads();
     if (!valid) return;
-    const uint32_t base = off[g0];
+    const uint32_t base = tl[ntiles];
     for (uint32_t w = 0; w < nw; w++) {
         uint32_t bits = wa[w] | (hb ? wa[live_words + w] : 0u);
         while (bits) {
@@ -411,11 +382,10 @@
     else launch_hit_count_pair_np<11>(s, p, nq, ntiles);
 }
 
-void launch_live_items(hipStream_t s, const uint32_t *live, uint32_t live_words, const uint32_t *pair_live, uint32_t nq, uint32_t ntiles, uint32_t *off,
-                       uint32_t *items, uint32_t *n_items) {
+void launch_live_items(hipStream_t s, const uint32_t *live, uint32_t live_words, uint32_t nq, uint32_t ntiles, uint32_t *items, uint32_t *n_items,
+                       unsigned long long *stats) {
     const uint32_t np = (nq + 1u) / 2u;
-    hipLaunchKernelGGL(live_offsets_kernel, dim3(1), dim3(1024), 0, s, pair_live, np, off, n_items);
-    hipLaunchKernelGGL(live_items_kernel, dim3((np + 1023u) / 1024u), dim3(1024), (size_t)ntiles * 4, s, live, live_words, nq, ntiles, off, items);
+    hipLaunchKernelGGL(live_items_kernel, dim3((np + 1023u) / 1024u), dim3(1024), ((size_t)ntiles + 1u) * 4, s, live, live_words, nq, ntiles, items, n_items, stats);
 }
 
 void launch_hit_count_pair_bounds(hipStream_t s, const HitParams &p, uint32_t nq, uint32_t u_ntiles, int planes) {
@@ -440,23 +410,29 @@
     return m;
 }
 __global__ __launch_bounds__(256) void fine_count_kernel(const uint32_t *__restrict__ live, uint32_t live_words, const uint32_t *__restrict__ pair_live,
-                                                         uint32_t nq, uint32_t f_ntiles, uint32_t *__restrict__ cnt) {
+                                                         uint32_t nq, uint32_t f_ntiles, uint32_t *__restrict__ cnt, uint32_t *__restrict__ n_items) {
     const uint32_t pair = blockIdx.x * 256u + threadIdx.x, np = (nq + 1u) / 2u, lane = threadIdx.x & 63u;
     const bool on = pair < np && pair_live[pair < np ? pair : 0u] >= kFineMinLive;
     for (uint32_t U = 0; U < f_ntiles; U++) {
         const unsigned long long b = __ballot(on && fine_pair_mask(live, live_words, pair, nq, U) != 0u);
         if (b && lane == (uint32_t)__builtin_ctzll(b)) atomicAdd(&cnt[U], (uint32_t)__popcll(b));
     }
-}
-__global__ void fine_scan_kernel(uint32_t *__restrict__ cnt, uint32_t f_ntiles, uint32_t *__restrict__ n_items) {
+    __shared__ uint32_t s_last;
+    __threadfence();
+    __syncthreads();
+    if (threadIdx.x == 0u) s_last = atomicAdd(&n_items[0], 1u) == gridDim.x - 1u ? 1u : 0u;
+    __syncthreads();
+    if (s_last == 0u || threadIdx.x >= 64u) return;
+    __threadfence();
     uint32_t run = 0;
-    for (uint32_t U = 0; U < f_ntiles; U++) {
-        const uint32_t c = cnt[U];
-        cnt[U] = run;
-        run += c;
-    }
-    n_items[0] = run;
-    for (uint32_t x = 1; x <= 8u; x++) n_items[x] = 0;
+    for (uint32_t U0 = 0; U0 < f_ntiles; U0 += 64) {
+        const uint32_t U = U0 + lane;
+        const uint32_t c = U < f_ntiles ? __hip_atomic_load(&cnt[U], __ATOMIC_RELAXED, __HIP_MEMORY_SCOPE_AGENT) : 0u;
+        const uint32_t incl = wave_incl_scan_u32(c);
+        if (U < f_ntiles) cnt[U] = run + incl - c;
+        run += (uint32_t)__builtin_amdgcn_readlane((int)incl, 63);
+    }
+    if (lane == 0u) n_items[0] = run;
 }
 __global__ __launch_bounds__(256) void fine_scatter_kernel(const uint32_t *__restrict__ live, uint32_t live_words, const uint32_t *__restrict__ pair_live,
                                                            uint32_t nq, uint32_t f_ntiles, uint32_t *__restrict__ cursor, uint32_t *__restrict__ items) {
@@ -473,37 +449,21 @@
         if (has) items[base + (uint32_t)__popcll(b & ((1ull << lane) - 1ull))] = pair * f_ntiles + U;
     }
 }
-__global__ __launch_bounds__(256) void pair_live_recount_kernel(const uint32_t *__restrict__ live, uint32_t live_words, uint32_t nq, uint32_t ntiles,
-                                                                uint32_t *__restrict__ pair_live, unsigned long long *__restrict__ stats) {
-    const uint32_t pair = blockIdx.x * 256u + threadIdx.x, np = (nq + 1u) / 2u;
-    uint32_t n = 0;
-    if (pair < np) {
-        const uint32_t *wa = live + (size_t)(pair * 2u) * live_words;
-        const bool hb = pair * 2u + 1u < nq;
-        for (uint32_t w = 0; w < (ntiles + 31u) >> 5; w++) n += (uint32_t)__popc(wa[w] | (hb ? wa[live_words + w] : 0u));
-        pair_live[pair] = n;
-    }
-    if (stats) {
-        n = wave_incl_scan_u32(n);
-        if ((threadIdx.x & 63u) == 63u && n) atomicAdd(&stats[(size_t)(blockIdx.x & (kPruneStatCopies - 1u)) * 8u + 2u], (unsigned long long)n);
-    }
-}
-
-void launch_fine_bounds(hipStream_t s, const HitParams &p, uint32_t nq, uint32_t ntiles, uint32_t f_ntiles, uint32_t *pair_live, uint32_t *cnt,
+#ifndef RTX_FINE_GRID_CAP
+#define RTX_FINE_GRID_CAP 4096
+#endif
+void launch_fine_bounds(hipStream_t s, const HitParams &p, uint32_t nq, uint32_t f_ntiles, const uint32_t *pair_live, uint32_t *cnt,
                         uint32_t *items, uint32_t *n_items, int planes) {
     const uint32_t np = (nq + 1u) / 2u, nb = (np + 255u) / 256u;
-    (void)hipMemsetAsync(cnt, 0, (size_t)f_ntiles * 4, s);
-    hipLaunchKernelGGL(fine_count_kernel, dim3(nb), dim3(256), 0, s, p.live, p.live_words, pair_live, nq, f_ntiles, cnt);
-    hipLaunchKernelGGL(fine_scan_kernel, dim3(1), dim3(1), 0, s, cnt, f_ntiles, n_items);
+    hipLaunchKernelGGL(fine_count_kernel, dim3(nb), dim3(256), 0, s, p.live, p.live_words, pair_live, nq, f_ntiles, cnt, n_items);
     hipLaunchKernelGGL(fine_scatter_kernel, dim3(nb), dim3(256), 0, s, p.live, p.live_words, pair_live, nq, f_ntiles, cnt, items);
     HitParams fp = p;
     fp.items = items;
     fp.n_items = n_items;
-    const dim3 grid((uint32_t)((std::min<uint64_t>((uint64_t)np * f_ntiles, std::max<uint64_t>((uint64_t)RTX_ITEM_GRID_HALVES * np / 2u, 2048ull)) + 7u) & ~7ull));
+    const dim3 grid((uint32_t)((std::min<uint64_t>((uint64_t)np * f_ntiles, (uint64_t)RTX_FINE_GRID_CAP) + 7u) & ~7ull));
     if (planes <= 8) hipLaunchKernelGGL((hit_count_pair_kernel<8, true, 2, true>), grid, dim3(64), kPairLdsBytes, s, fp);
     else if (planes <= 10) hipLaunchKernelGGL((hit_count_pair_kernel<10, true, 2, true>), grid, dim3(64), kPairLdsBytes, s, fp);
     else hipLaunchKernelGGL((hit_count_pair_kernel<11, false, 2, true>), grid, dim3(64), kPairLdsBytes, s, fp);
-    hipLaunchKernelGGL(pair_live_recount_kernel, dim3(nb), dim3(256), 0, s, p.live, p.live_words, nq, ntiles, pair_live, p.fine_stats);
-}
-
-}
+}
+
+}
diff --git a/raxtax_amd/csrc/rtx_index.hpp b/raxtax_amd/csrc/rtx_index.hpp
--- a/raxtax_amd/csrc/rtx_index.hpp
+++ b/raxtax_amd/csrc/rtx_index.hpp
@@ -282,12 +282,13 @@
         DevBuf<uint16_t> d_rec_nslots, d_rec_slots;
         DevBuf<uint32_t> d_rec_cnt, d_rec;
         DevBuf<uint32_t> d_cnt_row, d_cnt_cursor;
+        DevBuf<uint32_t> d_dense_q;
         template <class S, class F>
         static void each(S &s, F &&f) {
             f(s.d_kmers); f(s.d_counts); f(s.d_tilemax); f(s.d_rows); f(s.d_t); f(s.d_nrows); f(s.d_hist); f(s.d_order); f(s.d_srows); f(s.d_nsparse);
             f(s.d_dmask); f(s.d_table_z); f(s.d_prefix); f(s.d_urec); f(s.d_nu); f(s.d_live); f(s.d_best_key); f(s.d_items); f(s.d_tile_ub); f(s.d_prune_thr);
             f(s.d_prune_i1); f(s.d_best); f(s.d_heavy); f(s.d_heavy_items); f(s.d_fine_items); f(s.d_rec_nslots); f(s.d_rec_slots); f(s.d_rec_cnt); f(s.d_rec);
-            f(s.d_cnt_row); f(s.d_cnt_cursor);
+            f(s.d_cnt_row); f(s.d_cnt_cursor); f(s.d_dense_q);
         }
         void release_all() { each(*this, [](auto &b) { b.release(); }); }
         uint64_t bytes() const {
@@ -505,9 +506,8 @@
 };
 struct ItemsLayout : ItemList {
     using ItemList::ItemList;
-    size_t total() const { return end() + 2u * np; }
+    size_t total() const { return end() + np; }
     uint32_t *pair_live(uint32_t *p) const { return p + end(); }
-    uint32_t *offsets(uint32_t *p) const { return p + end() + np; }
 };
 struct FineItemsLayout : ItemList {
     using ItemList::ItemList;
@@ -533,6 +533,7 @@
     size_t tile_ub = 0, best_key = 0, prune_thr = 0, prune_i1 = 0, best = 0, live = 0, items = 0;
     size_t heavy = 0, heavy_items = 0, fine_items = 0;
     size_t rec_nslots = 0, rec_slots = 0, rec_cnt = 0, rec = 0, cnt_row = 0, cnt_cursor = 0;
+    size_t dense_q = 0;
     ScratchNeed &set_queries(const rtx_index *ix, size_t B) {
         const size_t nt = ix->ntiles;
         t = nrows = order = best_key = prune_thr = prune_i1 = rec_nslots = cnt_row = B;
@@ -557,6 +558,7 @@
         up(dmask, B * ix->ntiles * (kc.rstride / 64));
         up(counts, counts_elems(ix, kc.planes, cnt_rows));
         up(prefix, cnt_rows * ix->n_bnd_local);
+        up(dense_q, cnt_rows);
         up(hist, B * kc.hstride);
         up(urec, ((B + 1u) / 2u) * 2u * kc.rstride);
         if (kc.huge) up(prob_scratch, B * ((prob_table_lds_bytes(kc.tmax) + 7) / 8));
diff --git a/raxtax_amd/csrc/rtx_kernels.hip b/raxtax_amd/csrc/rtx_kernels.hip
--- a/raxtax_amd/csrc/rtx_kernels.hip
+++ b/raxtax_amd/csrc/rtx_kernels.hip
@@ -131,6 +131,11 @@
     {
         uint32_t *h = p.hist + (size_t)q * p.hstride;
         for (uint32_t i = lane; i < p.hstride; i += 64) h[i] = 0;
+    }
+    if (q == 0u) {
+#pragma unroll
+        for (int k = 0; k < 3; k++)
+            for (uint32_t i = lane; i < p.zero_n[k]; i += 64) p.zero[k][i] = 0;
     }
     __syncthreads();
 
@@ -764,7 +769,16 @@
 __global__ __launch_bounds__(NW * 64) void taxon_prefix_kernel(PrefixParams p) {
     extern __shared__ double tz_lds[];
     __shared__ double wsum[2][NW];
-    const uint32_t q = blockIdx.x, tid = threadIdx.x, lane = tid & 63u, wave = tid >> 6;
+    const uint32_t tid = threadIdx.x, lane = tid & 63u, wave = tid >> 6;
+    uint32_t q = blockIdx.x;
+    if (p.dense_q) {
+        const uint32_t handed = *p.cnt_cursor;
+        if (handed > p.cnt_cap && p.fuse_walk && tid == 0u)
+            for (uint32_t o = blockIdx.x; o < p.nq; o += gridDim.x)
+                if ((!p.rec_nslots || p.rec_nslots[o] == 0u) && p.cnt_row[o] == 0xFFFFFFFFu) { p.walk.n_rows[p.q0 + o] = 0; p.walk.row_start[p.q0 + o] = 0; }
+        if (q >= (handed < p.cnt_cap ? handed : p.cnt_cap)) return;
+        q = p.dense_q[q];
+    }
     const uint64_t gq = p.q0 + q;
     if (p.rec_nslots && p.rec_nslots[q] != 0u) return;
     if (p.status[gq] != RTX_Q_OK || (p.cnt_row && p.cnt_row[q] == 0xFFFFFFFFu)) {
@@ -1054,8 +1068,9 @@
 #ifndef RTX_PREFIX_NW_PRUNED
 #define RTX_PREFIX_NW_PRUNED 2
 #endif
-    if (p.prune_thr) launch_taxon_prefix_nw<RTX_PREFIX_NW_PRUNED>(s, p, nq, lds);
-    else launch_taxon_prefix_nw<RTX_PREFIX_NW>(s, p, nq, lds);
+    const uint32_t grid = p.dense_q ? std::min(nq, p.cnt_cap) : nq;
+    if (p.prune_thr) launch_taxon_prefix_nw<RTX_PREFIX_NW_PRUNED>(s, p, grid, lds);
+    else launch_taxon_prefix_nw<RTX_PREFIX_NW>(s, p, grid, lds);
 }
 void launch_lineage_walk(hipStream_t s, const WalkParams &p, uint32_t nq) {
     hipLaunchKernelGGL(lineage_walk_kernel, dim3(nq), dim3(64), 0, s, p);
diff --git a/raxtax_amd/csrc/rtx_kernels.hpp b/raxtax_amd/csrc/rtx_kernels.hpp
--- a/raxtax_amd/csrc/rtx_kernels.hpp
+++ b/raxtax_amd/csrc/rtx_kernels.hpp
@@ -199,6 +199,8 @@
     uint32_t mode;
     const uint32_t *live;
     uint32_t live_words;
+    uint32_t *zero[3];
+    uint32_t zero_n[3];
 };
 
 constexpr uint32_t kRecMaxSlots = 16;
@@ -328,6 +330,7 @@
     uint32_t *cnt_row;
     uint32_t *cnt_cursor;
     uint32_t cnt_cap;
+    uint32_t *dense_q;
     uint32_t *flags_out;
 };
 constexpr uint32_t kPruneDetailWords = 72;
@@ -441,6 +444,10 @@
     WalkParams walk;
     const uint16_t *rec_nslots;
     const uint32_t *cnt_row;
+    const uint32_t *dense_q;
+    const uint32_t *cnt_cursor;
+    uint32_t cnt_cap;
+    uint32_t nq;
 };
 
 
@@ -476,11 +483,11 @@
 void launch_pair_union(hipStream_t s, const uint32_t *rows, const uint32_t *nrows, uint32_t rstride, uint32_t nq, uint2 *urec,
                        uint32_t *nu, uint32_t ustride);
 void launch_hit_count_pair(hipStream_t s, const HitParams &p, uint32_t nq, uint32_t ntiles, int planes);
-void launch_live_items(hipStream_t s, const uint32_t *live, uint32_t live_words, const uint32_t *pair_live, uint32_t nq, uint32_t ntiles, uint32_t *off,
-                       uint32_t *items, uint32_t *n_items);
+void launch_live_items(hipStream_t s, const uint32_t *live, uint32_t live_words, uint32_t nq, uint32_t ntiles, uint32_t *items, uint32_t *n_items,
+                       unsigned long long *stats);
 void launch_hit_count_pair_bounds(hipStream_t s, const HitParams &p, uint32_t nq, uint32_t u_ntiles, int planes);
 void launch_hit_count_pair_bounds_items(hipStream_t s, const HitParams &p, uint32_t nq, uint32_t u_ntiles, int planes);
-void launch_fine_bounds(hipStream_t s, const HitParams &p, uint32_t nq, uint32_t ntiles, uint32_t f_ntiles, uint32_t *pair_live, uint32_t *cnt,
+void launch_fine_bounds(hipStream_t s, const HitParams &p, uint32_t nq, uint32_t f_ntiles, const uint32_t *pair_live, uint32_t *cnt,
                         uint32_t *items, uint32_t *n_items, int planes);
 size_t prob_table_lds_bytes(uint32_t tmax);
 void launch_prob_table(hipStream_t s, const ProbParams &p, uint32_t nq);
diff --git a/raxtax_amd/csrc/rtx_prune.hip b/raxtax_amd/csrc/rtx_prune.hip
--- a/raxtax_amd/csrc/rtx_prune.hip
+++ b/raxtax_amd/csrc/rtx_prune.hip
@@ -417,15 +417,18 @@
             p.rec.nslots[pair * 2u] = (uint16_t)(ra ? n_rec[0] : 0u);
             if (has_b) p.rec.nslots[pair * 2u + 1u] = (uint16_t)(rb ? n_rec[1] : 0u);
             if (p.cnt_row) {
-                auto row_for = [&](bool records) -> uint32_t {
+                auto row_for = [&](bool records, uint32_t q) -> uint32_t {
                     if (records) return 0xFFFFFFFFu;
                     const uint32_t r = atomicAdd(p.cnt_cursor, 1u);
-                    if (r < p.cnt_cap) return r;
+                    if (r < p.cnt_cap) {
+                        if (p.dense_q) p.dense_q[r] = q;
+                        return r;
+                    }
                     atomicOr(p.flags_out, 4u);
                     return 0xFFFFFFFFu;
                 };
-                p.cnt_row[pair * 2u] = row_for(ra);
-                if (has_b) p.cnt_row[pair * 2u + 1u] = row_for(rb);
+                p.cnt_row[pair * 2u] = row_for(ra, pair * 2u);
+                if (has_b) p.cnt_row[pair * 2u + 1u] = row_for(rb, pair * 2u + 1u);
             }
         }
     }
```
